# TinyMPC/tinympc-julia

Hardware: AMD Instinct MI355X
Metric: qp_solves_per_sec (higher is better)
Workload: dtype f64 recurrences and state trajectory, f32 input slack / dual

## Files before the change

### tinympc-julia_amd/csrc/admm_lean.hip.h

```cpp
#pragma once
#include <hip/hip_runtime.h>

#include "admm_params.h"
#include "admm_quad.hip.h"

#ifndef TMPC_LEAN_KNOT_BARRIER
#define TMPC_LEAN_KNOT_BARRIER 0
#endif
#ifndef TMPC_LEAN_SPLITK
#define TMPC_LEAN_SPLITK 0
#endif

#ifndef TMPC_LEAN_WIDE_STORE
#define TMPC_LEAN_WIDE_STORE 1
#endif
#ifndef TMPC_LEAN_STORE_W
#define TMPC_LEAN_STORE_W 0
#endif
#ifndef TMPC_LEAN_PK
#define TMPC_LEAN_PK 1
#endif
#ifndef TMPC_LEAN_FOLD_FIRST
#define TMPC_LEAN_FOLD_FIRST 0
#endif

namespace tmpc {

template <int NX, int NU>
struct LeanPack {
    static constexpr LeanLayout LL = lean_layout(NX, NU);
    static constexpr int O_M = LL.oM, O_K = LL.oK, O_B = LL.oB, O_C = LL.oC, O_H = LL.oH, O_S = LL.oS, O_P = LL.oP, O_T = LL.oT, LEN = LL.len;
    static constexpr int NLOADS = LL.padded / 8;
};

typedef float lean_f2 __attribute__((ext_vector_type(2)));

__device__ __forceinline__ float clamp3(float t, float lo, float hi) { return __builtin_amdgcn_fmed3f(t, lo, hi); }
__device__ __forceinline__ double clamp3(double t, double lo, double hi) { return fmin(fmax(t, lo), hi); }
__device__ __forceinline__ float lean_max(float a, float b) { return fmaxf(a, b); }
__device__ __forceinline__ double lean_max(double a, double b) { return fmax(a, b); }
__device__ __forceinline__ float lean_abs(float a) { return fabsf(a); }
__device__ __forceinline__ double lean_abs(double a) { return fabs(a); }

constexpr int lean_park_stride(int EX) { return (((EX + 3) / 4) % 2 ? (EX + 3) / 4 : (EX + 3) / 4 + 1) * 4; }
template <int NX, int NU, int N, bool LIVE, bool UBK, bool ONE, bool XB = false, int REFS = REF_ZERO, class ST = float, uint64_t SP = 0, bool WS = false,
          bool MPC = false>
__global__ __launch_bounds__(256, (ONE ? 1 : 2)) void admm_lean_kernel(const AdmmParams P) {
    constexpr bool F64 = std::is_same<ST, double>::value;
    static_assert(!F64 || ONE, "fp64 state: the 512-register form");
    static_assert(!WS || !F64, "kept workspace: fp32 state (the fp64 workspace has another format)");
    static_assert(!MPC || (WS && LIVE && ONE), "in-kernel closed loop: the tolerance-terminated workspace-keeping form");
    static_assert(REFS == REF_ZERO || REFS == REF_SHARED, "lean kernel: zero or shared references");
#ifdef TMPC_LEAN_CLOCK_PROBE
    const unsigned long long probe_entry = __builtin_amdgcn_s_memrealtime();
#endif
    using L = LeanPack<NX, NU>;
    constexpr int EX = NX * N, EU = NU * (N - 1);
    constexpr bool SPR = SP != 0;
    static_assert(!SPR || (NX <= 4 && NU <= 4), "sparse pattern: nx, nu <= 4");
    constexpr bool HB = !SPR && !LIVE && !XB && ONE;
    constexpr bool PK = TMPC_LEAN_PK && ONE && !LIVE && !XB && !WS && UBK && !F64;
    auto mh_zero = [](int m, int j) { return HB && j < m - NU; };
    auto bh_zero = [](int m, int a) { return HB && m > a; };
    auto a_nz = [](int m, int j) { return !SPR || lsp_a(SP, NX, m, j); };
    auto a_one = [](int m, int j) { return SPR && lsp_one(SP, NX, m, j); };
    auto b_nz = [](int m, int a) { return !SPR || lsp_b(SP, NU, m, a); };
    constexpr int BW = 2 * NX + 2 * NU;
    static_assert(L::NLOADS <= 4, "coefficient block too large for SGPRs");

    __shared__ float s_bnd[UBK ? 1 : 2 * NU * (N - 1)];
    __shared__ float s_xb[XB ? 2 * NX * N : 1];
    __shared__ double s_cq[REFS == REF_SHARED ? NX * N : 1], s_cr[REFS == REF_SHARED ? NU * (N - 1) : 1], s_cpt[REFS == REF_SHARED ? NX : 1];
    const int tid = threadIdx.x;
    if constexpr (!UBK) {
        for (int i = tid; i < 2 * NU * (N - 1); i += 256) {
            const int k = i / (2 * NU), j = i % (2 * NU);
            s_bnd[i] = P.bounds[k * BW + 2 * NX + j];
        }
    }
    if constexpr (XB)
        for (int i = tid; i < 2 * NX * N; i += 256) s_xb[i] = P.bounds[(i / (2 * NX)) * BW + i % (2 * NX)];
    if constexpr (REFS == REF_SHARED) {
        const float *qd = P.bounds + N * BW, *rd = qd + NX;
        const double irho = 1.0 / P.rho_family;
        for (int i = tid; i < NU * (N - 1); i += 256) s_cr[i] = (double)P.uref[i] * (double)rd[i % NU] * irho;
        if constexpr (HB) {
            const double *T = P.lean + L::O_T;
            for (int k = tid; k < N; k += 256) {
                double c[NX];
                for (int j = 0; j < NX; ++j) c[j] = (double)P.xref[k * NX + j] * (double)qd[j] * irho;
                for (int m = 0; m < NX; ++m) {
                    double acc = 0.0;
                    for (int j = 0; j < NX; ++j) acc = fma(T[j * NX + m], c[j], acc);
                    s_cq[k * NX + m] = acc;
                }
            }
            if (tid == 0) {
                double c[NX];
                for (int i = 0; i < NX; ++i) {
                    double acc = 0.0;
                    for (int j = 0; j < NX; ++j) acc = fma(P.lean[L::O_P + j * NX + i], (double)P.xref[(N - 1) * NX + j], acc);
                    c[i] = acc * irho;
                }
                for (int m = 0; m < NX; ++m) {
                    double acc = 0.0;
                    for (int j = 0; j < NX; ++j) acc = fma(T[j * NX + m], c[j], acc);
                    s_cpt[m] = acc;
                }
            }
        } else {
            for (int i = tid; i < NX * N; i += 256) s_cq[i] = (double)P.xref[i] * (double)qd[i % NX] * irho;
            if (tid < NX) {
                double acc = 0.0;
                for (int j = 0; j < NX; ++j) acc = fma(P.lean[L::O_P + j * NX + tid], (double)P.xref[(N - 1) * NX + j], acc);
                s_cpt[tid] = acc * irho;
            }
        }
    }
    __shared__ double s_T[HB ? NX * NX : 1];
    if constexpr (HB)
        if (tid < NX * NX) s_T[tid] = P.lean[L::O_T + tid];
    if constexpr (!UBK || XB || REFS == REF_SHARED || HB) __syncthreads();
    const long b = (long)blockIdx.x * 256 + tid;
    const bool active = b < P.batch;
    const int lane = tid & 63;
    constexpr int SW = !TMPC_LEAN_WIDE_STORE ? 0 : (TMPC_LEAN_STORE_W ? TMPC_LEAN_STORE_W : wide_stage_width(EX));
    static_assert(SW == 0 || (SW % 4 == 0 && EX % SW == 0), "wide store: W a multiple of 4 that divides nx N");
    constexpr int STAGE = SW ? wave_stage_floats_wide(EU, SW) : wave_stage_floats(EU);
    static_assert(SW == 0 || 4 * 64 * wide_stage_stride(SW) * sizeof(float) <= 48 * 1024, "wide store: staging beyond its 48 KiB");
    __shared__ __attribute__((aligned(16))) float s_stage[4][STAGE];
    constexpr bool PARK = WS && LIVE;
    constexpr int PVS = lean_park_stride(EX), PZS = EU | 1;
    __shared__ __attribute__((aligned(16))) float s_pv[PARK ? 256 * PVS : 4];
    __shared__ float s_pz[PARK ? 256 * PZS : 1];

    const SBlock<double, L::NLOADS> blk(P.lean + (HB ? L::O_H : (SPR ? L::O_S : 0)));
    const auto cM = blk.at(L::O_M), cK = blk.at(L::O_K), cB = blk.at(L::O_B), cC = blk.at(L::O_C);

    ST lo[NU], hi[NU];
#pragma unroll
    for (int a = 0; a < NU; ++a) lo[a] = (ST)P.bounds[2 * NX + a], hi[a] = (ST)P.bounds[2 * NX + NU + a];

    double X[XB ? 1 : N][NX];
    ST G[XB ? N : 1][NX], QT[XB ? N : 1][NX];
    ST Y[N - 1][NU], Z[N - 1][NU];
    using DT = std::conditional_t<ONE, double, float>;
    DT D[N - 1][NU];
#pragma unroll
    for (int m = 0; m < NX; ++m) {
        if constexpr (WS) X[0][m] = !active ? 0.0 : (P.x0d ? P.x0d[b * NX + m] : (double)P.x0[b * NX + m]);
        else X[0][m] = active ? (double)P.x0[b * NX + m] : 0.0;
    }
    if constexpr (HB) {
        double x0[NX];
#pragma unroll
        for (int m = 0; m < NX; ++m) x0[m] = X[0][m];
#pragma unroll
        for (int m = 0; m < NX; ++m) {
            double acc = P.lean[L::O_T + m] * x0[0];
#pragma unroll
            for (int j = 1; j < NX; ++j) acc = fma(P.lean[L::O_T + j * NX + m], x0[j], acc);
            X[0][m] = acc;
        }
    }
#pragma unroll
    for (int k = 1; k < (XB ? 1 : N); ++k)
#pragma unroll
        for (int m = 0; m < NX; ++m) X[k][m] = 0.0;
#pragma unroll
    for (int k = 0; k < (XB ? N : 1); ++k)
#pragma unroll
        for (int m = 0; m < NX; ++m) G[k][m] = (ST)0, QT[k][m] = (ST)0;
#pragma unroll
    for (int k = 0; k < N - 1; ++k)
#pragma unroll
        for (int a = 0; a < NU; ++a) Y[k][a] = (ST)0, Z[k][a] = (ST)0, D[k][a] = (DT)0;
    if constexpr (MPC) {
        const unsigned long long mask = __builtin_amdgcn_ballot_w64(active);
        int td = tid;
        asm volatile("" : "+v"(td));
        const int ln = td & 63;
        const long w0 = (long)blockIdx.x * 256 + (td & ~63);
        float *so = s_stage[td >> 6];
        load_wave_x<EX>(so, P.sv + w0 * EX, ln, mask, [&](auto ee, float val) { s_pv[td * PVS + decltype(ee)::value] = val; });
        load_wave_u<EU>(so, P.sz + w0 * EU, ln, mask, [&](auto ee, float val) { s_pz[td * PZS + decltype(ee)::value] = val; });
    }
    if constexpr (WS && !MPC) {
        if (!P.cold_start) {
            const unsigned long long mask = __builtin_amdgcn_ballot_w64(active);
            int td = tid;
            asm volatile("" : "+v"(td));
            const int ln = td & 63;
            const long w0 = (long)blockIdx.x * 256 + (td & ~63);
            float *so = s_stage[td >> 6];
            if (mask) {
                if constexpr (XB) {
                    load_wave_x<EX>(so, P.sg + w0 * EX, ln, mask, [&](auto ee, float val) { constexpr int e = decltype(ee)::value; G[e / NX][e % NX] = val; });
                    load_wave_x<EX>(so, P.sv + w0 * EX, ln, mask, [&](auto ee, float val) { constexpr int e = decltype(ee)::value; QT[e / NX][e % NX] = val - G[e / NX][e % NX]; });
                } else {
                    load_wave_x<EX>(so, P.sv + w0 * EX, ln, mask, [&](auto ee, float val) { constexpr int e = decltype(ee)::value; if constexpr (e >= NX) X[e / NX][e % NX] = (double)val; });
                    if constexpr (HB) {
#pragma unroll
                        for (int k = 1; k < N; ++k) {
                            double vk[NX];
#pragma unroll
                            for (int m = 0; m < NX; ++m) vk[m] = X[k][m];
#pragma unroll
                            for (int m = 0; m < NX; ++m) {
                                double acc = P.lean[L::O_T + m] * vk[0];
#pragma unroll
                                for (int j = 1; j < NX; ++j) acc = fma(P.lean[L::O_T + j * NX + m], vk[j], acc);
                                X[k][m] = acc;
                            }
                        }
                    }
                }
                load_wave_u<EU>(so, P.sy + w0 * EU, ln, mask, [&](auto ee, float val) { constexpr int e = decltype(ee)::value; Y[e / NU][e % NU] = val; });
                load_wave_u<EU>(so, P.sz + w0 * EU, ln, mask, [&](auto ee, float val) { constexpr int e = decltype(ee)::value; Z[e / NU][e % NU] = val; });
                load_wave_u<EU>(so, P.sd + w0 * EU, ln, mask, [&](auto ee, float val) { constexpr int e = decltype(ee)::value; D[e / NU][e % NU] = (DT)val; });
            }
        }
    }

#ifdef TMPC_LEAN_CLOCK_PROBE
    const unsigned long long probe_t0 = __builtin_amdgcn_s_memtime(), probe_r0 = __builtin_amdgcn_s_memrealtime();
#endif
    int it = 0, conv = 0;
    ST res0 = 0, res1 = 0, res2 = 0, res3 = 0;
    const int ct = P.check_termination;
    const int last_check_it = ct > 0 ? (P.max_iter / ct) * ct : 0;
    const ST rho = F64 ? (ST)P.rho_family : (ST)P.rho;
    const ST ptol = F64 ? (ST)P.abs_pri_tol64 : (ST)P.abs_pri_tol, dtol = F64 ? (ST)P.abs_dua_tol64 : (ST)P.abs_dua_tol;
    double dua_x = 0.0;
    ST pri_u = 0, dua_u = 0, pri_xf = 0, dua_xf = 0;
    auto park_v = [&](int k, const float (&pv)[NX]) {
        float *row = s_pv + tid * PVS + k * NX;
        if constexpr (NX % 4 == 0) {
#pragma unroll
            for (int q = 0; q < NX / 4; ++q)
                *reinterpret_cast<float4 *>(row + 4 * q) = make_float4(pv[4 * q], pv[4 * q + 1], pv[4 * q + 2], pv[4 * q + 3]);
        } else {
#pragma unroll
            for (int m = 0; m < NX; ++m) row[m] = pv[m];
        }
    };
    auto state_sets = [&](auto res_tag, auto kk, const double (&x)[NX]) {
        constexpr bool RES = decltype(res_tag)::value;
        constexpr int k = decltype(kk)::value;
#pragma unroll
        for (int m = 0; m < NX; ++m) {
            const ST xf = (ST)x[m];
            const ST t = xf + G[k][m];
            const ST vn = clamp3(t, (ST)s_xb[k * 2 * NX + m], (ST)s_xb[k * 2 * NX + NX + m]);
            const ST gn = t - vn;
            if constexpr (RES && PARK) {
                if constexpr (MPC) {
                    if (!conv) s_pv[tid * PVS + k * NX + m] = (float)(QT[k][m] + G[k][m]);
                } else {
                    s_pv[tid * PVS + k * NX + m] = (float)(QT[k][m] + G[k][m]);
                }
            }
            if constexpr (RES) {
                pri_xf = lean_max(pri_xf, lean_abs(xf - vn));
                dua_xf = lean_max(dua_xf, lean_abs((QT[k][m] + G[k][m]) - vn));
            }
            G[k][m] = gn;
            QT[k][m] = vn - gn;
        }
    };

    auto load_T = [&](double (&Tm)[NX * NX]) {
        const double *tp = s_T;
        asm volatile("" : "+v"(tp));
#pragma unroll
        for (int i = 0; i < NX * NX; ++i) Tm[i] = tp[i];
    };
    auto to_x = [](const double (&Tm)[NX * NX], const double (&xh)[NX], int m) {
        double acc = Tm[m * NX] * xh[0];
#pragma unroll
        for (int j = 1; j < NX; ++j) acc = fma(Tm[m * NX + j], xh[j], acc);
        return acc;
    };

    auto forward = [&](auto res_tag, bool first_iter) {
        constexpr bool RES = decltype(res_tag)::value;
        if constexpr (RES) {
            dua_x = 0.0, pri_u = 0, dua_u = 0, pri_xf = 0, dua_xf = 0;
            if constexpr (WS && !XB) {
                float v0p[NX];
#pragma unroll
                for (int m = 0; m < NX; ++m) v0p[m] = (float)X[0][m];
                if (first_iter) {
                    int td = tid;
                    asm volatile("" : "+v"(td));
                    const long bb = (long)blockIdx.x * 256 + td;
                    const bool warm0 = bb < P.batch && !P.cold_start;
                    double x0v[NX];
                    if constexpr (HB) {
                        double Tm[NX * NX];
#pragma unroll
                        for (int i = 0; i < NX * NX; ++i) Tm[i] = P.lean[L::O_T + i];
#pragma unroll
                        for (int m = 0; m < NX; ++m) x0v[m] = to_x(Tm, X[0], m);
                    } else {
#pragma unroll
                        for (int m = 0; m < NX; ++m) x0v[m] = X[0][m];
                    }
#pragma unroll
                    for (int m = 0; m < NX; ++m) {
                        if constexpr (MPC) v0p[m] = s_pv[td * PVS + m];
                        else v0p[m] = warm0 ? P.sv[bb * EX + m] : 0.f;
                        dua_x = fmax(dua_x, fabs((double)v0p[m] - x0v[m]));
                    }
                }
                if constexpr (PARK) {
                    if constexpr (MPC) {
                        if (!conv) park_v(0, v0p);
                    } else {
                        park_v(0, v0p);
                    }
                }
            }
            if constexpr (!WS && !XB)
                if (first_iter) {
#pragma unroll
                    for (int m = 0; m < NX; ++m) {
                        if constexpr (HB) {
                            double Tm[NX * NX];
                            load_T(Tm);
                            dua_x = fmax(dua_x, fabs(to_x(Tm, X[0], m)));
                        } else {
                            dua_x = fmax(dua_x, fabs(X[0][m]));
                        }
                    }
                }
        }
        if constexpr (HB || (SPR && (ONE || XB)))
#pragma unroll
            for (int m = 0; m < NX; ++m) asm volatile("" : "+v"(X[0][m]));
        double xr[NX];
#pragma unroll
        for (int m = 0; m < NX; ++m) xr[m] = X[0][m];
        float upk[PK ? NU : 1];
        sfor<0, N - 1>([&](auto kk) {
            constexpr int k = decltype(kk)::value;
            constexpr int kx = XB ? 0 : k;
            if constexpr (!UBK || XB) asm volatile("" ::: "memory");
            if constexpr (XB) state_sets(res_tag, kk, xr);
            const double (&xk)[NX] = XB ? xr : X[kx];
            double dk[NU], u[NU], xn[NX];
#pragma unroll
            for (int a = 0; a < NU; ++a) dk[a] = (double)D[k][a];
            bool started[NX];
            if constexpr (!SPR) {
#pragma unroll
                for (int m = 0; m < NX; ++m) {
                    started[m] = false;
#pragma unroll
                    for (int a = 0; a < NU; ++a) {
                        if (bh_zero(m, a)) continue;
                        xn[m] = started[m] ? fma(-cB[m * NU + a], dk[a], xn[m]) : -(cB[m * NU + a] * dk[a]);
                        started[m] = true;
                    }
                }
#pragma unroll
                for (int j = 0; j < NX; ++j)
#pragma unroll
                    for (int m = 0; m < NX; ++m) {
                        if (mh_zero(m, j)) continue;
                        xn[m] = started[m] ? fma(cM[m * NX + j], xk[j], xn[m]) : cM[m * NX + j] * xk[j];
                        started[m] = true;
                    }
            }
#pragma unroll
            for (int a = 0; a < NU; ++a) {
                if constexpr (SPR) {
                    double acc = -dk[a];
#pragma unroll
                    for (int pass = 0; pass < 2; ++pass)
#pragma unroll
                        for (int j = 0; j < NX; ++j) {
                            bool late = false;
#pragma unroll
                            for (int c = 0; c < NU; ++c) late = late || b_nz(j, c);
                            if (late == (pass == 1)) acc = fma(-cK[a * NX + j], xk[j], acc);
                        }
                    u[a] = acc;
                } else if constexpr (TMPC_LEAN_SPLITK && NX >= 4) {
                    double u0 = -dk[a], u1 = -(cK[a * NX + NX / 2] * xk[NX / 2]);
#pragma unroll
                    for (int j = 0; j < NX / 2; ++j) u0 = fma(-cK[a * NX + j], xk[j], u0);
#pragma unroll
                    for (int j = NX / 2 + 1; j < NX; ++j) u1 = fma(-cK[a * NX + j], xk[j], u1);
                    u[a] = u0 + u1;
                } else {
                    double acc = -dk[a];
#pragma unroll
                    for (int j = 0; j < NX; ++j) acc = fma(-cK[a * NX + j], xk[j], acc);
                    u[a] = acc;
                }
            }
            if constexpr (SPR) {
#pragma unroll
                for (int m = 0; m < NX; ++m) {
                    int s = -1;
#pragma unroll
                    for (int j = NX - 1; j >= 0; --j)
                        if (a_one(m, j)) s = j;
                    started[m] = s >= 0;
                    xn[m] = 0.0;
                    if (s >= 0) xn[m] = xk[s];
#pragma unroll
                    for (int j = 0; j < NX; ++j) {
                        if (!a_nz(m, j) || j == s) continue;
                        xn[m] = !started[m] ? cM[m * NX + j] * xk[j] : (a_one(m, j) ? xn[m] + xk[j] : fma(cM[m * NX + j], xk[j], xn[m]));
                        started[m] = true;
                    }
#pragma unroll
                    for (int a = 0; a < NU; ++a) {
                        if (!b_nz(m, a)) continue;
                        xn[m] = started[m] ? fma(cB[m * NU + a], u[a], xn[m]) : cB[m * NU + a] * u[a];
                        started[m] = true;
                    }
                }
            }
            constexpr bool PK_ODD = PK && !RES && (k & 1), PK_EVEN = PK && !RES && !(k & 1) && k + 1 < N - 1;
            if constexpr (PK_EVEN) {
#pragma unroll
                for (int a = 0; a < NU; ++a) upk[a] = (float)u[a];
            }
            if constexpr (PK_ODD) {
#pragma unroll
                for (int a = 0; a < NU; ++a) {
                    const lean_f2 t = lean_f2{upk[a], (float)u[a]} + lean_f2{(float)Y[k - 1][a], (float)Y[k][a]};
                    const lean_f2 zn = {clamp3(t.x, (float)lo[a], (float)hi[a]), clamp3(t.y, (float)lo[a], (float)hi[a])};
                    const lean_f2 yn = t - zn;
                    Y[k - 1][a] = yn.x, Y[k][a] = yn.y;
                    Z[k - 1][a] = zn.x, Z[k][a] = zn.y;
                }
            }
            if constexpr (!PK_ODD && !PK_EVEN)
#pragma unroll
            for (int a = 0; a < NU; ++a) {
                const ST uf = (ST)u[a];
                const ST t = uf + Y[k][a];
                ST l_ = lo[a], h_ = hi[a];
                if constexpr (!UBK) l_ = (ST)s_bnd[k * 2 * NU + a], h_ = (ST)s_bnd[k * 2 * NU + NU + a];
                const ST zn = clamp3(t, l_, h_);
                Y[k][a] = t - zn;
                if constexpr (RES) {
                    pri_u = lean_max(pri_u, lean_abs(uf - zn));
                    dua_u = lean_max(dua_u, lean_abs(Z[k][a] - zn));
                    if constexpr (PARK) {
                        if constexpr (MPC) {
                            if (!conv) s_pz[tid * PZS + k * NU + a] = (float)Z[k][a];
                        } else {
                            s_pz[tid * PZS + k * NU + a] = (float)Z[k][a];
                        }
                    }
                }
                Z[k][a] = zn;
            }
            if constexpr (RES && PARK && !XB) {
                float pv[NX];
#pragma unroll
                for (int m = 0; m < NX; ++m) pv[m] = (float)X[k + 1][m];
                if constexpr (MPC) {
                    if (!conv) park_v(k + 1, pv);
                } else {
                    park_v(k + 1, pv);
                }
            }
#pragma unroll
            for (int m = 0; m < NX; ++m) {
                if constexpr (XB) {
                    xr[m] = xn[m];
                } else {
                    if constexpr (RES && !HB) dua_x = fmax(dua_x, fabs(X[k + 1][m] - xn[m]));
                    if constexpr (!(RES && HB)) X[k + 1][m] = xn[m];
                }
            }
            if constexpr (RES && HB) {
                double dl[NX], Tm[NX * NX];
                load_T(Tm);
#pragma unroll
                for (int m = 0; m < NX; ++m) dl[m] = X[k + 1][m] - xn[m], X[k + 1][m] = xn[m];
#pragma unroll
                for (int m = 0; m < NX; ++m) dua_x = fmax(dua_x, fabs(to_x(Tm, dl, m)));
            }
            if constexpr (RES) asm volatile("" : "+v"(pri_u), "+v"(dua_u), "+v"(dua_x), "+v"(pri_xf), "+v"(dua_xf));
            if constexpr (TMPC_LEAN_KNOT_BARRIER) __builtin_amdgcn_sched_barrier(0);
        });
        if constexpr (XB) {
            asm volatile("" ::: "memory");
            state_sets(res_tag, std::integral_constant<int, N - 1>{}, xr);
            if constexpr (RES) asm volatile("" : "+v"(pri_xf), "+v"(dua_xf));
        }
    };

    auto backward = [&]() {
        double p[NX];
        if constexpr (REFS == REF_SHARED) asm volatile("" ::: "memory");
#pragma unroll
        for (int m = 0; m < NX; ++m) {
            p[m] = XB ? (double)QT[N - 1][m] : X[XB ? 0 : N - 1][m];
            if constexpr (REFS == REF_SHARED) p[m] += s_cpt[m];
        }
        float rpk[PK ? NU : 1];
        sfor<0, N - 1>([&](auto kk) {
            constexpr int k = N - 2 - decltype(kk)::value;
            double r[NU], t[NU];
            if constexpr (REFS == REF_SHARED) asm volatile("" ::: "memory");
#pragma unroll
            for (int a = 0; a < NU; ++a) {
                if constexpr (PK && (k & 1)) {
                    const lean_f2 rp = lean_f2{(float)Z[k - 1][a], (float)Z[k][a]} - lean_f2{(float)Y[k - 1][a], (float)Y[k][a]};
                    rpk[a] = rp.x;
                    r[a] = (double)rp.y;
                } else if constexpr (PK && k + 1 < N - 1) {
                    r[a] = (double)rpk[a];
                } else
                r[a] = (double)(Z[k][a] - Y[k][a]);
                if constexpr (REFS == REF_SHARED) r[a] += s_cr[k * NU + a];
                t[a] = r[a];
            }
#pragma unroll
            for (int j = 0; j < NX; ++j)
#pragma unroll
                for (int a = 0; a < NU; ++a)
                    if (!bh_zero(j, a) && b_nz(j, a)) t[a] = fma(cB[j * NU + a], p[j], t[a]);
#pragma unroll
            for (int a = 0; a < NU; ++a) {
                double acc = cC[a * NU] * t[0];
#pragma unroll
                for (int c = 1; c < NU; ++c) acc = fma(cC[a * NU + c], t[c], acc);
                D[k][a] = (DT)acc;
            }
            if constexpr (k > 0 && SPR) {
                double ap[NX];
#pragma unroll
                for (int m = 0; m < NX; ++m) {
                    double acc = XB ? (double)QT[k][m] : X[XB ? 0 : k][m];
                    if constexpr (REFS == REF_SHARED) acc += s_cq[k * NX + m];
#pragma unroll
                    for (int j = 0; j < NX; ++j)
                        if (a_nz(j, m)) acc = a_one(j, m) ? acc + p[j] : fma(cM[j * NX + m], p[j], acc);
#pragma unroll
                    for (int a = 0; a < NU; ++a) acc = fma(-cK[a * NX + m], t[a], acc);
                    ap[m] = acc;
                }
#pragma unroll
                for (int m = 0; m < NX; ++m) p[m] = ap[m];
            } else if constexpr (k > 0) {
                double ap[NX];
#pragma unroll
                for (int m = 0; m < NX; ++m) {
                    double acc = XB ? (double)QT[k][m] : X[XB ? 0 : k][m];
                    if constexpr (REFS == REF_SHARED) acc += s_cq[k * NX + m];
#pragma unroll
                    for (int a = 0; a < NU; ++a) acc = fma(-cK[a * NX + m], r[a], acc);
                    ap[m] = acc;
                }
#pragma unroll
                for (int j = 0; j < NX; ++j)
#pragma unroll
                    for (int m = 0; m < NX; ++m)
                        if (!mh_zero(j, m)) ap[m] = fma(cM[j * NX + m], p[j], ap[m]);
#pragma unroll
                for (int m = 0; m < NX; ++m) p[m] = ap[m];
            }
            if constexpr (TMPC_LEAN_KNOT_BARRIER) __builtin_amdgcn_sched_barrier(0);
        });
    };

    double Ts[HB ? NX * NX : 1];
    auto vnew_at = [&](auto kk, auto mm) -> float {
        constexpr int k = decltype(kk)::value, m = decltype(mm)::value;
        if constexpr (XB) return (float)clamp3(QT[k][m] + G[k][m], (ST)s_xb[k * 2 * NX + m], (ST)s_xb[k * 2 * NX + NX + m]);
        else if constexpr (HB) return (float)to_x(Ts, X[k], m);
        else return (float)X[XB ? 0 : k][m];
    };
    auto store = [&](bool solved_flag) {
        float *xo = P.xout + b * EX, *uo = P.uout + b * EU, *ro = P.res + b * 4;
        asm volatile("" : "+v"(xo), "+v"(uo), "+v"(ro));
        sfor<0, N>([&](auto kk) {
            constexpr int k = decltype(kk)::value;
            sfor<0, NX>([&](auto mm) { xo[k * NX + decltype(mm)::value] = vnew_at(kk, mm); });
            __builtin_amdgcn_sched_barrier(0);
        });
#pragma unroll
        for (int k = 0; k < N - 1; ++k)
#pragma unroll
            for (int a = 0; a < NU; ++a) uo[k * NU + a] = (float)Z[k][a];
        P.iter[b] = P.iter_offset + it;
        P.solved[b] = solved_flag ? 1 : 0;
        ro[0] = (float)res0;
        ro[1] = (float)res1;
        ro[2] = (float)res2;
        ro[3] = (float)res3;
    };

    auto store_ws = [&](unsigned long long mask, bool mine, auto conv_tag) {
        constexpr bool CV = decltype(conv_tag)::value;
        int td = tid;
        asm volatile("" : "+v"(td));
        const int ln = td & 63;
        const long bb = (long)blockIdx.x * 256 + td;
        float *so = s_stage[td >> 6];
        const long w0 = (long)blockIdx.x * 256 + (td & ~63);
        auto pair = [&](float *xo, float *uo, auto &&gx, auto &&gu) {
            if constexpr (SW != 0) store_wave_wide<EX, EU, SW>(so, xo, uo, ln, mask, gx, gu);
            else store_wave_coalesced<EX, EU>(so, xo, uo, ln, mask, gx, gu);
        };
        auto single = [&](float *uo, auto &&gu) {
            if constexpr (SW != 0) {
                if (mask == ~0ull) store_wave_u_wide<EU>(so, uo, ln, gu);
                else store_wave_u<EU, false>(so, uo, ln, mask, gu);
            } else {
                store_wave_u<EU, false>(so, uo, ln, mask, gu);
            }
        };
        auto getx = [&](auto ee) { constexpr int e = decltype(ee)::value; return vnew_at(std::integral_constant<int, e / NX>{}, std::integral_constant<int, e % NX>{}); };
        auto getu = [&](auto ee) { constexpr int e = decltype(ee)::value; return (float)Z[e / NU][e % NU]; };
        auto gety = [&](auto ee) { constexpr int e = decltype(ee)::value; return (float)Y[e / NU][e % NU]; };
        auto getd = [&](auto ee) { constexpr int e = decltype(ee)::value; return (float)D[e / NU][e % NU]; };
        pair(P.xout + w0 * EX, P.uout + w0 * EU, getx, getu);
        if (P.save_state) {
            if constexpr (CV) {
                pair(P.sv + w0 * EX, P.sz + w0 * EU, [&](auto ee) { return s_pv[td * PVS + decltype(ee)::value]; },
                     [&](auto ee) { return s_pz[td * PZS + decltype(ee)::value]; });
            } else {
                pair(P.sv + w0 * EX, P.sz + w0 * EU, getx, getu);
            }
            if constexpr (XB) pair(P.sg + w0 * EX, P.sy + w0 * EU, [&](auto ee) { constexpr int e = decltype(ee)::value; return (float)G[e / NX][e % NX]; }, gety);
            else single(P.sy + w0 * EU, gety);
            single(P.sd + w0 * EU, getd);
        }
        if (mine) {
            float *ro = P.res + bb * 4;
            P.iter[bb] = P.iter_offset + it;
            P.solved[bb] = CV ? 1 : 0;
            ro[0] = (float)res0, ro[1] = (float)res1, ro[2] = (float)res2, ro[3] = (float)res3;
        }
    };

    const bool can_converge = P.abs_pri_tol > 0.f && P.abs_dua_tol > 0.f;
    const int max_iter = P.max_iter;
    auto store_step = [&](unsigned long long mask) {
        int td = tid;
        asm volatile("" : "+v"(td));
        const int ln = td & 63;
        float *so = s_stage[td >> 6];
        const long w0 = (long)blockIdx.x * 256 + (td & ~63);
        auto single = [&](float *uo, auto &&gu) {
            if constexpr (SW != 0) {
                if (mask == ~0ull) store_wave_u_wide<EU>(so, uo, ln, gu);
                else store_wave_u<EU, false>(so, uo, ln, mask, gu);
            } else {
                store_wave_u<EU, false>(so, uo, ln, mask, gu);
            }
        };
        auto gety = [&](auto ee) { constexpr int e = decltype(ee)::value; return (float)Y[e / NU][e % NU]; };
        auto getd = [&](auto ee) { constexpr int e = decltype(ee)::value; return (float)D[e / NU][e % NU]; };
        if constexpr (XB) {
            auto getg = [&](auto ee) { constexpr int e = decltype(ee)::value; return (float)G[e / NX][e % NX]; };
            if constexpr (SW != 0) store_wave_wide<EX, EU, SW>(so, P.sg + w0 * EX, P.sy + w0 * EU, ln, mask, getg, gety);
            else store_wave_coalesced<EX, EU>(so, P.sg + w0 * EX, P.sy + w0 * EU, ln, mask, getg, gety);
        } else {
            single(P.sy + w0 * EU, gety);
        }
        single(P.sd + w0 * EU, getd);
    };
    float u0c[MPC ? NU : 1];
    auto plant = [&](int step, bool final_step) {
        const double *ab = P.lean + L::O_S;
        double xn[NX];
#pragma unroll
        for (int r = 0; r < NX; ++r) {
            double acc = 0.0;
#pragma unroll
            for (int j = 0; j < NX; ++j) acc = fma(ab[L::O_M + r * NX + j], X[0][j], acc);
#pragma unroll
            for (int a = 0; a < NU; ++a) acc = fma(ab[L::O_B + r * NU + a], (double)u0c[a], acc);
            xn[r] = acc;
        }
        int td = tid;
        asm volatile("" : "+v"(td));
        const long bb = (long)blockIdx.x * 256 + td;
        if (bb < P.batch) {
            const long so = bb * P.mpc_steps + step;
#pragma unroll
            for (int r = 0; r < NX; ++r) P.mpc_x[so * NX + r] = (float)xn[r];
#pragma unroll
            for (int a = 0; a < NU; ++a) P.mpc_u[so * NU + a] = u0c[a];
            P.mpc_iter[so] = conv ? P.iter_offset + it : -(P.iter_offset + it);
            if (final_step) {
#pragma unroll
                for (int r = 0; r < NX; ++r) P.x0_out[bb * NX + r] = (float)xn[r];
                if (double *xd = const_cast<double *>(P.x0d)) {
#pragma unroll
                    for (int r = 0; r < NX; ++r) xd[bb * NX + r] = xn[r];
                }
            }
        }
#pragma unroll
        for (int r = 0; r < NX; ++r) X[0][r] = xn[r];
    };
    int step = 0;
#ifdef TMPC_LEAN_CLOCK_PROBE
    unsigned long long probe_ph[4] = {0, 0, 0, 0}, probe_a = 0, probe_c = 0;
#endif
    do {
#ifdef TMPC_LEAN_CLOCK_PROBE
    probe_a = __builtin_amdgcn_s_memtime();
#endif
    if constexpr (MPC) {
        __builtin_amdgcn_fence(__ATOMIC_ACQUIRE, "agent");
        int td = tid;
        asm volatile("" : "+v"(td));
        const int ln = td & 63;
        const long w0 = (long)blockIdx.x * 256 + (td & ~63);
        const unsigned long long mask = __builtin_amdgcn_ballot_w64(w0 + ln < P.batch);
        float *so = s_stage[td >> 6];
        const float *rv = s_pv + td * PVS, *rz = s_pz + td * PZS;
        if constexpr (XB) {
            load_wave_x<EX>(so, P.sg + w0 * EX, ln, mask, [&](auto ee, float val) { constexpr int e = decltype(ee)::value; G[e / NX][e % NX] = val; });
            sfor<0, EX>([&](auto ee) { constexpr int e = decltype(ee)::value; QT[e / NX][e % NX] = rv[e] - G[e / NX][e % NX]; });
        } else {
            sfor<NX, EX>([&](auto ee) { constexpr int e = decltype(ee)::value; X[e / NX][e % NX] = (double)rv[e]; });
        }
        sfor<0, EU>([&](auto ee) { constexpr int e = decltype(ee)::value; Z[e / NU][e % NU] = rz[e]; });
        load_wave_u<EU>(so, P.sy + w0 * EU, ln, mask, [&](auto ee, float val) { constexpr int e = decltype(ee)::value; Y[e / NU][e % NU] = val; });
        load_wave_u<EU>(so, P.sd + w0 * EU, ln, mask, [&](auto ee, float val) { constexpr int e = decltype(ee)::value; D[e / NU][e % NU] = (DT)val; });
        it = 0, conv = 0;
        res0 = 0, res1 = 0, res2 = 0, res3 = 0;
    }
    const bool last_step = !MPC || step + 1 >= P.mpc_steps;
#ifdef TMPC_LEAN_CLOCK_PROBE
    probe_ph[0] += __builtin_amdgcn_s_memtime() - probe_a, probe_a = __builtin_amdgcn_s_memtime();
#endif
    int i = 0;
    while (i < max_iter) {
        int next_res = max_iter;
        if (ct > 0) {
            if (LIVE && can_converge) next_res = (i / ct) * ct + ct - 1;
            else if (last_check_it - 1 >= i) next_res = last_check_it - 1;
        }
        const int n_plain = (next_res < max_iter ? next_res : max_iter) - i;
        for (int j = 0; j < n_plain; ++j) {
            forward(std::false_type{}, false);
            backward();
        }
        i += n_plain;
        if (!LIVE || !conv) it += n_plain;
        if (i >= max_iter) break;
        forward(std::true_type{}, i == 0);
        i += 1;
        if (!LIVE || !conv) {
            it += 1;
            res0 = XB ? pri_xf : (ST)0;
            res1 = (XB ? dua_xf : (ST)dua_x) * rho;
            res2 = pri_u;
            res3 = dua_u * rho;
        }
        if constexpr (LIVE) {
            const bool now = active && !conv && res0 < ptol && res2 < ptol && res1 < dtol && res3 < dtol;
            if constexpr (WS) {
                const unsigned long long cm = __builtin_amdgcn_ballot_w64(now);
                if constexpr (MPC) {
#ifdef TMPC_LEAN_CLOCK_PROBE
                    probe_c = __builtin_amdgcn_s_memtime();
#endif
                    if (cm) {
                        if (last_step) store_ws(cm, now, std::true_type{});
                        else store_step(cm);
                    }
#ifdef TMPC_LEAN_CLOCK_PROBE
                    probe_ph[2] += __builtin_amdgcn_s_memtime() - probe_c;
#endif
                    if (now) {
#pragma unroll
                        for (int a = 0; a < NU; ++a) u0c[a] = (float)Z[0][a];
                    }
                } else
                if (cm) store_ws(cm, now, std::true_type{});
                if (now) conv = 1;
            } else
            if (now) {
                store(true);
                conv = 1;
            }
            if (!__builtin_amdgcn_ballot_w64(active && !conv)) break;
        }
        if (!(ONE && !XB) || WS || i < max_iter) backward();
    }
    if constexpr (MPC) {
#ifdef TMPC_LEAN_CLOCK_PROBE
        probe_ph[1] += __builtin_amdgcn_s_memtime() - probe_a, probe_a = __builtin_amdgcn_s_memtime();
#endif
#pragma unroll
        for (int a = 0; a < NU; ++a)
            if (!conv) u0c[a] = (float)Z[0][a];
        if (last_step) break;
        const bool mine = active && !conv;
        const unsigned long long mask = __builtin_amdgcn_ballot_w64(mine);
        if (mask) {
            if (mine) {
                int td = tid;
                asm volatile("" : "+v"(td));
                float *rv = s_pv + td * PVS, *rz = s_pz + td * PZS;
                sfor<0, EX>([&](auto ee) {
                    constexpr int e = decltype(ee)::value;
                    rv[e] = vnew_at(std::integral_constant<int, e / NX>{}, std::integral_constant<int, e % NX>{});
                });
                sfor<0, EU>([&](auto ee) { constexpr int e = decltype(ee)::value; rz[e] = (float)Z[e / NU][e % NU]; });
            }
            store_step(mask);
        }
        plant(step, false);
        asm volatile("s_waitcnt vmcnt(0)" ::: "memory");
#ifdef TMPC_LEAN_CLOCK_PROBE
        probe_ph[3] += __builtin_amdgcn_s_memtime() - probe_a;
#endif
        ++step;
    }
    } while (MPC);
    auto fold = [&]() {
        float m0 = active ? (float)res0 : 0.f, m1 = active ? (float)res1 : 0.f, m2 = active ? (float)res2 : 0.f, m3 = active ? (float)res3 : 0.f;
#pragma unroll
        for (int o = 1; o < 64; o <<= 1) {
            m0 = fmaxf(m0, __shfl_xor(m0, o, 64));
            m1 = fmaxf(m1, __shfl_xor(m1, o, 64));
            m2 = fmaxf(m2, __shfl_xor(m2, o, 64));
            m3 = fmaxf(m3, __shfl_xor(m3, o, 64));
        }
        const unsigned long long unsolved = __builtin_amdgcn_ballot_w64(active && !conv);
        if constexpr (WS) fold_status(P, m0, m1, m2, m3, __popcll(unsolved), tid);
        else fold_status_records(P, m0, m1, m2, m3, __popcll(unsolved), tid);
    };
#ifdef TMPC_LEAN_CLOCK_PROBE
    const unsigned long long probe_t1 = __builtin_amdgcn_s_memtime(), probe_r1 = __builtin_amdgcn_s_memrealtime();
    unsigned long long probe_fold = 0;
#endif
    if constexpr (TMPC_LEAN_FOLD_FIRST) {
        fold();
#ifdef TMPC_LEAN_CLOCK_PROBE
        probe_fold = __builtin_amdgcn_s_memrealtime();
#endif
    }
    {
        const bool mine = active && !conv;
        const unsigned long long mask = __builtin_amdgcn_ballot_w64(mine);
        if (mask) {
            if constexpr (HB) load_T(Ts);
            if constexpr (WS) {
                store_ws(mask, mine, std::false_type{});
            } else {
                const long w0 = (long)blockIdx.x * 256 + (tid & ~63);
                auto getx = [&](auto ee) { constexpr int e = decltype(ee)::value; return vnew_at(std::integral_constant<int, e / NX>{}, std::integral_constant<int, e % NX>{}); };
                auto getu = [&](auto ee) { constexpr int e = decltype(ee)::value; return (float)Z[e / NU][e % NU]; };
                if constexpr (SW != 0) store_wave_wide<EX, EU, SW>(s_stage[tid >> 6], P.xout + w0 * EX, P.uout + w0 * EU, lane, mask, getx, getu);
                else store_wave_coalesced<EX, EU>(s_stage[tid >> 6], P.xout + w0 * EX, P.uout + w0 * EU, lane, mask, getx, getu);
                if (mine) {
                    float *ro = P.res + b * 4;
                    P.iter[b] = P.iter_offset + it;
                    P.solved[b] = 0;
                    ro[0] = (float)res0, ro[1] = (float)res1, ro[2] = (float)res2, ro[3] = (float)res3;
                }
            }
        }
    }
    if constexpr (MPC) plant(step, true);
#ifdef TMPC_LEAN_CLOCK_PROBE
    if (active) P.iter[b] = (int)(__builtin_amdgcn_s_memrealtime() & 0xFFFFFFull);
    __builtin_amdgcn_s_waitcnt(0);
    if (active) P.solved[b] = (int)(__builtin_amdgcn_s_memrealtime() & 0xFFFFFFull);
#endif
    if constexpr (!TMPC_LEAN_FOLD_FIRST) {
        fold();
#ifdef TMPC_LEAN_CLOCK_PROBE
        probe_fold = __builtin_amdgcn_s_memrealtime();
#endif
    }
#ifdef TMPC_LEAN_CLOCK_PROBE
    if constexpr (MPC) {
        if (active)
            for (int q = 0; q < 4; ++q) P.res[b * 4 + q] = (float)probe_ph[q];
    } else
    if (active) {
        P.res[b * 4 + 0] = (float)(probe_t1 - probe_t0);
        P.res[b * 4 + 1] = (float)(probe_r1 - probe_r0);
        P.res[b * 4 + 2] = (float)(probe_entry & 0xFFFFFFull);
        P.res[b * 4 + 3] = (float)(probe_fold & 0xFFFFFFull);
    }
#endif
}

}
```

### tinympc-julia_amd/csrc/admm_params.h

```cpp
#pragma once
#include <stdint.h>

namespace tmpc {

enum RefMode : int {
    REF_ZERO = 0,
    REF_SHARED = 1,
    REF_PER_INSTANCE = 2,
};

enum { QUAD_REF_SEQ_MAX_N = 20 };

enum { GSTAT_WORDS = 8 };
enum { GSLOT_WORDS = 8, GSLOT_DEFAULT_CAP = 1024 };

constexpr int LIN_MAX_ROWS = 8, GEN_MAX_NX = 64;
constexpr int GEN_MAX_NU = 32;

struct AdmmParams {
    const float *coef;
    const float *bounds;
    const float *x0;
    const double *x0d;
    const float *xref;
    const float *uref;
    float *xout;
    float *uout;
    int *iter;
    int *solved;
    float *res;
    float *sd, *sy, *sz, *sg, *sv;
    uint32_t *gstat;
    uint32_t *gacc;
    float *scratch;
    const int *idx;
    int iter_offset;
    int batch;
    int max_iter;
    int check_termination;
    int ref_mode;
    int cold_start;
    int save_state;
    float abs_pri_tol, abs_dua_tol, rho;
    int nx, nu, N;
    int mpc_steps;
    float *mpc_x;
    float *mpc_u;
    int *mpc_iter;
    float *x0_out;
    int xb_active;
    int has_fdyn;
    int ncx, ncu;
    int Acx[8], qcx[8], Acu[8], qcu[8];
    float cx[8], cu[8];
    float *sgc, *svc, *syc, *szc;
    int mlx, mlu;
    const float *lin;
    float *sgl, *svl, *syl, *szl;
    int adaptive_rho;
    int rho_clip;
    double rho_family;
    float rho_min, rho_max;
    const double *sens;
    double *adapt;
    long adapt_stride;
    void *adp_cols;
    const float *het_aux;
    int bounds_stride;
    const float *xref_seq, *uref_seq;
    const double *lean;
    int host_flags;
    double *ws64;
    double abs_pri_tol64, abs_dua_tol64;
    uint32_t *gslot;
    int gslot_cap;
    const float *ibx, *ibu;
    long ib_kx, ib_ku, ib_hx, ib_hu;
    int ib_on;
};
enum : int { IB_STATE = 1, IB_INPUT = 2 };
enum : int { HF_NO_REFILL = 1, HF_NO_UNI = 2, HF_NO_OS = 4 };

struct LeanLayout {
    int oM;
    int oK;
    int oB;
    int oC;
    int len;
    int padded;
    int oH;
    int oS;
    int oP;
    int oT;
    int total;
};
constexpr LeanLayout lean_layout(int nx, int nu) {
    return LeanLayout{0, nx * nx, nx * nx + nu * nx, nx * nx + 2 * nu * nx, nx * nx + 2 * nu * nx + nu * nu,
                      (nx * nx + 2 * nu * nx + nu * nu + 7) / 8 * 8, (nx * nx + 2 * nu * nx + nu * nu + 7) / 8 * 8,
                      2 * ((nx * nx + 2 * nu * nx + nu * nu + 7) / 8 * 8),
                      3 * ((nx * nx + 2 * nu * nx + nu * nu + 7) / 8 * 8),
                      3 * ((nx * nx + 2 * nu * nx + nu * nu + 7) / 8 * 8) + nx * nx,
                      3 * ((nx * nx + 2 * nu * nx + nu * nu + 7) / 8 * 8) + 2 * nx * nx};
}

enum : int { LSP_UNIT = 16, LSP_B = 32, LSP_ON = 48 };
constexpr bool lsp_a(uint64_t sp, int nx, int i, int j) { return (sp >> (i * nx + j)) & 1; }
constexpr bool lsp_one(uint64_t sp, int nx, int i, int j) { return (sp >> (LSP_UNIT + i * nx + j)) & 1; }
constexpr bool lsp_b(uint64_t sp, int nu, int i, int a) { return (sp >> (LSP_B + i * nu + a)) & 1; }
constexpr uint64_t lean_pattern_rm(int nx, int nu, const double *A, const double *B) {
    if (nx < 1 || nu < 1 || nx > 4 || nu > 4) return 0;
    uint64_t sp = 1ull << LSP_ON;
    for (int i = 0; i < nx; ++i) {
        for (int j = 0; j < nx; ++j) {
            if (A[i * nx + j] != 0.0) sp |= 1ull << (i * nx + j);
            if (A[i * nx + j] == 1.0) sp |= 1ull << (LSP_UNIT + i * nx + j);
        }
        for (int a = 0; a < nu; ++a)
            if (B[i * nu + a] != 0.0) sp |= 1ull << (LSP_B + i * nu + a);
    }
    return sp;
}
constexpr int lean_cost_sparse(uint64_t sp, int nx, int nu) {
    int c = 2 * nx * nu + nu * nu;
    for (int i = 0; i < nx; ++i) {
        int terms = 0;
        bool unit = false;
        for (int j = 0; j < nx; ++j) terms += lsp_a(sp, nx, i, j), unit = unit || lsp_one(sp, nx, i, j);
        for (int a = 0; a < nu; ++a) terms += 2 * lsp_b(sp, nu, i, a);
        for (int j = 0; j < nx; ++j) terms += lsp_a(sp, nx, j, i);
        c += terms - (unit ? 1 : 0);
    }
    return c;
}
constexpr int lean_cost_hessenberg(int nx, int nu) {
    int band = 0, trap = 0;
    for (int m = 0; m < nx; ++m) {
        for (int j = 0; j < nx; ++j) band += j >= m - nu;
        for (int a = 0; a < nu; ++a) trap += m <= a;
    }
    return 2 * band + 2 * trap + 2 * nx * nu + nu * nu;
}
constexpr int lean_cost_dense(int nx, int nu) { return 2 * nx * nx + 4 * nx * nu + nu * nu; }
constexpr bool lean_pattern_covers(uint64_t built, uint64_t model) {
    const uint64_t nz = 0xFFFFull | (0xFFFFull << LSP_B), one = 0xFFFFull << LSP_UNIT;
    return built != 0 && model != 0 && (model & nz & ~built) == 0 && ((built & one) & ~(model & one)) == 0;
}

#ifdef __HIPCC__
__device__ __forceinline__ void fold_status(const AdmmParams &P, float m0, float m1, float m2, float m3,
                                            int unsolved_in_wave, int tid) {
    __shared__ float s_fold_m[4][4];
    __shared__ int s_fold_u[4];
    const int w = tid >> 6, nw = ((int)blockDim.x + 63) >> 6;
    const bool merged = nw <= 4;
    if ((tid & 63) == 0) {
        if (merged) {
            s_fold_m[w][0] = m0, s_fold_m[w][1] = m1, s_fold_m[w][2] = m2, s_fold_m[w][3] = m3;
            s_fold_u[w] = unsolved_in_wave;
        } else {
            atomicMax(&P.gacc[0], __float_as_uint(m0));
            atomicMax(&P.gacc[1], __float_as_uint(m1));
            atomicMax(&P.gacc[2], __float_as_uint(m2));
            atomicMax(&P.gacc[3], __float_as_uint(m3));
            if (unsolved_in_wave) atomicAdd(&P.gacc[4], (uint32_t)unsolved_in_wave);
        }
    }
    __syncthreads();
    if (tid == 0) {
        if (merged) {
            int un = 0;
            for (int i = 0; i < nw; ++i) {
                m0 = i ? fmaxf(m0, s_fold_m[i][0]) : s_fold_m[0][0];
                m1 = i ? fmaxf(m1, s_fold_m[i][1]) : s_fold_m[0][1];
                m2 = i ? fmaxf(m2, s_fold_m[i][2]) : s_fold_m[0][2];
                m3 = i ? fmaxf(m3, s_fold_m[i][3]) : s_fold_m[0][3];
                un += s_fold_u[i];
            }
            atomicMax(&P.gacc[0], __float_as_uint(m0));
            atomicMax(&P.gacc[1], __float_as_uint(m1));
            atomicMax(&P.gacc[2], __float_as_uint(m2));
            atomicMax(&P.gacc[3], __float_as_uint(m3));
            if (un) atomicAdd(&P.gacc[4], (uint32_t)un);
        }
        __threadfence();
        if (atomicAdd(&P.gacc[7], 1u) == gridDim.x - 1) {
            __threadfence();
            uint32_t tot[5];
#pragma unroll
            for (int i = 0; i < 5; ++i) tot[i] = atomicExch(&P.gacc[i], 0u);
            atomicExch(&P.gacc[6], 0u);
            atomicExch(&P.gacc[7], 0u);
#pragma unroll
            for (int i = 0; i < 5; ++i) P.gstat[i] = tot[i];
        }
    }
}

__device__ __forceinline__ void fold_status_records(const AdmmParams &P, float m0, float m1, float m2, float m3,
                                            int unsolved_in_wave, int tid) {
    __shared__ float s_fold_m[4][4];
    __shared__ int s_fold_u[4];
    const int w = tid >> 6, nw = ((int)blockDim.x + 63) >> 6;
    const bool merged = nw <= 4;
    if ((tid & 63) == 0) {
        if (merged) {
            s_fold_m[w][0] = m0, s_fold_m[w][1] = m1, s_fold_m[w][2] = m2, s_fold_m[w][3] = m3;
            s_fold_u[w] = unsolved_in_wave;
        } else {
            atomicMax(&P.gacc[0], __float_as_uint(m0));
            atomicMax(&P.gacc[1], __float_as_uint(m1));
            atomicMax(&P.gacc[2], __float_as_uint(m2));
            atomicMax(&P.gacc[3], __float_as_uint(m3));
            if (unsolved_in_wave) atomicAdd(&P.gacc[4], (uint32_t)unsolved_in_wave);
        }
    }
    __syncthreads();
    if (tid >= 64) return;
    const int nrec = P.gslot ? min((int)gridDim.x, P.gslot_cap) : 0;
    int last = 0;
    if (tid == 0) {
        bool recorded = false;
        if (merged) {
            int un = 0;
            for (int i = 0; i < nw; ++i) {
                m0 = i ? fmaxf(m0, s_fold_m[i][0]) : s_fold_m[0][0];
                m1 = i ? fmaxf(m1, s_fold_m[i][1]) : s_fold_m[0][1];
                m2 = i ? fmaxf(m2, s_fold_m[i][2]) : s_fold_m[0][2];
                m3 = i ? fmaxf(m3, s_fold_m[i][3]) : s_fold_m[0][3];
                un += s_fold_u[i];
            }
            if ((int)blockIdx.x < nrec) {
                unsigned long long *rec = reinterpret_cast<unsigned long long *>(P.gslot + (size_t)blockIdx.x * GSLOT_WORDS);
                __hip_atomic_store(rec + 0, (unsigned long long)__float_as_uint(m0) | ((unsigned long long)__float_as_uint(m1) << 32),
                                   __ATOMIC_RELAXED, __HIP_MEMORY_SCOPE_AGENT);
                __hip_atomic_store(rec + 1, (unsigned long long)__float_as_uint(m2) | ((unsigned long long)__float_as_uint(m3) << 32),
                                   __ATOMIC_RELAXED, __HIP_MEMORY_SCOPE_AGENT);
                __hip_atomic_store(rec + 2, (unsigned long long)(uint32_t)un, __ATOMIC_RELAXED, __HIP_MEMORY_SCOPE_AGENT);
                asm volatile("s_waitcnt vmcnt(0)" ::: "memory");
                recorded = true;
            } else {
                atomicMax(&P.gacc[0], __float_as_uint(m0));
                atomicMax(&P.gacc[1], __float_as_uint(m1));
                atomicMax(&P.gacc[2], __float_as_uint(m2));
                atomicMax(&P.gacc[3], __float_as_uint(m3));
                if (un) atomicAdd(&P.gacc[4], (uint32_t)un);
            }
        }
        if (!recorded) __threadfence();
        last = __hip_atomic_fetch_add(&P.gacc[7], 1u, __ATOMIC_RELAXED, __HIP_MEMORY_SCOPE_AGENT) == gridDim.x - 1;
    }
    if (!__shfl(last, 0, 64)) return;
    __builtin_amdgcn_fence(__ATOMIC_ACQUIRE, "agent");
    uint32_t tot[5] = {0, 0, 0, 0, 0};
    if (tid == 0) {
#pragma unroll
        for (int i = 0; i < 5; ++i) tot[i] = atomicExch(&P.gacc[i], 0u);
        atomicExch(&P.gacc[6], 0u);
        atomicExch(&P.gacc[7], 0u);
    }
    uint32_t r0 = 0, r1 = 0, r2 = 0, r3 = 0, ru = 0;
    for (int base = 0; base < nrec; base += 4 * 64) {
        unsigned long long a[4], b[4], c[4];
#pragma unroll
        for (int q = 0; q < 4; ++q) {
            const int s = min(base + q * 64 + tid, nrec - 1);
            unsigned long long *rec = reinterpret_cast<unsigned long long *>(P.gslot + (size_t)s * GSLOT_WORDS);
            a[q] = __hip_atomic_load(rec + 0, __ATOMIC_RELAXED, __HIP_MEMORY_SCOPE_AGENT);
            b[q] = __hip_atomic_load(rec + 1, __ATOMIC_RELAXED, __HIP_MEMORY_SCOPE_AGENT);
            c[q] = __hip_atomic_load(rec + 2, __ATOMIC_RELAXED, __HIP_MEMORY_SCOPE_AGENT);
        }
#pragma unroll
        for (int q = 0; q < 4; ++q)
            if (base + q * 64 + tid >= nrec) a[q] = b[q] = c[q] = 0;
#pragma unroll
        for (int q = 0; q < 4; ++q) {
            r0 = max(r0, (uint32_t)a[q]), r1 = max(r1, (uint32_t)(a[q] >> 32));
            r2 = max(r2, (uint32_t)b[q]), r3 = max(r3, (uint32_t)(b[q] >> 32));
            ru += (uint32_t)c[q];
        }
    }
    if (nrec) {
#pragma unroll
        for (int off = 1; off < 64; off <<= 1) {
            r0 = max(r0, (uint32_t)__shfl_xor((int)r0, off, 64)), r1 = max(r1, (uint32_t)__shfl_xor((int)r1, off, 64));
            r2 = max(r2, (uint32_t)__shfl_xor((int)r2, off, 64)), r3 = max(r3, (uint32_t)__shfl_xor((int)r3, off, 64));
            ru += (uint32_t)__shfl_xor((int)ru, off, 64);
        }
    }
    if (tid == 0) {
        tot[0] = max(tot[0], r0), tot[1] = max(tot[1], r1), tot[2] = max(tot[2], r2), tot[3] = max(tot[3], r3), tot[4] += ru;
#pragma unroll
        for (int i = 0; i < 5; ++i) P.gstat[i] = tot[i];
    }
}
#endif

}
```

### tinympc-julia_amd/csrc/kernels.hip

```cpp
#include <algorithm>
#include <atomic>
#include <cmath>
#include <cstring>
#include <limits>

#include "admm_generic.hip.h"
#include "host_setup.h"
#include "solver.h"

namespace tmpc {

#define TMPC_ENTRY(NX, NU, NN, GG) const KernelEntry *quad_entry_##NX##_##NU##_##NN##_g##GG();
TMPC_ENTRY(4, 1, 20, 4) TMPC_ENTRY(4, 1, 20, 2) TMPC_ENTRY(4, 1, 20, 1)
TMPC_ENTRY(4, 1, 10, 4) TMPC_ENTRY(4, 1, 10, 2) TMPC_ENTRY(4, 1, 10, 1) TMPC_ENTRY(4, 1, 2, 4)
TMPC_ENTRY(4, 1, 5, 4) TMPC_ENTRY(4, 1, 5, 1) TMPC_ENTRY(4, 1, 15, 4) TMPC_ENTRY(4, 1, 15, 1) TMPC_ENTRY(4, 1, 30, 4) TMPC_ENTRY(4, 1, 30, 1)
TMPC_ENTRY(12, 4, 30, 4) TMPC_ENTRY(12, 4, 20, 4)
TMPC_ENTRY(6, 3, 10, 4) TMPC_ENTRY(6, 3, 10, 2) TMPC_ENTRY(6, 3, 50, 4)
#undef TMPC_ENTRY

const KernelEntry *find_quad_kernel(int nx, int nu, int N, int group) {
    static const KernelEntry *const table[] = {
        quad_entry_4_1_20_g4(),  quad_entry_4_1_20_g2(),  quad_entry_4_1_20_g1(), quad_entry_4_1_10_g4(),
        quad_entry_4_1_10_g2(),  quad_entry_4_1_10_g1(),  quad_entry_4_1_2_g4(),  quad_entry_12_4_30_g4(),
        quad_entry_12_4_20_g4(), quad_entry_6_3_10_g4(),  quad_entry_6_3_10_g2(), quad_entry_6_3_50_g4(),
        quad_entry_4_1_5_g4(),   quad_entry_4_1_5_g1(),   quad_entry_4_1_15_g4(), quad_entry_4_1_15_g1(),
        quad_entry_4_1_30_g4(),  quad_entry_4_1_30_g1(),
    };
    for (const KernelEntry *e : table)
        if (e->nx == nx && e->nu == nu && e->N == N && (group < 0 || e->G == group)) return e;
    return jit_find(false, nx, nu, N, group);
}

const KernelEntry *mfma_entry_12_4_30();
const KernelEntry *mfma_entry_12_4_25();
const KernelEntry *mfma_entry_12_4_20();
const KernelEntry *mfma_entry_12_4_15();
const KernelEntry *mfma_entry_12_4_10();

const KernelEntry *find_mfma_kernel(int nx, int nu, int N) {
    static const KernelEntry *const table[] = {mfma_entry_12_4_30(), mfma_entry_12_4_25(), mfma_entry_12_4_20(), mfma_entry_12_4_15(),
                                               mfma_entry_12_4_10()};
    for (const KernelEntry *e : table)
        if (e->nx == nx && e->nu == nu && e->N == N) return e;
    return jit_find(true, nx, nu, N, -1);
}

const LeanEntry *lean_entry_4_1_20();
const LeanEntry *lean_entry_4_1_15();
const LeanEntry *lean_entry_4_1_10();
const LeanEntry *lean_entry_4_1_5();

const LeanEntry *find_lean_kernel(int nx, int nu, int N) {
    static const LeanEntry *const table[] = {lean_entry_4_1_20(), lean_entry_4_1_15(), lean_entry_4_1_10(), lean_entry_4_1_5()};
    for (const LeanEntry *e : table)
        if (e->nx == nx && e->nu == nu && e->N == N) return e;
    return nullptr;
}

bool build_lean_pack(const Solver &sv, std::vector<double> &out) {
    const int nx = sv.nx, nu = sv.nu;
    const LeanLayout L = lean_layout(nx, nu);
    out.assign((size_t)L.total, 0.0);
    const Cache &c = sv.cache;
    double scale = 0.0, diff = 0.0;
    for (int i = 0; i < nx; ++i)
        for (int j = 0; j < nx; ++j) {
            double m = sv.A(i, j);
            for (int a = 0; a < nu; ++a) m -= sv.B(i, a) * c.Kinf(a, j);
            out[L.oM + i * nx + j] = m;
            scale = std::max(scale, std::fabs(m));
            diff = std::max(diff, std::fabs(m - c.AmBKt(j, i)));
        }
    if (!(diff <= 1e-12 * std::max(scale, 1.0))) return false;
    for (int i = 0; i < nx; ++i)
        for (int j = 0; j < nx; ++j) out[L.oM + i * nx + j] = c.AmBKt(j, i);
    for (int a = 0; a < nu; ++a)
        for (int j = 0; j < nx; ++j) out[L.oK + a * nx + j] = c.Kinf(a, j);
    for (int i = 0; i < nx; ++i)
        for (int a = 0; a < nu; ++a) out[L.oB + i * nu + a] = sv.B(i, a);
    for (int a = 0; a < nu; ++a)
        for (int b2 = 0; b2 < nu; ++b2) out[L.oC + a * nu + b2] = -c.rho * c.Quu_inv(a, b2);
    for (int i = 0; i < nx; ++i)
        for (int j = 0; j < nx; ++j) out[L.oP + i * nx + j] = c.Pinf(i, j);
    std::vector<double> Mh((size_t)nx * nx), Bh((size_t)nx * nu);
    staircase_form(nx, nu, out.data() + L.oM, out.data() + L.oB, out.data() + L.oT, Mh.data(), Bh.data());
    const double *T = out.data() + L.oT;
    for (int i = 0; i < nx * nx; ++i) out[L.oH + L.oM + i] = Mh[i];
    for (int i = 0; i < nx * nu; ++i) out[L.oH + L.oB + i] = Bh[i];
    for (int a = 0; a < nu; ++a)
        for (int j = 0; j < nx; ++j) {
            double s = 0.0;
            for (int l = 0; l < nx; ++l) s += c.Kinf(a, l) * T[l * nx + j];
            out[L.oH + L.oK + a * nx + j] = s;
        }
    for (int i = 0; i < nu * nu; ++i) out[L.oH + L.oC + i] = out[L.oC + i];
    for (int i = 0; i < nx; ++i)
        for (int j = 0; j < nx; ++j) out[L.oS + L.oM + i * nx + j] = sv.A(i, j);
    for (int i = L.oK; i < L.len; ++i) out[L.oS + i] = out[i];
    return true;
}

void append_lean_bounds(const Solver &sv, std::vector<double> &out) {
    constexpr float kInf = std::numeric_limits<float>::infinity();
    const int nx = sv.nx, nu = sv.nu, N = sv.N, BW = 2 * nx + 2 * nu;
    std::vector<float> lb((size_t)N * BW + nx + nu + 1, 0.f);
    for (int k = 0; k < N; ++k) {
        float *p = lb.data() + (size_t)k * BW;
        for (int r = 0; r < nx; ++r) {
            p[r] = sv.st.en_state_bound ? (float)sv.x_min[r + (size_t)k * nx] : -kInf;
            p[nx + r] = sv.st.en_state_bound ? (float)sv.x_max[r + (size_t)k * nx] : kInf;
        }
        for (int a = 0; a < nu; ++a) {
            const bool on = sv.st.en_input_bound && k < N - 1;
            p[2 * nx + a] = on ? (float)sv.u_min[a + (size_t)k * nu] : -kInf;
            p[2 * nx + nu + a] = on ? (float)sv.u_max[a + (size_t)k * nu] : kInf;
        }
    }
    for (int r = 0; r < nx; ++r) lb[(size_t)N * BW + r] = (float)sv.cache.Qd[r];
    for (int a = 0; a < nu; ++a) lb[(size_t)N * BW + nx + a] = (float)sv.cache.Rd[a];
    const size_t at = out.size();
    out.resize(at + (lb.size() + 1) / 2, 0.0);
    std::memcpy(out.data() + at, lb.data(), lb.size() * sizeof(float));
}

LeanPlan lean_plan(const LeanPlanIn &in) {
    LeanPlan p;
    const int nx = in.nx, nu = in.nu, N = in.N;
    const bool f64 = in.precision == 2 && in.quad_G == 0 && in.lean_jit && !in.stream_ext;
    if (!(in.quad_G ? in.precision == 0 : f64) || !in.lean_ok || !(in.builtin || in.lean_jit)) return p;
    if (in.indexed || in.ref_mode == REF_PER_INSTANCE || in.adaptive_rho || in.iters < 1) return p;
    const bool ws = !(in.cold && !in.save);
    if (ws && !(in.sw_ws && in.quad_G > 0 && in.quad_G < 16 && in.precision == 0 && (!in.builtin || (in.kinds & LK_WS)))) return p;
    const bool mpc = in.loop && in.sw_loop && ws && in.mpc_steps > 0;
    if ((in.loop || in.mpc_steps > 0) && !mpc) return p;
    const bool xb = in.state_bounds || (ws && in.g_maybe_nonzero), shared = in.ref_mode == REF_SHARED;
    const bool live = in.live || mpc || (ws && xb && shared && in.knot_bounds);
    const bool one = live || ws || f64 || in.sw_one || (in.slots + 255) / 256 <= in.cus ||
                     (!in.builtin && 2 * N * nx + 3 * N * nu + 50 > 250);
    if (ws && !in.builtin && !lean_ws_fits(nx, nu, N, live, xb, shared, in.knot_bounds)) return p;
    bool sparse_allowed = !in.sw_dense;
    p.sp = in.model_sp;
    if (in.builtin) {
        const bool has = (in.kinds & (mpc ? LK_SPARSE_MPC : (ws ? LK_SPARSE_WS : LK_SPARSE))) != 0;
        p.sp = has ? in.builtin_sp : 0;
        sparse_allowed = sparse_allowed && has && in.ref_mode == REF_ZERO && !in.knot_bounds;
    }
    p.form = lean_pick_form(nx, nu, p.sp, in.model_sp, one, live, xb, sparse_allowed);
    if (mpc && in.builtin && !(in.kinds & (p.form == LF_SPARSE ? LK_SPARSE_MPC : LK_MPC))) return LeanPlan();
    p.take = true;
    p.variant = (live ? LV_LIVE : 0) | (in.knot_bounds ? 0 : LV_UBK) | (one ? LV_ONE : 0) | (xb ? LV_XB : 0) | (shared ? LV_SHARED : 0) |
                (f64 ? LV_F64 : 0) | (p.form == LF_SPARSE ? LV_SPARSE : 0) | (ws ? LV_WS : 0) | (mpc ? LV_MPC : 0);
    p.cost_sparse = p.sp ? lean_cost_sparse(p.sp, nx, nu) : 0;
    p.cost_dense = (one && !live && !xb) ? lean_cost_hessenberg(nx, nu) : lean_cost_dense(nx, nu);
    return p;
}

uint64_t lean_pattern(const Mat &A, const Mat &B) {
    const int nx = A.r, nu = B.c;
    if (nx < 1 || nu < 1 || nx > 4 || nu > 4) return 0;
    double a[16], b[16];
    for (int i = 0; i < nx; ++i) {
        for (int j = 0; j < nx; ++j) a[i * nx + j] = A(i, j);
        for (int c = 0; c < nu; ++c) b[i * nu + c] = B(i, c);
    }
    return lean_pattern_rm(nx, nu, a, b);
}

}

extern "C" unsigned long long tmpc_lean_pattern(int nx, int nu, const double *A, const double *B) {
    return (A && B) ? tmpc::lean_pattern_rm(nx, nu, A, B) : 0;
}
extern "C" int tmpc_lean_costs(int nx, int nu, unsigned long long sp, int *out3) {
    if (nx < 1 || nu < 1 || nx > 4 || nu > 4 || !out3) return 1;
    out3[0] = tmpc::lean_cost_sparse(sp, nx, nu), out3[1] = tmpc::lean_cost_hessenberg(nx, nu), out3[2] = tmpc::lean_cost_dense(nx, nu);
    return 0;
}
extern "C" int tmpc_lean_covers(unsigned long long built, unsigned long long model) { return tmpc::lean_pattern_covers(built, model) ? 1 : 0; }
extern "C" int tmpc_lean_pick_form(int nx, int nu, unsigned long long built, unsigned long long model, int one, int live, int xb) {
    return tmpc::lean_pick_form(nx, nu, built, model, one != 0, live != 0, xb != 0, true);
}
extern "C" unsigned long long tmpc_lean_builtin_pattern(int nx, int nu, int N) {
    const tmpc::LeanEntry *e = tmpc::find_lean_kernel(nx, nu, N);
    return (e && (e->kinds & tmpc::LK_SPARSE)) ? e->sp : 0;
}
extern "C" int tmpc_lean_plan(const int *in, int n_in, unsigned long long builtin_sp, unsigned long long model_sp, int *out5,
                              unsigned long long *weighed) {
    if (!in || n_in != 28 || !out5) return -1;
    tmpc::LeanPlanIn q;
    int i = 0;
    q.nx = in[i++], q.nu = in[i++], q.N = in[i++];
    q.builtin = in[i++] != 0, q.kinds = in[i++], q.builtin_sp = builtin_sp;
    q.lean_jit = in[i++] != 0, q.lean_ok = in[i++] != 0, q.model_sp = model_sp, q.knot_bounds = in[i++] != 0;
    q.quad_G = in[i++], q.precision = in[i++];
    q.sw_one = in[i++] != 0, q.sw_dense = in[i++] != 0, q.sw_ws = in[i++] != 0, q.sw_loop = in[i++] != 0;
    q.slots = in[i++], q.iters = in[i++], q.mpc_steps = in[i++];
    q.cold = in[i++] != 0, q.save = in[i++] != 0, q.indexed = in[i++] != 0, q.adaptive_rho = in[i++] != 0;
    q.ref_mode = in[i++];
    q.loop = in[i++] != 0, q.state_bounds = in[i++] != 0, q.g_maybe_nonzero = in[i++] != 0, q.live = in[i++] != 0, q.stream_ext = in[i++] != 0;
    q.cus = in[i++];
    const tmpc::LeanPlan p = tmpc::lean_plan(q);
    out5[0] = p.take ? 1 : 0, out5[1] = p.variant, out5[2] = p.form, out5[3] = p.cost_sparse, out5[4] = p.cost_dense;
    if (weighed) *weighed = p.sp;
    return 0;
}

namespace tmpc {

const KernelEntry *select_quad_kernel(int nx, int nu, int N, int batch) {
    const int pref[2][3] = {{1, 2, 4}, {4, 2, 1}};
    const int *order = batch >= 20480 ? pref[0] : pref[1];
    for (int i = 0; i < 3; ++i)
        if (const KernelEntry *e = find_quad_kernel(nx, nu, N, order[i])) return e;
    return nullptr;
}

const ConeEntry *mfmac_entry_6_3();
const ConeEntry *mfmar_entry_6_3_50();
const ConeEntry *mfmar_entry_6_3_10();
const ConeEntry *mfmar_entry_6_3_20();
const ConeEntry *mfmar_entry_6_3_30();

const ConeEntry *find_cone_kernel(int nx, int nu, int N) {
    static const ConeEntry *const table[] = {mfmar_entry_6_3_50(), mfmar_entry_6_3_30(), mfmar_entry_6_3_20(), mfmar_entry_6_3_10(), mfmac_entry_6_3()};
    for (const ConeEntry *e : table)
        if (e->nx == nx && e->nu == nu && e->N == N) return e;
    return nullptr;
}

const ConeEntry *mfmat_entry_6_3_50();
const ConeEntry *mfmat_entry_6_3_30();
const ConeEntry *mfmat_entry_6_3_20();
const ConeEntry *mfmat_entry_6_3_10();

const ConeEntry *find_trans_kernel(int nx, int nu, int N) {
    static const ConeEntry *const table[] = {mfmat_entry_6_3_50(), mfmat_entry_6_3_30(), mfmat_entry_6_3_20(), mfmat_entry_6_3_10()};
    for (const ConeEntry *e : table)
        if (e->nx == nx && e->nu == nu && e->N == N) return e;
    return nullptr;
}

int device_cu_count() {
    static std::atomic<int> cus[64];
    int dev = 0;
    if (hipGetDevice(&dev) != hipSuccess) return 256;
    int c = cus[dev & 63].load(std::memory_order_relaxed);
    if (c <= 0) {
        hipDeviceProp_t prop;
        c = hipGetDeviceProperties(&prop, dev) == hipSuccess && prop.multiProcessorCount > 0 ? prop.multiProcessorCount : 256;
        cus[dev & 63].store(c, std::memory_order_relaxed);
    }
    return c;
}

const StreamEntry *stream4_entry_2_1();
const StreamEntry *stream4_entry_2_2();
const StreamEntry *stream4_entry_3_1();
const StreamEntry *stream4_entry_3_2();
const StreamEntry *stream4_entry_3_3();
const StreamEntry *stream4_entry_4_1();
const StreamEntry *stream4_entry_4_2();
const StreamEntry *stream4_entry_4_3();
const StreamEntry *stream4_entry_4_4();
const StreamEntry *stream4_entry_6_1();
const StreamEntry *stream4_entry_6_2();
const StreamEntry *stream4_entry_6_3();
const StreamEntry *stream4_entry_6_4();
const StreamEntry *stream4_entry_8_1();
const StreamEntry *stream4_entry_8_2();
const StreamEntry *stream4_entry_8_3();
const StreamEntry *stream4_entry_8_4();
const StreamEntry *stream4_entry_10_1();
const StreamEntry *stream4_entry_10_2();
const StreamEntry *stream4_entry_10_3();
const StreamEntry *stream4_entry_10_4();
const StreamEntry *stream4_entry_12_1();
const StreamEntry *stream4_entry_12_2();
const StreamEntry *stream4_entry_12_3();
const StreamEntry *stream4_entry_12_4();

const StreamEntry *find_stream_kernel(int nx, int nu) {
    static const StreamEntry *const table[] = {stream4_entry_2_1(), stream4_entry_2_2(), stream4_entry_3_1(), stream4_entry_3_2(), stream4_entry_3_3(), stream4_entry_4_1(), stream4_entry_4_2(), stream4_entry_4_3(), stream4_entry_4_4(), stream4_entry_6_1(), stream4_entry_6_2(), stream4_entry_6_3(), stream4_entry_6_4(), stream4_entry_8_1(), stream4_entry_8_2(), stream4_entry_8_3(), stream4_entry_8_4(), stream4_entry_10_1(), stream4_entry_10_2(), stream4_entry_10_3(), stream4_entry_10_4(), stream4_entry_12_1(), stream4_entry_12_2(), stream4_entry_12_3(), stream4_entry_12_4()};
    for (const StreamEntry *e : table)
        if (e->nx == nx && e->nu == nu) return e;
    return nullptr;
}

hipError_t launch_generic(const AdmmParams &P, int precision, hipStream_t stream) {
    const int threads = 256;
    const int grid = (P.batch + threads - 1) / threads;
    if (P.ibx) {
        if (precision == 2)
            hipLaunchKernelGGL((admm_generic_kernel<double, double, true>), dim3(grid), dim3(threads), 0, stream, P);
        else if (precision == 0)
            hipLaunchKernelGGL((admm_generic_kernel<double, float, true>), dim3(grid), dim3(threads), 0, stream, P);
        else
            hipLaunchKernelGGL((admm_generic_kernel<float, float, true>), dim3(grid), dim3(threads), 0, stream, P);
        return hipGetLastError();
    }
    if (precision == 2)
        hipLaunchKernelGGL((admm_generic_kernel<double, double>), dim3(grid), dim3(threads), 0, stream, P);
    else if (precision == 0)
        hipLaunchKernelGGL((admm_generic_kernel<double, float>), dim3(grid), dim3(threads), 0, stream, P);
    else
        hipLaunchKernelGGL((admm_generic_kernel<float, float>), dim3(grid), dim3(threads), 0, stream, P);
    return hipGetLastError();
}

template <class RT>
static void fill_generic_coef(const Solver &sv, std::vector<unsigned char> &out) {
    const int nx = sv.nx, nu = sv.nu;
    const GenericPack pk(nx, nu);
    out.assign((size_t)pk.len * sizeof(RT), 0);
    auto put = [&](size_t idx, double val) {
        const RT v = (RT)val;
        std::memcpy(out.data() + idx * sizeof(RT), &v, sizeof(RT));
    };
    const Cache &c = sv.cache;
    for (int j = 0; j < nx; ++j)
        for (int i = 0; i < nx; ++i) {
            put(pk.oA + i + j * nx, sv.A(i, j));
            put(pk.oP + i + j * nx, c.Pinf(i, j));
            put(pk.oAt + i + j * nx, c.AmBKt(i, j));
        }
    for (int a = 0; a < nu; ++a)
        for (int i = 0; i < nx; ++i) {
            put(pk.oB + i + a * nx, sv.B(i, a));
            put(pk.oK + a + i * nu, c.Kinf(a, i));
        }
// ... 43 lines not shown
```

### tinympc-julia_amd/csrc/lean_entry.hip.h

```cpp
#pragma once
#include <hip/hip_ext.h>

#include "admm_lean.hip.h"
#include "solver.h"

namespace tmpc {

template <class K>
inline void lean_dispatch(K kernel, int grid, hipStream_t stream, hipEvent_t ev0, hipEvent_t ev1, const AdmmParams &P) {
    if (ev0 || ev1) hipExtLaunchKernelGGL(kernel, dim3(grid), dim3(256), 0, stream, ev0, ev1, 0, P);
    else hipLaunchKernelGGL(kernel, dim3(grid), dim3(256), 0, stream, P);
}

#define TMPC_LEAN_ARGS const AdmmParams &P, int variant, hipStream_t stream, hipEvent_t ev0, hipEvent_t ev1

template <int NX, int NU, int N, bool XB, int REFS, bool WS = false, bool MPC = false>
hipError_t launch_lean_v(TMPC_LEAN_ARGS) {
    const int grid = (P.batch + 255) / 256;
    constexpr bool FIXED = !MPC, FIXED_KNOT = FIXED && !(WS && XB && REFS == REF_SHARED), TWO = !WS;
#define TMPC_LEAN_LAUNCH(LIVE_, UBK_, ONE_) \
    lean_dispatch(admm_lean_kernel<NX, NU, N, LIVE_, UBK_, ONE_, XB, REFS, float, 0, WS, MPC>, grid, stream, ev0, ev1, P)
    switch (variant & (LV_LIVE | LV_UBK | LV_ONE)) {
        case LV_LIVE | LV_UBK | LV_ONE: TMPC_LEAN_LAUNCH(true, true, true); break;
        case LV_LIVE | LV_ONE: TMPC_LEAN_LAUNCH(true, false, true); break;
        case LV_UBK | LV_ONE: if constexpr (FIXED) TMPC_LEAN_LAUNCH(false, true, true); else return hipErrorNotSupported; break;
        case LV_ONE: if constexpr (FIXED_KNOT) TMPC_LEAN_LAUNCH(false, false, true); else return hipErrorNotSupported; break;
        case LV_UBK: if constexpr (TWO) TMPC_LEAN_LAUNCH(false, true, false); else return hipErrorNotSupported; break;
        case 0: if constexpr (TWO) TMPC_LEAN_LAUNCH(false, false, false); else return hipErrorNotSupported; break;
        default: return hipErrorNotSupported;
    }
#undef TMPC_LEAN_LAUNCH
    return hipGetLastError();
}

template <int NX, int NU, int N>
hipError_t launch_lean(TMPC_LEAN_ARGS) {
    if (variant & (LV_F64 | LV_SPARSE | LV_WS | LV_MPC)) return hipErrorNotSupported;
    if (variant & LV_SHARED)
        return (variant & LV_XB) ? launch_lean_v<NX, NU, N, true, REF_SHARED>(P, variant, stream, ev0, ev1)
                                 : launch_lean_v<NX, NU, N, false, REF_SHARED>(P, variant, stream, ev0, ev1);
    return (variant & LV_XB) ? launch_lean_v<NX, NU, N, true, REF_ZERO>(P, variant, stream, ev0, ev1)
                             : launch_lean_v<NX, NU, N, false, REF_ZERO>(P, variant, stream, ev0, ev1);
}

template <int NX, int NU, int N, uint64_t SP, bool WS = false, bool MPC = false>
hipError_t launch_lean_sparse(TMPC_LEAN_ARGS) {
    if ((variant & (LV_UBK | LV_SHARED)) != LV_UBK) return hipErrorNotSupported;
    const int grid = (P.batch + 255) / 256;
#define TMPC_LEAN_LAUNCH(LIVE_, ONE_, XB_) \
    lean_dispatch(admm_lean_kernel<NX, NU, N, LIVE_, true, ONE_, XB_, REF_ZERO, float, SP, WS, MPC>, grid, stream, ev0, ev1, P)
    switch (variant & (LV_LIVE | LV_ONE | LV_XB)) {
        case LV_LIVE | LV_ONE | LV_XB: TMPC_LEAN_LAUNCH(true, true, true); break;
        case LV_LIVE | LV_ONE: TMPC_LEAN_LAUNCH(true, true, false); break;
        case LV_ONE | LV_XB: if constexpr (!MPC) TMPC_LEAN_LAUNCH(false, true, true); else return hipErrorNotSupported; break;
        case LV_ONE: if constexpr (!MPC) TMPC_LEAN_LAUNCH(false, true, false); else return hipErrorNotSupported; break;
        case LV_XB: if constexpr (!WS) TMPC_LEAN_LAUNCH(false, false, true); else return hipErrorNotSupported; break;
        case 0: if constexpr (!WS) TMPC_LEAN_LAUNCH(false, false, false); else return hipErrorNotSupported; break;
        default: return hipErrorNotSupported;
    }
#undef TMPC_LEAN_LAUNCH
    return hipGetLastError();
}

template <int NX, int NU, int N, int V, class ST, uint64_t SP>
hipError_t launch_lean_exact(TMPC_LEAN_ARGS) {
    if (variant != V) return hipErrorNotSupported;
    lean_dispatch(admm_lean_kernel<NX, NU, N, (V & LV_LIVE) != 0, (V & LV_UBK) != 0, (V & LV_ONE) != 0, (V & LV_XB) != 0,
                                   (V & LV_SHARED) ? REF_SHARED : REF_ZERO, ST, SP, (V & LV_WS) != 0, (V & LV_MPC) != 0>,
                  (P.batch + 255) / 256, stream, ev0, ev1, P);
    return hipGetLastError();
}
#define TMPC_DEFINE_LEAN_JIT_VARIANT(NAME, NX, NU, NN, V, ST, SP)                                                       \
    namespace tmpc {                                                                                                     \
    const LeanEntry *lean_jit_entry() {                                                                                  \
        static const LeanEntry e = {NX, NU, NN, NAME, SP, 0, &launch_lean_exact<NX, NU, NN, (V), ST, SP>};               \
        return &e;                                                                                                       \
    }                                                                                                                    \
    }                                                                                                                    \
    extern "C" const void *tmpc_jit_entry() { return tmpc::lean_jit_entry(); }
#define TMPC_LEAN_BITS(LIVE, UBK, ONE, XB, REFS, ST, SP)                                                                 \
    ((LIVE ? tmpc::LV_LIVE : 0) | (UBK ? tmpc::LV_UBK : 0) | (ONE ? tmpc::LV_ONE : 0) | (XB ? tmpc::LV_XB : 0) |       \
     ((REFS) == tmpc::REF_SHARED ? tmpc::LV_SHARED : 0) | (sizeof(ST) == 8 ? tmpc::LV_F64 : 0) | ((SP) ? tmpc::LV_SPARSE : 0))
#define TMPC_DEFINE_LEAN_JIT_ENTRY_SP(NAME, NX, NU, NN, LIVE, UBK, ONE, XB, REFS, ST, SP) \
    TMPC_DEFINE_LEAN_JIT_VARIANT(NAME, NX, NU, NN, TMPC_LEAN_BITS(LIVE, UBK, ONE, XB, REFS, ST, SP), ST, SP)
#define TMPC_DEFINE_LEAN_JIT_ENTRY(NAME, NX, NU, NN, LIVE, UBK, ONE, XB, REFS, ST) \
    TMPC_DEFINE_LEAN_JIT_ENTRY_SP(NAME, NX, NU, NN, LIVE, UBK, ONE, XB, REFS, ST, 0)
#define TMPC_DEFINE_LEAN_JIT_ENTRY_WS(NAME, NX, NU, NN, LIVE, UBK, ONE, XB, REFS, SP) \
    TMPC_DEFINE_LEAN_JIT_VARIANT(NAME, NX, NU, NN, TMPC_LEAN_BITS(LIVE, UBK, ONE, XB, REFS, float, SP) | tmpc::LV_WS, float, SP)
#define TMPC_DEFINE_LEAN_JIT_ENTRY_MPC(NAME, NX, NU, NN, LIVE, UBK, ONE, XB, REFS, SP) \
    TMPC_DEFINE_LEAN_JIT_VARIANT(NAME, NX, NU, NN, TMPC_LEAN_BITS(LIVE, UBK, ONE, XB, REFS, float, SP) | tmpc::LV_WS | tmpc::LV_MPC, float, SP)

#define TMPC_DEFINE_LEAN_ENTRY(NX, NU, NN)                                                                \
    const LeanEntry *lean_entry_##NX##_##NU##_##NN() {                                                    \
        static const LeanEntry e = {NX, NU, NN, "lean<" #NX "," #NU "," #NN ">", 0, 0, &launch_lean<NX, NU, NN>}; \
        return &e;                                                                                        \
    }

constexpr double kCartpoleA[16] = {1.0, 0.01, 0.0, 0.0,
                                   0.0, 1.0, 0.039, 0.0,
                                   0.0, 0.0, 1.002, 0.01,
                                   0.0, 0.0, 0.458, 1.002};
constexpr double kCartpoleB[4] = {0.0, 0.02, 0.0, 0.067};
constexpr uint64_t kCartpolePattern = lean_pattern_rm(4, 1, kCartpoleA, kCartpoleB);

#define TMPC_DECLARE_LEAN_PARTS(KIND, NX, NU, NN)                          \
    hipError_t lean_##KIND##_##NX##_##NU##_##NN##_z(TMPC_LEAN_ARGS);      \
    hipError_t lean_##KIND##_##NX##_##NU##_##NN##_zx(TMPC_LEAN_ARGS);     \
    hipError_t lean_##KIND##_##NX##_##NU##_##NN##_s(TMPC_LEAN_ARGS);      \
    hipError_t lean_##KIND##_##NX##_##NU##_##NN##_sx(TMPC_LEAN_ARGS);     \
    hipError_t lean_##KIND##_##NX##_##NU##_##NN##_sparse(TMPC_LEAN_ARGS);
#define TMPC_LEAN_PARTS(KIND, NX, NU, NN)                                                                              \
    {&lean_##KIND##_##NX##_##NU##_##NN##_z, &lean_##KIND##_##NX##_##NU##_##NN##_zx, &lean_##KIND##_##NX##_##NU##_##NN##_s, \
     &lean_##KIND##_##NX##_##NU##_##NN##_sx, &lean_##KIND##_##NX##_##NU##_##NN##_sparse}
#define TMPC_DEFINE_LEAN_PART(KIND, WS, MPC, NX, NU, NN, TAG, XB, REFS)                          \
    hipError_t lean_##KIND##_##NX##_##NU##_##NN##_##TAG(TMPC_LEAN_ARGS) {                         \
        return launch_lean_v<NX, NU, NN, XB, REFS, WS, MPC>(P, variant, stream, ev0, ev1);        \
    }
#define TMPC_DEFINE_LEAN_PART_SPARSE(KIND, WS, MPC, NX, NU, NN, SP)                               \
    hipError_t lean_##KIND##_##NX##_##NU##_##NN##_sparse(TMPC_LEAN_ARGS) {                        \
        return launch_lean_sparse<NX, NU, NN, (SP), WS, MPC>(P, variant, stream, ev0, ev1);       \
    }
#define TMPC_DEFINE_LEAN_WS_PART(NX, NU, NN, TAG, XB, REFS) TMPC_DEFINE_LEAN_PART(ws, true, false, NX, NU, NN, TAG, XB, REFS)
#define TMPC_DEFINE_LEAN_WS_SPARSE(NX, NU, NN, SP) TMPC_DEFINE_LEAN_PART_SPARSE(ws, true, false, NX, NU, NN, SP)
#define TMPC_DEFINE_LEAN_MPC_PART(NX, NU, NN, TAG, XB, REFS) TMPC_DEFINE_LEAN_PART(mpc, true, true, NX, NU, NN, TAG, XB, REFS)
#define TMPC_DEFINE_LEAN_MPC_SPARSE(NX, NU, NN, SP) TMPC_DEFINE_LEAN_PART_SPARSE(mpc, true, true, NX, NU, NN, SP)
#define TMPC_DEFINE_LEAN_ENTRY_FULL(NX, NU, NN, SP)                                                                    \
    TMPC_DECLARE_LEAN_PARTS(ws, NX, NU, NN)                                                                            \
    TMPC_DECLARE_LEAN_PARTS(mpc, NX, NU, NN)                                                                           \
    static hipError_t lean_launch_##NX##_##NU##_##NN(TMPC_LEAN_ARGS) {                                                 \
        static constexpr LeanLaunch ws[5] = TMPC_LEAN_PARTS(ws, NX, NU, NN), mpc[5] = TMPC_LEAN_PARTS(mpc, NX, NU, NN); \
        if (variant & LV_F64) return hipErrorNotSupported;                                                             \
        const int part = (variant & LV_SPARSE) ? 4 : ((variant & LV_SHARED) ? 2 : 0) + ((variant & LV_XB) ? 1 : 0);    \
        if (variant & LV_MPC) return mpc[part](P, variant, stream, ev0, ev1);                                          \
        if (variant & LV_WS) return ws[part](P, variant, stream, ev0, ev1);                                            \
        return part == 4 ? launch_lean_sparse<NX, NU, NN, (SP)>(P, variant, stream, ev0, ev1)                          \
                         : launch_lean<NX, NU, NN>(P, variant, stream, ev0, ev1);                                      \
    }                                                                                                                  \
    const LeanEntry *lean_entry_##NX##_##NU##_##NN() {                                                                 \
        static const LeanEntry e = {NX, NU, NN, "lean<" #NX "," #NU "," #NN ">", (SP), LK_ALL, &lean_launch_##NX##_##NU##_##NN}; \
        return &e;                                                                                                     \
    }

}
```

### tinympc-julia_amd/csrc/linst_4_1_20.hip

```cpp
#include "lean_entry.hip.h"
namespace tmpc {
TMPC_DEFINE_LEAN_ENTRY_FULL(4, 1, 20, kCartpolePattern)
}
```

### tinympc-julia_amd/csrc/solver.h

```cpp
#pragma once
#include <hip/hip_runtime.h>

#include <string>
#include <vector>

#include "admm_params.h"
#include "host_setup.h"

namespace tmpc {

struct Solver;

struct KernelEntry {
    int nx, nu, N, G;
    const char *name;
    void (*build_coef)(const Solver &, std::vector<unsigned char> &);
    void (*build_bounds)(const Solver &, std::vector<float> &);
    hipError_t (*launch)(const AdmmParams &, int precision, bool state_bounds_active, hipStream_t);
    bool adp = false;
    bool jit = false;
};
const KernelEntry *jit_kernel_for(int nx, int nu, int N, int verbose);
const KernelEntry *jit_find(bool mfma, int nx, int nu, int N, int group);
struct ConeEntry;
const ConeEntry *jit_trans_find(const Solver &);
const ConeEntry *jit_trans_for(const Solver &, int verbose);
const KernelEntry *find_quad_kernel(int nx, int nu, int N, int group = -1);
const KernelEntry *select_quad_kernel(int nx, int nu, int N, int batch);
const KernelEntry *find_mfma_kernel(int nx, int nu, int N);
enum { LV_LIVE = 1, LV_UBK = 2, LV_ONE = 4, LV_XB = 8, LV_SHARED = 16, LV_F64 = 32, LV_SPARSE = 64, LV_WS = 128, LV_MPC = 256, LV_COUNT = 512 };
enum { LK_SPARSE = 1, LK_WS = 2, LK_SPARSE_WS = 4, LK_MPC = 8, LK_SPARSE_MPC = 16, LK_ALL = 31 };
using LeanLaunch = hipError_t (*)(const AdmmParams &, int variant, hipStream_t, hipEvent_t ev0, hipEvent_t ev1);
struct LeanEntry {
    int nx, nu, N;
    const char *name;
    uint64_t sp;
    int kinds;
    LeanLaunch launch;
};
const LeanEntry *find_lean_kernel(int nx, int nu, int N);
const LeanEntry *jit_lean_for(int nx, int nu, int N, int variant, uint64_t sp, int verbose);
bool lean_ws_fits(int nx, int nu, int N, bool live, bool xb, bool shared, bool knot_bounds);
int device_cu_count();
enum { LF_NONE = 0, LF_PLAIN = 1, LF_HB = 2, LF_SPARSE = 3 };
inline int lean_pick_form(int nx, int nu, uint64_t built, uint64_t model, bool one, bool live, bool xb, bool sparse_allowed) {
    const bool hb = one && !live && !xb;
    const int dense = hb ? lean_cost_hessenberg(nx, nu) : lean_cost_dense(nx, nu);
    if (sparse_allowed && lean_pattern_covers(built, model) && lean_cost_sparse(built, nx, nu) < dense) return LF_SPARSE;
    return hb ? LF_HB : LF_PLAIN;
}
struct LeanPlanIn {
    int nx = 0, nu = 0, N = 0;
    bool builtin = false;
    int kinds = 0;
    uint64_t builtin_sp = 0;
    bool lean_jit = false;
    bool lean_ok = false;
    uint64_t model_sp = 0;
    bool knot_bounds = false;
    int quad_G = 0;
    int precision = 0;
    bool sw_one = false, sw_dense = false, sw_ws = false, sw_loop = false;
    int slots = 0, iters = 0, mpc_steps = 0;
    bool cold = false, save = false, indexed = false, adaptive_rho = false;
    int ref_mode = REF_ZERO;
    bool loop = false;
    bool state_bounds = false;
    bool g_maybe_nonzero = false;
    bool live = false;
    bool stream_ext = false;
    int cus = 256;
};
struct LeanPlan {
    bool take = false;
    int variant = 0;
    int form = LF_NONE;
    uint64_t sp = 0;
    int cost_sparse = 0, cost_dense = 0;
};
LeanPlan lean_plan(const LeanPlanIn &);
uint64_t lean_pattern(const Mat &A, const Mat &B);
bool build_lean_pack(const Solver &, std::vector<double> &);
void append_lean_bounds(const Solver &, std::vector<double> &);
struct StreamEntry {
    int nx, nu;
    int lanes;
    const char *name;
    void (*build_coef)(const Solver &, std::vector<unsigned char> &);
    void (*build_bounds)(const Solver &, std::vector<float> &);
    size_t (*lds_bytes)(int N, int precision);
    size_t (*scratch_floats)(int N, int sets);
    hipError_t (*launch)(const AdmmParams &, int precision, int ext, bool het, hipStream_t);
    hipError_t (*launch_f64)(const AdmmParams &, int ext, hipStream_t) = nullptr;
    const char *name_f64 = nullptr;
    hipError_t (*launch_mpc)(const AdmmParams &, int precision, int ext, bool het, hipStream_t) = nullptr;
    bool (*has_mpc)(int precision, int ext, bool het) = nullptr;
    hipError_t (*launch_ib)(const AdmmParams &, int ext, bool het, hipStream_t) = nullptr;
    const char *name_ib = nullptr;
};
const StreamEntry *find_stream_kernel(int nx, int nu);
struct ConeEntry {
    int nx, nu;
    int N;
    bool (*supports)(const Solver &);
    bool plain;
    const char *name;
    void (*build_coef)(const Solver &, std::vector<unsigned char> &);
    void (*build_bounds)(const Solver &, std::vector<float> &);
    size_t (*lds_bytes)(const Solver &);
    size_t (*scratch_floats)(const Solver &);
    bool (*bounds_vary)(const Solver &);
    hipError_t (*launch)(const AdmmParams &, bool ext, size_t lds, hipStream_t);
    bool ws = false;
};
const ConeEntry *find_cone_kernel(int nx, int nu, int N);
const ConeEntry *find_trans_kernel(int nx, int nu, int N);
hipError_t launch_generic(const AdmmParams &, int precision, hipStream_t);
void build_generic_coef(const Solver &, std::vector<unsigned char> &);
void build_generic_bounds(const Solver &, std::vector<float> &);

struct Switches {
    int group = 0;
    bool strict_fp32 = false, no_quad = false, no_quad_adp = false, no_quad_adp1 = false, no_mfma = false, no_mfma_adp = false,
         mfma_oneshot_only = false, no_stream = false, no_stream_adp = false, no_mfmar = false, no_mfmac = false, mfmac_all = false,
         no_mfmat = false, mfmat_all = false, mfmat_ws_only = false, no_lean = false, no_refill = false,
         no_uni = false, no_os = false, lean_one = false,
         no_jit = false,
         lean_dense = false,
         lean_ws = false,
         lean_loop = false,
         stream_f64 = false,
         stream_mpc = false,
         stream_loop = false,
         event_markers = false,
         noise_split = false;
    int mfmac_debug = 0;
    int fold_slots = -1;
};
Switches read_switches();

struct Settings {
    double abs_pri_tol = 1e-3, abs_dua_tol = 1e-3;
    int max_iter = 100;
    int check_termination = 1;
    int en_state_bound = 0, en_input_bound = 0;
    int en_state_soc = 0, en_input_soc = 0;
    int en_state_linear = 0, en_input_linear = 0;
    int adaptive_rho = 0, adaptive_rho_clip = 1;
    double adaptive_rho_min = 0.1, adaptive_rho_max = 10.0;
};

struct Solver {
    int nx = 0, nu = 0, N = 0, batch = 1, device = 0;
    int verbose = 0;
    Mat A, B, Q, R;
    Cache cache;
    Settings st;
    std::vector<double> x_min, x_max, u_min, u_max;
    int bounds_mode = 0;
    std::vector<double> ib_xmin, ib_xmax, ib_umin, ib_umax;
    float *d_ibx = nullptr, *d_ibu = nullptr;
    int set_instance_bounds(const double *xmin, const double *xmax, const double *umin, const double *umax, int per_knot);
    void drop_instance_bounds();
    int upload_instance_bounds();
    std::vector<double> fdyn;
    bool has_fdyn = false;
    int ncx = 0, ncu = 0;
    int Acx[8] = {0}, qcx[8] = {0}, Acu[8] = {0}, qcu[8] = {0};
    double cx[8] = {0}, cu[8] = {0};
    float *d_sgc = nullptr, *d_svc = nullptr, *d_syc = nullptr, *d_szc = nullptr;
    bool cones_active() const { return (st.en_state_soc && ncx > 0) || (st.en_input_soc && ncu > 0); }
    int mlx = 0, mlu = 0;
    std::vector<double> lin_Ax, lin_bx, lin_Au, lin_bu;
    float *d_lin = nullptr, *d_sgl = nullptr, *d_svl = nullptr, *d_syl = nullptr, *d_szl = nullptr;
    bool lin_dirty = false;
    bool lin_active() const { return (st.en_state_linear && mlx > 0) || (st.en_input_linear && mlu > 0); }
    int constraint_sets() const { return lin_active() ? 3 : (cones_active() ? 2 : 1); }
    std::vector<double> sens;
    bool sens_set = false, sens_dirty = true, adapt_dirty = true;
    bool adapt_pure = true;
    double *d_sens = nullptr, *d_adapt = nullptr;
    unsigned char *d_adp_cols = nullptr;
    size_t adp_cols_bytes = 0;
    int set_sensitivity(const double *dK, const double *dP);
    int get_adaptive_state(double *rho, double *Kinf, double *Pinf);
    bool hetero = false;
    bool no_specialise = false;
    bool layout_final = false;
    std::vector<double> het_A, het_B;
    std::vector<Cache> het_cache;
    float *d_het_aux = nullptr;
    std::vector<float> h_xref, h_uref;
    int xref_kind = 0, uref_kind = 0;
    bool refs_dirty = true;
    bool refs_device_owned = false;
    bool refs_per_instance() const { return refs_device_owned ? ref_mode == REF_PER_INSTANCE : (xref_kind >= 2 || uref_kind >= 2); }
    int ref_mode = REF_ZERO;
    bool warm_start = true;
    bool cache_overridden = false;
    bool packs_dirty = true;
    bool state_bounds_active = false;
    const KernelEntry *ke = nullptr;
    const StreamEntry *se = nullptr;
    const ConeEntry *ce = nullptr;
    std::string kernel_name;
    const LeanEntry *le = nullptr;
    bool lean_jit = false;
    const LeanEntry *le_var[LV_COUNT] = {};
    bool le_var_tried[LV_COUNT] = {};
    double *d_lean = nullptr;
    bool lean_ok = false, lean_knot_bounds = false;
    bool lean_enabled = true;
    uint64_t lean_sp = 0;
    int last_lean_form = LF_NONE;
    int last_lean_cost[2] = {0, 0};
    std::string last_launch_name;
    unsigned char *d_coef = nullptr;
    float *d_bounds = nullptr;
    float *d_x0 = nullptr, *d_xref = nullptr, *d_uref = nullptr;
    size_t xref_cap = 0, uref_cap = 0;
    float *d_xout = nullptr, *d_uout = nullptr, *d_res = nullptr;
    int *d_iter = nullptr, *d_solved = nullptr;
    float *d_sd = nullptr, *d_sy = nullptr, *d_sz = nullptr, *d_sg = nullptr, *d_sv = nullptr;
    uint32_t *d_gstat = nullptr;
    uint32_t *d_gslot = nullptr;
    uint32_t *h_gstat = nullptr;
    float *h_stage = nullptr;
    size_t stage_cap = 0;
    hipStream_t s_copy = nullptr;
    hipEvent_t ev_copy[2] = {nullptr, nullptr};
    int d2h_double(const float *d, double *out, size_t n);
    std::vector<std::pair<void *, size_t>> pinned_ranges;
    int pin_host_range(void *p, size_t bytes);
    int unpin_host_range(void *p);
    int h2d_float(float *d, const double *in, size_t n);
    float *d_scratch = nullptr;
    double *d_ws64 = nullptr;
    size_t ws64_cap = 0;
    float *d_mpc_x = nullptr, *d_mpc_u = nullptr;
    int *d_mpc_iter = nullptr;
    int mpc_cap = 0, mpc_steps_last = 0;
    size_t scratch_cap = 0;
    bool solved_once = false;
    bool g_maybe_nonzero = false;
    bool profiling = false;
    static constexpr int EV_RING = 256;
    std::vector<hipEvent_t> ev_ring;
    long launches = 0;
    int precision = 0;

    int ex() const { return nx * N; }
    int eu() const { return nu * (N - 1); }

    ~Solver();
    int init(const double *A_, const double *B_, const double *Q_, const double *R_, double rho,
             int nx_, int nu_, int N_, int batch_, int device_, int verbose_);
    int init_families(const double *A_, const double *B_, const double *Q_, const double *R_, const double *rho_,
                      int nx_, int nu_, int N_, int batch_, int device_, int verbose_);
    int alloc_batch(int batch_);
    int copy_family_state(const Solver &o);
    hipEvent_t ev_done = nullptr, ev_wait = nullptr;
    bool ev_done_pending = false;
    int wait_last_launch();
    int select_kernel(bool rollout = false);
    Switches sw;
    bool strict_precision = false;
    bool strict_fp32() const { return precision != 0 && (sw.strict_fp32 || strict_precision); }
    bool extensions_active() const { return has_fdyn || cones_active() || lin_active(); }
    bool rollout_on_quad() const { return sw.mfma_oneshot_only || !warm_start; }
    const KernelEntry *route_quad(bool rollout) const;
    const KernelEntry *route_mfma(bool rollout, const KernelEntry *quad) const;
    const StreamEntry *route_stream() const;
    const StreamEntry *route_stream_f64() const;
    const ConeEntry *route_cone(bool rollout, bool have_quad, bool have_stream) const;
    const ConeEntry *route_trans(bool rollout, const ConeEntry *oneshot) const;
    std::vector<long> routing_key(bool rollout) const;
    bool bounds_vary_by_knot() const;
    std::vector<long> routed_key;
    bool routed = false;
    unsigned route_gen = 0;
    void free_batch();
    int upload_packs();
    int upload_refs();
    int set_x0(const double *x0, int cols);
    int set_ref(bool is_x, const double *ref, int cols);
    int set_ref_sequence(const double *x_seq, const double *u_seq, int steps);
    float *d_xref_seq = nullptr, *d_uref_seq = nullptr;
    int ref_seq_steps = 0;
    int set_bounds(const double *xmin, const double *xmax, const double *umin, const double *umax);
    int set_fdyn(const double *f);
    int set_cones(const int *Acu_, const int *qcu_, const double *cu_, int ncu_, const int *Acx_, const int *qcx_,
                  const double *cx_, int ncx_);
    int set_linear(const double *Ax, int mx, const double *bx, const double *Au, int mu, const double *bu);
    int ensure_extension_buffers();
    int reset();
    int solve_async(hipStream_t stream, int mpc_steps = 0);
    struct Pass {
        const int *idx = nullptr;
        int slots = 0, iter_offset = 0, iters = 0;
        bool cold = false, save = false;
        int mpc_steps = 0;
        const double *x0d = nullptr;
        const float *xref = nullptr, *uref = nullptr;
        bool loop = false;
        bool stream_loop = false;
    };
    Pass whole_batch(bool cold, bool save, int mpc_steps = 0) const;
    int launch_pass(hipStream_t stream, const Pass &);
    LeanPlan plan_lean(const Pass &) const;
    struct Pick {
        LeanPlan plan;
        const LeanEntry *lean = nullptr;
        bool stream_loop = false;
    };
    Pick pick_kernel(const Pass &);
    void fill_params(AdmmParams &P, const Pass &) const;
    int ensure_mpc_log(int mpc_steps);
    int record_done(hipStream_t stream, hipEvent_t carried = nullptr);
    int solve_chunked(hipStream_t stream);
    enum class Rollout { Refused, Fused, Chain, LeanLoop, StreamLoop };
    struct RolloutPlan {
        Rollout route = Rollout::Refused;
        bool stream_plant = false;
        bool own_plant = false;
    };
    RolloutPlan plan_rollout(int mpc_steps);
    int rollout_chain(hipStream_t stream, int mpc_steps, bool stream_plant);
    int rollout_chain_own(hipStream_t stream, int mpc_steps);
    int rollout_loop(hipStream_t stream, int mpc_steps, Rollout route);
    int stream_ext() const { return lin_active() ? 2 : ((has_fdyn || cones_active()) ? 1 : 0); }
    int last_rollout_launches = -1;
    double *d_plant = nullptr, *d_x0d = nullptr;
    double *d_plant_het = nullptr;
    bool plant_dirty = true;
    bool x0d_live = false;
    int plant_start(hipStream_t stream, bool resume);
    int ensure_plant();
    int plant_kind = 0, dist_kind = 0, dist_steps = 0;
    std::vector<double> own_A, own_B, own_f, dist_w;
    double *d_own_plant = nullptr, *d_dist = nullptr;
    bool own_plant_dirty = true;
    bool own_plant() const { return plant_kind != 0 || dist_kind != 0 || noisy(); }
    bool own_plant_per_instance() const { return plant_kind == 2 || (plant_kind == 0 && hetero); }
    int plant_mode() const { return plant_kind | (dist_kind == 1 ? 4 : (dist_kind == 2 ? 8 : 0)); }
    int set_plant(const double *A_, const double *B_, const double *f_, int per_instance);
    int set_disturbance(const double *w, int steps, int per_instance);
    void drop_own_plant();
    int ensure_own_plant();
    int noise_kind[2] = {0, 0};
    unsigned long long noise_seed[2] = {0, 0};
    int noise_cursor = 0;
    std::vector<double> noise_G[2];
    double *d_noise_G[2] = {nullptr, nullptr};
    float *d_mpc_y = nullptr;
    int mpc_y_cap = 0, mpc_y_steps = 0;
    bool noisy() const { return noise_kind[0] != 0 || noise_kind[1] != 0; }
    int noise_mode() const { return noise_kind[0] | (noise_kind[1] == 1 ? 4 : (noise_kind[1] == 2 ? 8 : 0)); }
    int set_noise(int which, const double *G, int per_instance, unsigned long long seed);
    void drop_noise();
    int get_noise(int which, int t0, int steps, double *buf);
    int get_mpc_measured(double *y);
    int traj_kind = 0, traj_Lx = 0, traj_Lu = 0;
    int ref_cursor = 0, traj_dev_cursor = -1;
    std::vector<float> h_xtraj, h_utraj;
    float *d_xtraj = nullptr, *d_utraj = nullptr;
    int set_ref_trajectory(const double *x_traj, int Lx, const double *u_traj, int Lu, int per_instance);
// ... 26 lines not shown
```

### tinympc-julia_amd/csrc/solver.hip

```cpp
#include "solver.h"
#include "admm_generic.hip.h"
#include "noise.h"

#include <climits>
#include <cmath>
#include <cstdio>
#include <cstdlib>
#include <algorithm>
#include <condition_variable>
#include <functional>
#include <mutex>
#include <cstring>
#include <thread>


namespace tmpc {

static thread_local std::string g_err;
void set_error(const std::string &msg) {
    g_err = msg;
    std::fprintf(stderr, "tinympc_hip: %s\n", msg.c_str());
}
const char *last_error() { return g_err.c_str(); }
bool hip_ok(hipError_t e, const char *what) {
// ... 176 lines not shown
    dev_free(d_xout);
    dev_free(d_uout);
    dev_free(d_res);
    dev_free(d_iter);
    dev_free(d_solved);
    dev_free(d_sd);
    dev_free(d_sy);
    dev_free(d_sz);
    dev_free(d_sg);
    dev_free(d_sv);
    dev_free(d_scratch);
    dev_free(d_ws64);
    ws64_cap = 0;
    dev_free(d_het_aux);
    dev_free(d_ibx);
    dev_free(d_ibu);
    dev_free(d_sgc);
    dev_free(d_svc);
    dev_free(d_syc);
    dev_free(d_szc);
    dev_free(d_idx[0]);
    dev_free(d_idx[1]);
    dev_free(d_count);
    dev_free(d_lin);
    dev_free(d_sgl);
    dev_free(d_svl);
    dev_free(d_syl);
    dev_free(d_szl);
    dev_free(d_adapt);
    dev_free(d_adp_cols);
    adp_cols_bytes = 0;
    dev_free(d_x0d);
    x0d_live = false;
    adapt_dirty = true;
    dev_free(d_mpc_x);
    dev_free(d_mpc_u);
    dev_free(d_mpc_iter);
    dev_free(d_mpc_y);
    mpc_y_steps = 0;
    dev_free(d_xref_seq);
    dev_free(d_uref_seq);
    ref_seq_steps = 0;
    mpc_cap = 0;
    xref_cap = uref_cap = scratch_cap = 0;
}

int Solver::init(const double *A_, const double *B_, const double *Q_, const double *R_, double rho,
                 int nx_, int nu_, int N_, int batch_, int device_, int verbose_) {
    if (nx_ < 1 || nu_ < 1 || N_ < 2 || batch_ < 1) {
        set_error("invalid dimensions (need nx >= 1, nu >= 1, N >= 2, batch >= 1)");
        return -1;
    }
    int ndev = 0;
    if (hipGetDeviceCount(&ndev) != hipSuccess || ndev < 1) {
        set_error("no HIP device available (this library has no CPU fallback)");
        return -1;
    }
    if (device_ < 0) HIP_TRY(hipGetDevice(&device_));
    device = device_;
    HIP_TRY(hipSetDevice(device));
    sw = read_switches();
    lean_enabled = !sw.no_lean;
    nx = nx_;
    nu = nu_;
    N = N_;
    verbose = verbose_;
    A = Mat(nx, nx, A_);
    B = Mat(nx, nu, B_);
    Q = Mat(nx, nx, Q_);
    R = Mat(nu, nu, R_);
    if (precompute_cache(A, B, Q, R, rho, cache) != 0) {
        set_error("Riccati precompute failed: R + B'PB is singular");
        return -1;
    }
    if (!no_specialise && !find_quad_kernel(nx, nu, N, -1) && !find_mfma_kernel(nx, nu, N) && !find_trans_kernel(nx, nu, N))
        (void)jit_kernel_for(nx, nu, N, verbose);
    if (verbose)
        std::printf("tinympc_hip: setup nx=%d nu=%d N=%d rho=%g batch=%d (Riccati %d sweeps)\n", nx, nu,
                    N, rho, batch_, cache.riccati_iters);
    fdyn.assign((size_t)nx, 0.0);
    x_min.assign((size_t)ex(), -1e17);
    x_max.assign((size_t)ex(), 1e17);
    u_min.assign((size_t)eu(), -1e17);
    u_max.assign((size_t)eu(), 1e17);
    batch = batch_;
    if (select_kernel()) return -1;
    if (dev_alloc(d_gstat, (size_t)2 * GSTAT_WORDS)) return -1;
    HIP_TRY(hipMemset(d_gstat, 0, 2 * GSTAT_WORDS * sizeof(uint32_t)));
    if (dev_alloc(d_gslot, (size_t)GSLOT_DEFAULT_CAP * GSLOT_WORDS)) return -1;
    HIP_TRY(hipHostMalloc((void **)&h_gstat, GSTAT_WORDS * sizeof(uint32_t), hipHostMallocDefault));
    std::memset(h_gstat, 0, GSTAT_WORDS * sizeof(uint32_t));
    packs_dirty = true;
    return alloc_batch(batch_);
}

int Solver::init_families(const double *A_, const double *B_, const double *Q_, const double *R_, const double *rho_,
                          int nx_, int nu_, int N_, int batch_, int device_, int verbose_) {
    no_specialise = true;
    if (init(A_, B_, Q_, R_, rho_[0], nx_, nu_, N_, batch_, device_, verbose_)) return -1;
    hetero = true;
    const size_t Bn = (size_t)batch, nxx = (size_t)nx * nx, nxu = (size_t)nx * nu, nuu = (size_t)nu * nu;
    het_A.assign(A_, A_ + Bn * nxx);
    het_B.assign(B_, B_ + Bn * nxu);
    het_cache.assign(Bn, Cache());
    std::vector<int> bad(1, 0);
    parallel_chunks(Bn, [&](size_t lo, size_t hi) {
        for (size_t b = lo; b < hi; ++b)
            if (precompute_cache(Mat(nx, nx, A_ + b * nxx), Mat(nx, nu, B_ + b * nxu), Mat(nx, nx, Q_ + b * nxx),
                                 Mat(nu, nu, R_ + b * nuu), rho_[b], het_cache[b]))
                bad[0] = 1;
    }, 64);
    if (bad[0]) {
        set_error("Riccati precompute failed for at least one instance (R + B'PB singular)");
        return -1;
    }
    std::vector<float> aux((size_t)(nx + nu + 1) * Bn);
    for (size_t b = 0; b < Bn; ++b) {
        for (int i = 0; i < nx; ++i) aux[(size_t)i * Bn + b] = (float)het_cache[b].Qd[i];
        for (int a = 0; a < nu; ++a) aux[(size_t)(nx + a) * Bn + b] = (float)het_cache[b].Rd[a];
        aux[(size_t)(nx + nu) * Bn + b] = (float)het_cache[b].rho;
    }
    if (dev_alloc(d_het_aux, aux.size())) return -1;
    HIP_TRY(hipMemcpy(d_het_aux, aux.data(), aux.size() * sizeof(float), hipMemcpyHostToDevice));
    packs_dirty = true;
    return select_kernel() || ensure_extension_buffers();
}

Switches read_switches() {
    auto on = [](const char *name) { return std::getenv(name) != nullptr; };
    Switches w;
    if (const char *g = std::getenv("TINYMPC_HIP_GROUP")) w.group = std::atoi(g);
    w.strict_fp32 = on("TINYMPC_HIP_STRICT_FP32");
    w.no_quad = on("TINYMPC_HIP_NO_QUAD");
    w.no_quad_adp = on("TINYMPC_HIP_NO_QUAD_ADP");
    w.no_quad_adp1 = on("TINYMPC_HIP_NO_QUAD_ADP1");
    w.no_mfma = on("TINYMPC_HIP_NO_MFMA");
    w.no_mfma_adp = on("TINYMPC_HIP_NO_MFMA_ADP");
    w.mfma_oneshot_only = on("TINYMPC_HIP_MFMA_ONESHOT_ONLY");
    w.no_stream = on("TINYMPC_HIP_NO_STREAM");
    w.no_stream_adp = on("TINYMPC_HIP_NO_STREAM_ADP");
    w.no_mfmar = on("TINYMPC_HIP_NO_MFMAR");
    w.no_mfmac = on("TINYMPC_HIP_NO_MFMAC");
    w.mfmac_all = on("TINYMPC_HIP_MFMAC_ALL");
    w.no_jit = on("TINYMPC_HIP_NO_JIT");
    w.no_mfmat = on("TINYMPC_HIP_NO_MFMAT");
    w.mfmat_all = on("TINYMPC_HIP_MFMAT_ALL");
    w.mfmat_ws_only = on("TINYMPC_HIP_MFMAT_WS_ONLY");
    w.no_lean = on("TINYMPC_HIP_NO_LEAN");
    w.no_refill = on("TINYMPC_HIP_NO_REFILL");
    w.no_uni = on("TINYMPC_HIP_NO_UNI");
    w.no_os = on("TINYMPC_HIP_NO_OS");
    w.lean_one = on("TINYMPC_HIP_LEAN_ONE");
    w.lean_dense = on("TINYMPC_HIP_LEAN_DENSE");
    w.lean_ws = on("TINYMPC_HIP_LEAN_WS");
    w.lean_loop = on("TINYMPC_HIP_LEAN_LOOP");
    w.stream_f64 = on("TINYMPC_HIP_STREAM_F64");
    w.stream_mpc = on("TINYMPC_HIP_STREAM_MPC");
    w.stream_loop = on("TINYMPC_HIP_STREAM_LOOP");
    w.event_markers = on("TINYMPC_HIP_EVENT_MARKERS");
    w.noise_split = on("TINYMPC_HIP_NOISE_SPLIT");
    if (const char *d = std::getenv("TINYMPC_HIP_MFMAC_DEBUG")) w.mfmac_debug = std::atoi(d);
    if (const char *f = std::getenv("TINYMPC_HIP_FOLD_SLOTS")) w.fold_slots = std::max(0, std::atoi(f));
    return w;
}


const KernelEntry *Solver::route_quad(bool rollout) const {
    if (sw.no_quad || extensions_active() || hetero || bounds_mode) return nullptr;
    if (!st.adaptive_rho) {
        const KernelEntry *k = sw.group ? find_quad_kernel(nx, nu, N, sw.group) : nullptr;
        if (!k) k = select_quad_kernel(nx, nu, N, batch);
        return (k && k->jit && (precision != 0 || sw.no_jit)) ? nullptr : k;
    }
    const KernelEntry *ka = sw.no_quad_adp ? nullptr : find_quad_kernel(nx, nu, N, 4);
    if (!(ka && ka->adp && chunk_iters == 0 && !rollout && !cache_overridden)) return nullptr;
    if (batch >= 20480 && precision == 0 && !sw.group && !refs_device_owned && xref_kind <= 1 && uref_kind <= 1 &&
        (adapt_pure || adapt_dirty) && !sw.no_quad_adp1)
        if (const KernelEntry *k1 = find_quad_kernel(nx, nu, N, 1))
            if (k1->adp) return k1;
    return ka;
}

const KernelEntry *Solver::route_mfma(bool rollout, const KernelEntry *quad) const {
    if (strict_fp32() || sw.group || sw.no_mfma || sw.no_quad || bounds_mode) return nullptr;
    const KernelEntry *m = find_mfma_kernel(nx, nu, N);
    if (!m || (m->jit && sw.no_jit)) return nullptr;
    if (st.adaptive_rho)
        return (!quad && m->adp && !extensions_active() && chunk_iters == 0 && !rollout && !cache_overridden &&
                (adapt_pure || adapt_dirty) && !sw.no_mfma_adp) ? m : nullptr;
    if (!(quad || !(extensions_active() || hetero))) return nullptr;
    if (rollout && rollout_on_quad()) return nullptr;
    if (!(!sw.mfma_oneshot_only || (!warm_start && chunk_iters == 0))) return nullptr;
    return m;
}

const StreamEntry *Solver::route_stream() const {
    const bool adp_ok = !extensions_active() && chunk_iters == 0 && !sw.no_stream_adp;
    if ((st.adaptive_rho && !adp_ok) || sw.no_stream) return nullptr;
    const StreamEntry *s2 = find_stream_kernel(nx, nu);
    if (s2 && 16.0 * batch * std::max(nx, nu) >= 4.0e9) s2 = nullptr;
    if (s2 && s2->lds_bytes(N, precision) > 150 * 1024) s2 = nullptr;
    if (s2 && bounds_mode && (precision != 0 || !s2->launch_ib)) s2 = nullptr;
    return s2;
}

const StreamEntry *Solver::route_stream_f64() const {
    if (!sw.stream_f64 || sw.no_stream || st.adaptive_rho || hetero || chunk_iters != 0 || bounds_mode) return nullptr;
    const StreamEntry *s2 = find_stream_kernel(nx, nu);
    if (!s2 || !s2->launch_f64) return nullptr;
    if (32.0 * batch * std::max(nx, nu) >= 4.0e9) return nullptr;
    if (s2->lds_bytes(N, 2) > 150 * 1024) return nullptr;
    return s2;
}

const ConeEntry *Solver::route_cone(bool rollout, bool have_quad, bool have_stream) const {
    if (bounds_mode) return nullptr;
    const ConeEntry *cn = sw.no_mfmar ? nullptr : find_cone_kernel(nx, nu, N);
    if (cn && cn->supports && !cn->supports(*this)) cn = nullptr;
    const bool plain_ok = sw.mfmac_all || (cn != nullptr && cn->plain);
    if (!((have_stream || (have_quad && plain_ok)) && !warm_start && chunk_iters == 0 && !rollout && !strict_fp32() && !hetero &&
          !st.adaptive_rho && (extensions_active() || plain_ok) && xref_kind < 2 && uref_kind < 2 &&
          !(refs_device_owned && ref_mode == REF_PER_INSTANCE) && !sw.no_mfmac && !sw.group && !sw.no_mfma))
        return nullptr;
    const ConeEntry *c2 = cn ? cn : find_cone_kernel(nx, nu, 0);
    if (c2 && c2->lds_bytes(*this) > 160 * 1024 - 1024) c2 = nullptr;
    if ((st.en_state_soc && ncx > 1) || (st.en_input_soc && ncu > 1) || lin_active()) c2 = nullptr;
    return c2;
}

const ConeEntry *Solver::route_trans(bool rollout, const ConeEntry *oneshot) const {
    if (sw.no_mfmat || sw.no_mfma || sw.group || bounds_mode) return nullptr;
    if (strict_fp32() || hetero || st.adaptive_rho || (rollout && refs_per_instance() && ref_seq_steps > 0) || st.max_iter < 1 || (double)batch * ex() >= 2.0e9)
        return nullptr;
    const ConeEntry *ct = find_trans_kernel(nx, nu, N);
    if (ct && (lin_active() || (ct->supports && !ct->supports(*this)))) ct = nullptr;
    if (ct && !(has_fdyn || cones_active() || ct->plain || sw.mfmat_all)) return nullptr;
    if (!ct && extensions_active() && !sw.no_jit) {
        ct = jit_trans_find(*this);
        if (!ct && !no_specialise && layout_final) ct = jit_trans_for(*this, verbose);
    }
    if (!ct || ct->lds_bytes(*this) > 160 * 1024 - 1024) return nullptr;
    if (sw.mfmat_ws_only && !warm_start && chunk_iters == 0 && !rollout && oneshot) return nullptr;
    return ct;
}

bool Solver::bounds_vary_by_knot() const {
    if (st.en_state_bound)
        for (int k = 1; k < N; ++k)
            for (int r = 0; r < nx; ++r)
                if (x_min[r + (size_t)k * nx] != x_min[r] || x_max[r + (size_t)k * nx] != x_max[r]) return true;
    if (st.en_input_bound)
        for (int k = 1; k < N - 1; ++k)
            for (int a = 0; a < nu; ++a)
                if (u_min[a + (size_t)k * nu] != u_min[a] || u_max[a + (size_t)k * nu] != u_max[a]) return true;
    return false;
}

std::vector<long> Solver::routing_key(bool rollout) const {
    return {nx, nu, N, batch, precision, warm_start, chunk_iters, has_fdyn, cones_active(), lin_active(), hetero, st.adaptive_rho,
            cache_overridden, refs_device_owned, xref_kind, uref_kind, ref_mode, adapt_pure, adapt_dirty, ref_seq_steps,
            st.max_iter < 1, st.en_state_soc, st.en_input_soc, ncx, ncu, Acx[0], qcx[0], Acu[0], qcu[0], mlx, mlu, rollout, strict_precision,
            (long)route_gen, Acx[1], qcx[1], Acu[1], qcu[1], st.en_state_linear, st.en_input_linear,
            extensions_active() && bounds_vary_by_knot(), layout_final, bounds_mode};
}

int Solver::select_kernel(bool rollout) {
    std::vector<long> key = routing_key(rollout);
    if (routed && key == routed_key) return 0;
    if (st.adaptive_rho && hetero) {
        set_error("adaptive_rho is not available on a per-instance-family solver");
        return -1;
    }
    if (st.adaptive_rho && bounds_mode) {
        set_error("adaptive_rho is not available with per-instance bounds (set_instance_bounds); shared bounds (set_bound_constraints) drop them");
        return -1;
    }
    if (precision == 2) {
        if (hetero || (rollout && !sw.stream_mpc)) {
            set_error(hetero ? "precision 2 is not available on a per-instance-family solver" : "precision 2 has no fused closed loop (step it from the host)");
            return -1;
        }
        if (nx > GEN_MAX_NX || nu > GEN_MAX_NU) {
            set_error("problem shape exceeds the generic kernel limits (nx <= 64, nu <= 32)");
            return -1;
        }
        const StreamEntry *s2 = route_stream_f64();
        if (ke || ce || s2 != se) packs_dirty = true;
        ke = nullptr, se = s2, ce = nullptr;
        kernel_name = se ? se->name_f64 : (bounds_mode ? "generic<f64;ib>" : "generic<f64>");
        routed_key = std::move(key);
        routed = true;
        return 0;
    }
    const KernelEntry *q = route_quad(rollout), *m = route_mfma(rollout, q), *k = m ? m : q;
    if (!k && (nx > GEN_MAX_NX || nu > GEN_MAX_NU)) {
        set_error("problem shape exceeds the generic kernel limits (nx <= 64, nu <= 32)");
        return -1;
    }
    const StreamEntry *s2 = k ? nullptr : route_stream();
    if (hetero && !s2) {
        set_error(bounds_mode ? "per-instance families with per-instance bounds need the stream kernel's ib form: (nx, nu) in {(4,1), (6,3), (12,4)}, precision 0" :
                  "per-instance families need a stream-kernel instantiation for (nx, nu) (nx in {2,3,4,6,8,10,12}, nu <= 4)");
        return -1;
    }
    const ConeEntry *c2 = route_cone(rollout, k != nullptr, s2 != nullptr), *ct = route_trans(rollout, c2);
    if (ct) c2 = ct;
// ... 2 lines not shown
    ke = k, se = s2, ce = c2;
    kernel_name = ke ? ke->name : (se ? (bounds_mode ? se->name_ib : se->name) : (ce ? ce->name : (bounds_mode ? "generic<ib>" : "generic")));
    routed_key = std::move(key);
    routed = true;
    return 0;
}

int Solver::alloc_batch(int batch_) {
    if (hetero && batch_ != batch) {
        set_error("set_batch_size: a per-instance-family solver has a fixed batch");
        return -1;
    }
    if (batch_ < 1) {
        set_error("batch must be >= 1");
        return -1;
    }
    HIP_TRY(hipSetDevice(device));
    free_batch();
    drop_instance_bounds();
    drop_own_plant();
    (void)drop_ref_trajectory(false);
    drop_noise();
    batch = batch_;
    if (select_kernel()) return -1;
    const size_t Bn = (size_t)batch, EX = (size_t)ex(), EU = (size_t)eu();
    if (dev_alloc(d_x0, Bn * nx) || dev_alloc(d_xout, Bn * EX) || dev_alloc(d_uout, Bn * EU) ||
        dev_alloc(d_res, Bn * 4) || dev_alloc(d_iter, Bn) || dev_alloc(d_solved, Bn) ||
        dev_alloc(d_sd, Bn * EU) || dev_alloc(d_sy, Bn * EU) || dev_alloc(d_sz, Bn * EU) ||
        dev_alloc(d_sg, Bn * EX) || dev_alloc(d_sv, Bn * EX))
        return -1;
    if (dev_alloc(d_xref, EX) || dev_alloc(d_uref, EU)) return -1;
    xref_cap = EX;
    uref_cap = EU;
    HIP_TRY(hipMemset(d_x0, 0, Bn * nx * sizeof(float)));
    HIP_TRY(hipMemset(d_xout, 0, Bn * EX * sizeof(float)));
    HIP_TRY(hipMemset(d_uout, 0, Bn * EU * sizeof(float)));
    HIP_TRY(hipMemset(d_iter, 0, Bn * sizeof(int)));
    HIP_TRY(hipMemset(d_solved, 0, Bn * sizeof(int)));
    HIP_TRY(hipMemset(d_xref, 0, EX * sizeof(float)));
    HIP_TRY(hipMemset(d_uref, 0, EU * sizeof(float)));
    h_xref.clear();
    h_uref.clear();
    xref_kind = uref_kind = 0;
    ref_mode = REF_ZERO;
    refs_dirty = false;
    refs_device_owned = false;
    if (ensure_extension_buffers()) return -1;
    solved_once = false;
    return reset();
}

int Solver::reset() {
    HIP_TRY(hipSetDevice(device));
    if (wait_last_launch()) return -1;
    const size_t Bn = (size_t)batch, EX = (size_t)ex(), EU = (size_t)eu();
    HIP_TRY(hipMemset(d_sd, 0, Bn * EU * sizeof(float)));
    HIP_TRY(hipMemset(d_sy, 0, Bn * EU * sizeof(float)));
    HIP_TRY(hipMemset(d_sz, 0, Bn * EU * sizeof(float)));
    HIP_TRY(hipMemset(d_sg, 0, Bn * EX * sizeof(float)));
    HIP_TRY(hipMemset(d_sv, 0, Bn * EX * sizeof(float)));
    HIP_TRY(hipMemset(d_res, 0, Bn * 4 * sizeof(float)));
    if (d_sgc) {
        HIP_TRY(hipMemset(d_sgc, 0, Bn * EX * sizeof(float)));
        HIP_TRY(hipMemset(d_svc, 0, Bn * EX * sizeof(float)));
        HIP_TRY(hipMemset(d_syc, 0, Bn * EU * sizeof(float)));
        HIP_TRY(hipMemset(d_szc, 0, Bn * EU * sizeof(float)));
    }
    if (d_sgl) {
        HIP_TRY(hipMemset(d_sgl, 0, Bn * EX * sizeof(float)));
        HIP_TRY(hipMemset(d_svl, 0, Bn * EX * sizeof(float)));
        HIP_TRY(hipMemset(d_syl, 0, Bn * EU * sizeof(float)));
        HIP_TRY(hipMemset(d_szl, 0, Bn * EU * sizeof(float)));
    }
    if (d_ws64) HIP_TRY(hipMemset(d_ws64, 0, ws64_cap * sizeof(double)));
    adapt_dirty = true;
    g_maybe_nonzero = false;
    return 0;
}

__global__ void adapt_fill_kernel(double *adapt, const double *family, int n, long batch) {
    const long i = (long)blockIdx.x * blockDim.x + threadIdx.x;
    if (i < (long)n * batch) adapt[i] = family[i / batch];
}

int Solver::set_sensitivity(const double *dK, const double *dP) {
    sens.assign((size_t)nu * nx + (size_t)nx * nx, 0.0);
    std::copy(dK, dK + (size_t)nu * nx, sens.begin());
    std::copy(dP, dP + (size_t)nx * nx, sens.begin() + (size_t)nu * nx);
    if (d_adapt && !adapt_dirty && sens_set) adapt_pure = false;
    sens_set = true;
    sens_dirty = true;
    packs_dirty = true;
    return 0;
}

int Solver::get_adaptive_state(double *rho, double *Kinf, double *Pinf) {
    HIP_TRY(hipSetDevice(device));
    if (wait_last_launch()) return -1;
    const size_t Bn = (size_t)batch, nk = (size_t)nu * nx, np = (size_t)nx * nx;
    if (!d_adapt || adapt_dirty) {
        for (size_t b = 0; b < Bn; ++b) {
            if (rho) rho[b] = cache.rho;
            if (Kinf) std::copy(cache.Kinf.a.begin(), cache.Kinf.a.end(), Kinf + b * nk);
            if (Pinf) std::copy(cache.Pinf.a.begin(), cache.Pinf.a.end(), Pinf + b * np);
        }
        return 0;
    }
    std::vector<double> h((1 + nk + np) * Bn);
    HIP_TRY(hipMemcpy(h.data(), d_adapt, h.size() * sizeof(double), hipMemcpyDeviceToHost));
    for (size_t b = 0; b < Bn; ++b) {
        if (rho) rho[b] = h[b];
        if (Kinf)
            for (size_t e = 0; e < nk; ++e) Kinf[b * nk + e] = h[(1 + e) * Bn + b];
        if (Pinf)
            for (size_t e = 0; e < np; ++e) Pinf[b * np + e] = h[(1 + nk + e) * Bn + b];
    }
    return 0;
}

int Solver::upload_packs() {
    if (wait_last_launch()) return -1;
    state_bounds_active = false;
    const std::vector<double> &sxmin = bounds_mode ? ib_xmin : x_min, &sxmax = bounds_mode ? ib_xmax : x_max;
    if (st.en_state_bound)
        for (size_t i = 0; i < sxmin.size(); ++i)
            if (sxmin[i] > -1e17 || sxmax[i] < 1e17) {
                state_bounds_active = true;
                break;
            }
    if (bounds_mode && upload_instance_bounds()) return -1;
    std::vector<unsigned char> coef;
    std::vector<float> bnd;
    if (ke) {
        ke->build_coef(*this, coef);
        ke->build_bounds(*this, bnd);
    } else if (ce) {
        ce->build_coef(*this, coef);
        ce->build_bounds(*this, bnd);
    } else if (se) {
        se->build_coef(*this, coef);
        se->build_bounds(*this, bnd);
    } else {
        build_generic_coef(*this, coef);
        build_generic_bounds(*this, bnd);
    }
    if (dev_alloc(d_coef, coef.size()) || dev_alloc(d_bounds, bnd.size())) return -1;
    HIP_TRY(hipMemcpy(d_coef, coef.data(), coef.size(), hipMemcpyHostToDevice));
    HIP_TRY(hipMemcpy(d_bounds, bnd.data(), bnd.size() * sizeof(float), hipMemcpyHostToDevice));
    le = (ke && ke->G == 1 && lean_enabled) ? find_lean_kernel(nx, nu, N) : nullptr;
    lean_jit = !le && ke && lean_enabled && !sw.no_jit && !no_specialise && (ke->G == 1 || (ke->jit && ke->G < 16 && batch >= 20480));
    if (precision == 2 && !ke && !ce && !hetero && !extensions_active() && lean_enabled && !sw.no_jit && !no_specialise && !bounds_mode) lean_jit = true;
    std::fill(le_var_tried, le_var_tried + LV_COUNT, false);
    lean_ok = false;
    lean_sp = lean_pattern(A, B);
    if (le || lean_jit) {
        std::vector<double> lp;
        if (build_lean_pack(*this, lp)) {
            if (!le && (!ke || ke->G != 1)) append_lean_bounds(*this, lp);
            if (dev_alloc(d_lean, lp.size())) return -1;
            HIP_TRY(hipMemcpy(d_lean, lp.data(), lp.size() * sizeof(double), hipMemcpyHostToDevice));
            lean_ok = true;
            lean_knot_bounds = false;
            if (st.en_input_bound)
                for (int k = 1; k < N - 1 && !lean_knot_bounds; ++k)
                    for (int a = 0; a < nu; ++a)
                        if (u_min[a + (size_t)k * nu] != u_min[a] || u_max[a + (size_t)k * nu] != u_max[a]) lean_knot_bounds = true;
        }
    }
    packs_dirty = false;
    return 0;
}

int Solver::set_x0(const double *x0, int cols) {
    if (cols != 1 && cols != batch) {
        set_error("set_x0: expected nx x 1 or nx x batch");
        return -1;
    }
    HIP_TRY(hipSetDevice(device));
    if (wait_last_launch()) return -1;
    std::vector<float> h((size_t)batch * nx);
    for (int b = 0; b < batch; ++b)
        for (int i = 0; i < nx; ++i) h[(size_t)b * nx + i] = (float)x0[(cols == 1 ? 0 : (size_t)b * nx) + i];
    HIP_TRY(hipMemcpy(d_x0, h.data(), h.size() * sizeof(float), hipMemcpyHostToDevice));
    return 0;
}

int Solver::set_ref(bool is_x, const double *ref, int cols) {
    const int kn = is_x ? N : N - 1;
    const int rows = is_x ? nx : nu;
    int kind;
    if (cols == kn)
        kind = 1;
    else if ((long)cols == (long)kn * batch)
        kind = 2;
    else {
        set_error(is_x ? "set_x_ref: expected nx x N or nx x (N*batch)"
                       : "set_u_ref: expected nu x (N-1) or nu x ((N-1)*batch)");
        return -1;
    }
    if (traj_kind && drop_ref_trajectory(true)) return -1;
    std::vector<float> &h = is_x ? h_xref : h_uref;
    const size_t n = (size_t)rows * cols;
    h.resize(n);
    bool all_zero = true;
    for (size_t i = 0; i < n; ++i) {
        h[i] = (float)ref[i];
        all_zero = all_zero && (ref[i] == 0.0);
    }
    if (all_zero) {
        kind = 0;
        h.clear();
    }
    (is_x ? xref_kind : uref_kind) = kind;
    if (kind != 2) ref_seq_steps = 0;
    refs_dirty = true;
    refs_device_owned = false;
    return 0;
}

int Solver::set_ref_sequence(const double *x_seq, const double *u_seq, int steps) {
    if (steps <= 0) {
        ref_seq_steps = 0;
        return 0;
    }
    if (!x_seq || !u_seq) {
        set_error("set_ref_sequence: null reference sequence");
        return -1;
    }
    HIP_TRY(hipSetDevice(device));
    if (wait_last_launch()) return -1;
    if (traj_kind && drop_ref_trajectory(false)) return -1;
    const size_t EX = (size_t)ex(), EU = (size_t)eu();
    std::vector<float> hx(EX * steps), hu(EU * steps);
    for (size_t i = 0; i < hx.size(); ++i) hx[i] = (float)x_seq[i];
    for (size_t i = 0; i < hu.size(); ++i) hu[i] = (float)u_seq[i];
    if (dev_alloc(d_xref_seq, hx.size()) || dev_alloc(d_uref_seq, hu.size())) return -1;
    HIP_TRY(hipMemcpy(d_xref_seq, hx.data(), hx.size() * sizeof(float), hipMemcpyHostToDevice));
    HIP_TRY(hipMemcpy(d_uref_seq, hu.data(), hu.size() * sizeof(float), hipMemcpyHostToDevice));
    h_xref.assign(hx.begin(), hx.begin() + EX);
    h_uref.assign(hu.begin(), hu.begin() + EU);
    xref_kind = uref_kind = 1;
    refs_dirty = true;
    refs_device_owned = false;
    ref_seq_steps = steps;
    return 0;
}

int Solver::upload_refs() {
    if (refs_device_owned || !refs_dirty) return 0;
    HIP_TRY(hipSetDevice(device));
    if (wait_last_launch()) return -1;
    const int mode = xref_kind > uref_kind ? xref_kind : uref_kind;
    const size_t EX = (size_t)ex(), EU = (size_t)eu(), Bn = (size_t)batch;
    auto put = [&](float *&dptr, size_t &cap, const std::vector<float> &h, int kind, size_t E) -> int {
        const size_t need = mode == REF_PER_INSTANCE ? Bn * E : E;
        if (cap < need) {
            if (dev_alloc(dptr, need)) return -1;
            cap = need;
        }
        if (mode == REF_ZERO) return 0;
        std::vector<float> tmp;
        const float *src;
        if (kind == mode) {
            src = h.data();
        } else {
            tmp.assign(need, 0.f);
            if (kind == 1)
                for (size_t b = 0; b < Bn; ++b) std::memcpy(tmp.data() + b * E, h.data(), E * sizeof(float));
            src = tmp.data();
        }
        HIP_TRY(hipMemcpy(dptr, src, need * sizeof(float), hipMemcpyHostToDevice));
        return 0;
    };
    if (put(d_xref, xref_cap, h_xref, xref_kind, EX)) return -1;
    if (put(d_uref, uref_cap, h_uref, uref_kind, EU)) return -1;
    ref_mode = mode;
    refs_dirty = false;
    return 0;
}

int Solver::set_bounds(const double *xmin, const double *xmax, const double *umin, const double *umax) {
    route_gen += 1;
    const bool had_instance_bounds = bounds_mode != 0;
    drop_instance_bounds();
    x_min.assign(xmin, xmin + ex());
    x_max.assign(xmax, xmax + ex());
    u_min.assign(umin, umin + eu());
    u_max.assign(umax, umax + eu());
    st.en_state_bound = 1;
    st.en_input_bound = 1;
    packs_dirty = true;
    return had_instance_bounds ? (select_kernel() || ensure_extension_buffers()) : 0;
}

int Solver::set_instance_bounds(const double *xmin, const double *xmax, const double *umin, const double *umax, int per_knot) {
    if (!xmin || !xmax || !umin || !umax) {
        set_error("set_instance_bounds: null bound array");
        return -1;
    }
    if (st.adaptive_rho) {
        set_error("set_instance_bounds: per-instance bounds are not available with adaptive rho");
        return -1;
    }
    if (wait_last_launch()) return -1;
    const int old_mode = bounds_mode;
    const size_t Bn = (size_t)batch, nxe = per_knot ? (size_t)ex() * Bn : (size_t)nx * Bn, nue = per_knot ? (size_t)eu() * Bn : (size_t)nu * Bn;
    route_gen += 1;
    bounds_mode = per_knot ? 2 : 1;
    ib_xmin.assign(xmin, xmin + nxe);
    ib_xmax.assign(xmax, xmax + nxe);
// ... 359 lines not shown
        if (dev_alloc(d_idx[0], (size_t)batch) || dev_alloc(d_idx[1], (size_t)batch) || dev_alloc(d_count, 1)) return -1;
    }
    uint32_t acc[GSTAT_WORDS] = {0};
    const int *idx = nullptr;
    int n = batch, offset = 0, cur = 0;
    for (;;) {
        const int iters = std::min(chunk, st.max_iter - offset);
        Pass chunk_pass;
        chunk_pass.idx = idx, chunk_pass.slots = n, chunk_pass.iter_offset = offset, chunk_pass.iters = iters;
        chunk_pass.cold = offset == 0 && !warm_start, chunk_pass.save = true;
        if (launch_pass(stream, chunk_pass)) return -1;
        offset += iters;
        HIP_TRY(hipMemcpyAsync(h_gstat, d_gstat, GSTAT_WORDS * sizeof(uint32_t), hipMemcpyDeviceToHost, stream));
        const bool last = offset >= st.max_iter;
        int count = 0;
        if (!last) {
            HIP_TRY(hipMemsetAsync(d_count, 0, sizeof(int), stream));
            hipLaunchKernelGGL(compact_unsolved_kernel, dim3((n + 255) / 256), dim3(256), 0, stream, d_solved, idx, n,
                               d_idx[cur], d_count);
            HIP_TRY(hipGetLastError());
            HIP_TRY(hipMemcpyAsync(&count, d_count, sizeof(int), hipMemcpyDeviceToHost, stream));
        }
        HIP_TRY(hipStreamSynchronize(stream));
        acc[4] = h_gstat[4];
        if (last || count == 0) {
            if (count == 0 && !last) acc[4] = 0;
            break;
        }
        idx = d_idx[cur];
        n = count;
        cur ^= 1;
    }
    HIP_TRY(hipMemcpyAsync(d_gstat, acc, GSTAT_WORDS * sizeof(uint32_t), hipMemcpyHostToDevice, stream));
    hipLaunchKernelGGL(residual_max_kernel, dim3((unsigned)std::min<long>(1024, ((long)batch + 255) / 256)), dim3(256), 0,
                       stream, d_res, (long)batch, d_gstat);
    HIP_TRY(hipGetLastError());
    HIP_TRY(hipStreamSynchronize(stream));
    return 0;
}

Solver::Pass Solver::whole_batch(bool cold, bool save, int mpc_steps) const {
    Pass a;
    a.slots = batch, a.iters = st.max_iter, a.cold = cold, a.save = save, a.mpc_steps = mpc_steps;
    return a;
}

LeanPlan Solver::plan_lean(const Pass &a) const {
    LeanPlanIn in;
    in.nx = nx, in.nu = nu, in.N = N;
    in.builtin = le != nullptr, in.kinds = le ? le->kinds : 0, in.builtin_sp = le ? le->sp : 0;
    in.lean_jit = lean_jit, in.lean_ok = lean_ok, in.model_sp = lean_sp, in.knot_bounds = lean_knot_bounds;
    in.quad_G = ke ? ke->G : 0, in.precision = precision;
    in.sw_one = sw.lean_one, in.sw_dense = sw.lean_dense, in.sw_ws = sw.lean_ws, in.sw_loop = sw.lean_loop;
    in.slots = a.slots, in.iters = a.iters, in.mpc_steps = a.mpc_steps;
    in.cold = a.cold, in.save = a.save, in.indexed = a.idx != nullptr, in.adaptive_rho = st.adaptive_rho != 0;
    in.ref_mode = ref_mode, in.loop = a.loop;
    in.state_bounds = state_bounds_active, in.g_maybe_nonzero = g_maybe_nonzero;
    in.live = st.abs_pri_tol > 0.0 && st.abs_dua_tol > 0.0;
    in.stream_ext = se && extensions_active();
    in.cus = device_cu_count();
    return lean_plan(in);
}

void Solver::fill_params(AdmmParams &P, const Pass &a) const {
    std::memset(&P, 0, sizeof(P));
    P.coef = reinterpret_cast<const float *>(d_coef);
    P.bounds = d_bounds;
    P.x0 = d_x0;
    P.x0d = a.x0d;
    P.xref = a.xref ? a.xref : d_xref;
    P.uref = a.uref ? a.uref : d_uref;
    P.xout = d_xout;
    P.uout = d_uout;
    P.iter = d_iter;
    P.solved = d_solved;
    P.res = d_res;
    P.sd = d_sd;
    P.sy = d_sy;
    P.sz = d_sz;
    P.sg = d_sg;
    P.sv = d_sv;
    P.gstat = d_gstat;
    P.gacc = d_gstat + GSTAT_WORDS;
    P.gslot_cap = sw.fold_slots < 0 ? (int)GSLOT_DEFAULT_CAP : std::min(sw.fold_slots, (int)GSLOT_DEFAULT_CAP);
    P.gslot = P.gslot_cap > 0 ? d_gslot : nullptr;
    P.scratch = d_scratch;
    P.idx = a.idx;
    P.iter_offset = a.iter_offset;
    P.batch = a.slots;
    P.max_iter = a.iters;
    P.check_termination = st.check_termination;
    P.ref_mode = ref_mode;
    P.cold_start = a.cold ? 1 : 0;
    P.save_state = a.save ? 1 : 0;
    P.abs_pri_tol = (float)st.abs_pri_tol;
    P.abs_dua_tol = (float)st.abs_dua_tol;
    P.rho = (float)cache.rho;
    P.nx = nx;
    P.nu = nu;
    P.N = N;
    P.mpc_steps = a.mpc_steps;
    P.mpc_x = d_mpc_x;
    P.mpc_u = d_mpc_u;
    P.mpc_iter = d_mpc_iter;
    P.x0_out = d_x0;
    P.xb_active = state_bounds_active ? 1 : 0;
    P.has_fdyn = has_fdyn ? 1 : 0;
    P.ncx = st.en_state_soc ? ncx : 0;
    P.ncu = st.en_input_soc ? ncu : 0;
    for (int i = 0; i < 8; ++i) {
        P.Acx[i] = Acx[i];
        P.qcx[i] = qcx[i];
        P.cx[i] = (float)cx[i];
        P.Acu[i] = Acu[i];
        P.qcu[i] = qcu[i];
        P.cu[i] = (float)cu[i];
    }
    P.het_aux = d_het_aux;
    P.adaptive_rho = st.adaptive_rho;
    P.rho_clip = st.adaptive_rho_clip;
    P.rho_family = cache.rho;
    P.rho_min = (float)st.adaptive_rho_min;
    P.rho_max = (float)st.adaptive_rho_max;
    P.sens = d_sens;
    P.adapt = d_adapt;
    P.adapt_stride = batch;
    P.adp_cols = d_adp_cols;
    P.sgc = d_sgc;
    P.svc = d_svc;
    P.syc = d_syc;
    P.szc = d_szc;
    P.mlx = st.en_state_linear ? mlx : 0;
    P.mlu = st.en_input_linear ? mlu : 0;
    P.lin = d_lin;
    P.sgl = d_sgl;
    P.svl = d_svl;
    P.syl = d_syl;
    P.szl = d_szl;
    P.bounds_stride = (ce && ce->bounds_vary(*this)) ? 1 : 0;
    if (a.mpc_steps > 0 && ref_seq_steps > 0) {
        P.xref_seq = d_xref_seq;
        P.uref_seq = d_uref_seq;
    }
    P.lean = d_lean;
    P.ws64 = d_ws64;
    P.abs_pri_tol64 = st.abs_pri_tol;
    P.abs_dua_tol64 = st.abs_dua_tol;
    if (bounds_mode) {
        P.ibx = d_ibx, P.ibu = d_ibu;
        P.ib_kx = bounds_mode == 2 ? (long)batch * nx : 0, P.ib_ku = bounds_mode == 2 ? (long)batch * nu : 0;
        P.ib_hx = (long)batch * nx * (bounds_mode == 2 ? N : 1), P.ib_hu = (long)batch * nu * (bounds_mode == 2 ? N - 1 : 1);
        P.ib_on = (st.en_state_bound ? IB_STATE : 0) | (st.en_input_bound ? IB_INPUT : 0);
    }
    P.host_flags = (sw.no_refill ? HF_NO_REFILL : 0) | (sw.no_uni ? HF_NO_UNI : 0) | (sw.no_os ? HF_NO_OS : 0);
}

int Solver::ensure_mpc_log(int mpc_steps) {
    if (mpc_cap < mpc_steps) {
        const size_t n = (size_t)batch * mpc_steps;
        if (dev_alloc(d_mpc_x, n * nx) || dev_alloc(d_mpc_u, n * nu) || dev_alloc(d_mpc_iter, n)) return -1;
        mpc_cap = mpc_steps;
    }
    return 0;
}

int Solver::record_done(hipStream_t stream, hipEvent_t carried) {
    if (carried) {
        ev_wait = carried;
    } else {
        if (!ev_done) HIP_TRY(hipEventCreateWithFlags(&ev_done, hipEventDisableTiming));
        HIP_TRY(hipEventRecord(ev_done, stream));
        ev_wait = ev_done;
    }
    ev_done_pending = true;
    return 0;
}

Solver::Pick Solver::pick_kernel(const Pass &a) {
    Pick k;
    k.plan = plan_lean(a);
    k.lean = k.plan.take ? le : nullptr;
    if (k.plan.take && !le) {
        const int v = k.plan.variant;
        if (!le_var_tried[v]) le_var[v] = jit_lean_for(nx, nu, N, v, k.plan.form == LF_SPARSE ? k.plan.sp : 0, verbose), le_var_tried[v] = true;
        k.lean = le_var[v];
    }
    k.stream_loop = a.stream_loop && !k.lean && se && !bounds_mode && se->launch_mpc && se->has_mpc(precision, stream_ext(), hetero);
    return k;
}

int Solver::launch_pass(hipStream_t stream, const Pass &a) {
    if (packs_dirty && upload_packs()) return -1;
    if (upload_refs()) return -1;
    if (a.mpc_steps > 0 && ref_seq_steps > 0 && ke && ke->N > QUAD_REF_SEQ_MAX_N) {
        set_error("mpc_rollout: the lanes-per-instance kernels take a reference sequence at horizons up to " +
                  std::to_string((int)QUAD_REF_SEQ_MAX_N) + " (this entry: " + ke->name + "); step the loop from the host");
        return -1;
    }
    AdmmParams P;
    fill_params(P, a);
    if (!ke && !se && !ce) HIP_TRY(hipMemsetAsync(d_gstat, 0, GSTAT_WORDS * sizeof(uint32_t), stream));
    hipEvent_t ev0 = nullptr, ev1 = nullptr;
    if (profiling) {
        if (ev_ring.empty()) {
            ev_ring.assign(2 * EV_RING, nullptr);
            for (hipEvent_t &e : ev_ring) HIP_TRY(hipEventCreate(&e));
        }
        ev0 = ev_ring[2 * (launches % EV_RING)];
        ev1 = ev_ring[2 * (launches % EV_RING) + 1];
    }
    if (state_bounds_active && a.save) g_maybe_nonzero = true;
    const bool carry_g = state_bounds_active || (ke && ke->G == 16 && g_maybe_nonzero);
    const Pick pick = pick_kernel(a);
    const LeanPlan &plan = pick.plan;
    const LeanEntry *lk = pick.lean;
    const bool lean = lk != nullptr, sloop = pick.stream_loop;
    if (lean && !le && (!ke || ke->G != 1)) P.bounds = reinterpret_cast<const float *>(d_lean + lean_layout(nx, nu).total);
    const bool attached = profiling && lean && !sw.event_markers;
    if (profiling && !attached) HIP_TRY(hipEventRecord(ev0, stream));
    if (lean)
        HIP_TRY(lk->launch(P, plan.variant, stream, attached ? ev0 : nullptr, attached ? ev1 : nullptr));
    else
        HIP_TRY(ke ? ke->launch(P, precision, carry_g, stream)
                   : (ce ? ce->launch(P, cones_active(), ce->lds_bytes(*this), stream)
                         : (se ? (sloop ? se->launch_mpc(P, precision, stream_ext(), hetero, stream)
                                        : (precision == 2 ? se->launch_f64(P, stream_ext(), stream)
                                                          : (bounds_mode ? se->launch_ib(P, stream_ext(), hetero, stream)
                                                                         : se->launch(P, precision, stream_ext(), hetero, stream))))
                               : launch_generic(P, precision, stream))));
    if (profiling) {
        if (!attached) HIP_TRY(hipEventRecord(ev1, stream));
        launches += 1;
    }
    last_launch_name = lean ? lk->name : kernel_name;
    last_lean_form = lean ? plan.form : LF_NONE;
    last_lean_cost[0] = lean ? plan.cost_sparse : 0;
    last_lean_cost[1] = lean ? plan.cost_dense : 0;
    solved_once = true;
    return record_done(stream, attached ? ev1 : nullptr);
}

__global__ void plant_init_kernel(double *x0d, const float *x0, long n) {
    const long i = (long)blockIdx.x * blockDim.x + threadIdx.x;
    if (i < n) x0d[i] = (double)x0[i];
}

__global__ void plant_resume_kernel(double *x0d, const float *x0, long n) {
    const long i = (long)blockIdx.x * blockDim.x + threadIdx.x;
    if (i < n && (float)x0d[i] != x0[i]) x0d[i] = (double)x0[i];
}

int Solver::plant_start(hipStream_t stream, bool resume) {
    if (!d_x0d && dev_alloc(d_x0d, (size_t)batch * nx)) return -1;
    const long n0 = (long)batch * nx;
    (resume && x0d_live ? plant_resume_kernel : plant_init_kernel)<<<(unsigned)((n0 + 255) / 256), 256, 0, stream>>>(d_x0d, d_x0, n0);
    HIP_TRY(hipGetLastError());
    if (resume) x0d_live = true;
    return 0;
}

__global__ void plant_step_kernel(double *x0d, float *x0, const float *uout, const int *iter, const int *solved,
                                  const double *AB, float *mpc_x, float *mpc_u, int *mpc_iter, int nx, int nu, int N,
                                  long batch, int steps, int step) {
    const long b = (long)blockIdx.x * blockDim.x + threadIdx.x;
    if (b >= batch) return;
    const double *A = AB, *Bm = AB + nx * nx;
    const float *u0 = uout + b * (long)nu * (N - 1);
    const long so = b * steps + step;
    double xn[GEN_MAX_NX];
    for (int r = 0; r < nx; ++r) {
        double acc = 0.0;
        for (int j = 0; j < nx; ++j) acc = fma(A[r + j * nx], x0d[b * nx + j], acc);
        for (int a = 0; a < nu; ++a) acc = fma(Bm[r + a * nx], (double)u0[a], acc);
        xn[r] = acc;
    }
    for (int r = 0; r < nx; ++r) {
        x0d[b * nx + r] = xn[r];
        x0[b * nx + r] = (float)xn[r];
        mpc_x[so * nx + r] = (float)xn[r];
    }
    for (int a = 0; a < nu; ++a) mpc_u[so * nu + a] = u0[a];
    mpc_iter[so] = solved[b] ? iter[b] : -iter[b];
}

__global__ void plant_step_affine_kernel(double *x0d, float *x0, const float *uout, const int *iter, const int *solved,
                                         const double *AB, const double *ABb, float *mpc_x, float *mpc_u, int *mpc_iter, int nx,
                                         int nu, int N, long batch, int steps, int step) {
    const int per_block = (int)blockDim.x / nx, t = (int)threadIdx.x, r = t % nx;
    const long b = (long)blockIdx.x * per_block + t / nx;
    const bool on = t < per_block * nx && b < batch;
    double acc = 0.0;
    if (on) {
        const double *A = ABb ? ABb + b * (long)(nx * nx + nx * nu) : AB, *Bm = A + nx * nx;
        const float *u0 = uout + b * (long)nu * (N - 1);
        acc = AB[nx * nx + nx * nu + r];
        for (int j = 0; j < nx; ++j) acc = fma(A[r + j * nx], x0d[b * nx + j], acc);
        for (int a = 0; a < nu; ++a) acc = fma(Bm[r + a * nx], (double)u0[a], acc);
    }
    __syncthreads();
    if (!on) return;
    const long so = b * steps + step;
    x0d[b * nx + r] = acc;
    x0[b * nx + r] = (float)acc;
    mpc_x[so * nx + r] = (float)acc;
    for (int a = r; a < nu; a += nx) mpc_u[so * nu + a] = uout[b * (long)nu * (N - 1) + a];
    if (r == 0) mpc_iter[so] = solved[b] ? iter[b] : -iter[b];
}

int Solver::ensure_plant() {
    const size_t nab = (size_t)nx * nx + (size_t)nx * nu;
    if (d_plant && !plant_dirty) return 0;
    if (wait_last_launch()) return -1;
    if (!d_plant && dev_alloc(d_plant, nab + nx)) return -1;
    std::vector<double> ab(A.a);
    ab.insert(ab.end(), B.a.begin(), B.a.end());
    for (int r = 0; r < nx; ++r) ab.push_back(has_fdyn ? fdyn[r] : 0.0);
    HIP_TRY(hipMemcpy(d_plant, ab.data(), ab.size() * sizeof(double), hipMemcpyHostToDevice));
    if (hetero && !d_plant_het) {
        std::vector<double> abb((size_t)batch * nab);
        for (size_t b = 0; b < (size_t)batch; ++b) {
            std::copy(het_A.begin() + b * nx * nx, het_A.begin() + (b + 1) * nx * nx, abb.begin() + b * nab);
            std::copy(het_B.begin() + b * nx * nu, het_B.begin() + (b + 1) * nx * nu, abb.begin() + b * nab + (size_t)nx * nx);
        }
        if (dev_alloc(d_plant_het, abb.size())) return -1;
        HIP_TRY(hipMemcpy(d_plant_het, abb.data(), abb.size() * sizeof(double), hipMemcpyHostToDevice));
    }
    plant_dirty = false;
    return 0;
}

int Solver::rollout_chain(hipStream_t stream, int mpc_steps, bool stream_plant) {
    if (ensure_plant() || plant_start(stream, stream_plant)) return -1;
    const size_t EX = (size_t)ex(), EU = (size_t)eu(), per_block = 256 / nx;
    Pass pass = whole_batch(false, true);
    pass.x0d = stream_plant ? nullptr : d_x0d;
    for (int step = 0; step < mpc_steps; ++step) {
        if (ref_seq_steps > 0 && step > 0) pass.xref = d_xref_seq + step * EX, pass.uref = d_uref_seq + step * EU;
        if (launch_pass(stream, pass)) return -1;
        if (stream_plant)
            plant_step_affine_kernel<<<(unsigned)((batch + per_block - 1) / per_block), 256, 0, stream>>>(
                d_x0d, d_x0, d_uout, d_iter, d_solved, d_plant, hetero ? d_plant_het : nullptr, d_mpc_x, d_mpc_u, d_mpc_iter, nx, nu, N, (long)batch,
                mpc_steps, step);
        else
            plant_step_kernel<<<(unsigned)((batch + 255) / 256), 256, 0, stream>>>(d_x0d, d_x0, d_uout, d_iter, d_solved, d_plant, d_mpc_x, d_mpc_u,
                                                                               d_mpc_iter, nx, nu, N, (long)batch, mpc_steps, step);
    }
    HIP_TRY(hipGetLastError());
    return record_done(stream);
}

__global__ void plant_step_own_kernel(double *x0d, float *x0, const float *uout, const int *iter, const int *solved,
                                      const double *plant, long plant_stride, const double *w, long w_stride, float *mpc_x,
                                      float *mpc_u, int *mpc_iter, int nx, int nu, int N, long batch, int steps, int step) {
    const int per_block = (int)blockDim.x / nx, t = (int)threadIdx.x, r = t % nx;
    const long b = (long)blockIdx.x * per_block + t / nx;
    const bool on = t < per_block * nx && b < batch;
    double acc = 0.0;
    if (on) {
        const double *A = plant + b * plant_stride, *Bm = A + nx * nx;
        const float *u0 = uout + b * (long)nu * (N - 1);
        acc = Bm[nx * nu + r];
        for (int j = 0; j < nx; ++j) acc = fma(A[r + j * nx], x0d[b * nx + j], acc);
        for (int a = 0; a < nu; ++a) acc = fma(Bm[r + a * nx], (double)u0[a], acc);
        if (w) acc = acc + w[b * w_stride + r];
    }
    __syncthreads();
    if (!on) return;
    const long so = b * steps + step;
    x0d[b * nx + r] = acc;
    x0[b * nx + r] = (float)acc;
    mpc_x[so * nx + r] = (float)acc;
    for (int a = r; a < nu; a += nx) mpc_u[so * nu + a] = uout[b * (long)nu * (N - 1) + a];
    if (r == 0) mpc_iter[so] = solved[b] ? iter[b] : -iter[b];
}

int Solver::set_plant(const double *A_, const double *B_, const double *f_, int per_instance) {
    if (!A_ && !B_) {
        if (plant_kind && wait_last_launch()) return -1;
        plant_kind = 0;
        own_A.clear(), own_B.clear(), own_f.clear();
        own_plant_dirty = true;
        if (!own_plant()) dev_free(d_own_plant);
        return 0;
    }
    if (!A_ || !B_) {
        set_error("set_plant: expected both A (nx x nx) and B (nx x nu), or neither to drop the plant");
        return -1;
    }
// ... 406 lines not shown
}

double Solver::kernel_elapsed_ms() { return kernel_elapsed_mean_ms(1); }

double Solver::kernel_elapsed_mean_ms(int last_n) {
    if (!profiling || ev_ring.empty() || launches == 0 || last_n <= 0) return -1.0;
    const long n = std::min<long>(std::min<long>(last_n, EV_RING), launches);
    double sum = 0.0;
    for (long i = launches - n; i < launches; ++i) {
        float ms = -1.f;
        if (hipEventElapsedTime(&ms, ev_ring[2 * (i % EV_RING)], ev_ring[2 * (i % EV_RING) + 1]) != hipSuccess) return -1.0;
        sum += ms;
    }
    return sum / (double)n;
}

int Solver::get_traj(bool states, double *buf) {
    HIP_TRY(hipSetDevice(device));
    if (wait_last_launch()) return -1;
    return d2h_double(states ? d_xout : d_uout, buf, (size_t)batch * (states ? ex() : eu()));
}

int Solver::get_status(int *iter, int *solved, double *res4) {
    HIP_TRY(hipSetDevice(device));
    if (wait_last_launch()) return -1;
    const size_t Bn = (size_t)batch;
    if (iter) HIP_TRY(hipMemcpy(iter, d_iter, Bn * sizeof(int), hipMemcpyDeviceToHost));
    if (solved) HIP_TRY(hipMemcpy(solved, d_solved, Bn * sizeof(int), hipMemcpyDeviceToHost));
    if (res4) {
        std::vector<float> h(Bn * 4);
        HIP_TRY(hipMemcpy(h.data(), d_res, Bn * 4 * sizeof(float), hipMemcpyDeviceToHost));
        for (size_t i = 0; i < Bn * 4; ++i) res4[i] = (double)h[i];
    }
    return 0;
}

int Solver::d2h_double(const float *d, double *out, size_t n) {
    if (!out || n == 0) return 0;
    constexpr size_t CHUNK = (size_t)1 << 21;
    if (!s_copy) {
        HIP_TRY(hipStreamCreate(&s_copy));
        for (hipEvent_t &e : ev_copy) HIP_TRY(hipEventCreateWithFlags(&e, hipEventDisableTiming));
    }
    if (stage_cap < 2 * CHUNK) {
        if (h_stage) (void)hipHostFree(h_stage);
        h_stage = nullptr;
        HIP_TRY(hipHostMalloc((void **)&h_stage, 2 * CHUNK * sizeof(float), hipHostMallocDefault));
        stage_cap = 2 * CHUNK;
    }
    const size_t nchunks = (n + CHUNK - 1) / CHUNK;
    for (size_t c = 0; c <= nchunks; ++c) {
        if (c < nchunks) {
            const size_t off = c * CHUNK, len = std::min(CHUNK, n - off);
            HIP_TRY(hipMemcpyAsync(h_stage + (c & 1) * CHUNK, d + off, len * sizeof(float), hipMemcpyDeviceToHost, s_copy));
            HIP_TRY(hipEventRecord(ev_copy[c & 1], s_copy));
        }
        if (c > 0) {
            const size_t pc = c - 1, off = pc * CHUNK, len = std::min(CHUNK, n - off);
            HIP_TRY(hipEventSynchronize(ev_copy[pc & 1]));
            widen(h_stage + (pc & 1) * CHUNK, out + off, len);
        }
    }
    return 0;
}
int Solver::pin_host_range(void *p, size_t bytes) {
    if (!p || bytes == 0) {
        set_error("pin_host: null or empty range");
        return -1;
    }
    for (const auto &r : pinned_ranges)
        if (r.first == p) {
            if (r.second >= bytes) return 0;
            set_error("pin_host: this address is already pinned with a smaller size; unpin it first");
            return -1;
        }
    HIP_TRY(hipSetDevice(device));
    HIP_TRY(hipHostRegister(p, bytes, hipHostRegisterDefault));
    pinned_ranges.emplace_back(p, bytes);
    return 0;
}
int Solver::unpin_host_range(void *p) {
    for (size_t i = 0; i < pinned_ranges.size(); ++i)
        if (pinned_ranges[i].first == p) {
            HIP_TRY(hipSetDevice(device));
            if (wait_last_launch()) return -1;
            pinned_ranges.erase(pinned_ranges.begin() + i);
            HIP_TRY(hipHostUnregister(p));
            return 0;
        }
    set_error("unpin_host: this address was not pinned through this solver");
    return -1;
}

int Solver::h2d_float(float *d, const double *in, size_t n) {
    if (!in) return 0;
    std::vector<float> h(n);
    narrow(in, h.data(), n);
    HIP_TRY(hipMemcpy(d, h.data(), n * sizeof(float), hipMemcpyHostToDevice));
    return 0;
}

int Solver::get_workspace(double *d, double *y, double *g, double *v, double *z) {
    HIP_TRY(hipSetDevice(device));
    if (wait_last_launch()) return -1;
    const size_t Bn = (size_t)batch, EX = (size_t)ex(), EU = (size_t)eu();
    if (precision == 2 && d_ws64) {
        const Ws64 w(d_ws64, (long)Bn, (long)EX, (long)EU);
        auto get = [&](double *dst, const double *src, size_t n) { return !dst || hipMemcpy(dst, src, n * sizeof(double), hipMemcpyDeviceToHost) == hipSuccess; };
        if (!(get(d, w.sd, Bn * EU) && get(y, w.sy, Bn * EU) && get(z, w.sz, Bn * EU) && get(g, w.sg, Bn * EX) && get(v, w.sv, Bn * EX))) {
            set_error("get_workspace: copy failed");
            return -1;
        }
        return 0;
    }
    if (d2h_double(d_sd, d, Bn * EU) || d2h_double(d_sy, y, Bn * EU) || d2h_double(d_sz, z, Bn * EU) ||
        d2h_double(d_sg, g, Bn * EX) || d2h_double(d_sv, v, Bn * EX))
        return -1;
    return 0;
}

int Solver::set_workspace(const double *d, const double *y, const double *g, const double *v,
                          const double *z) {
    HIP_TRY(hipSetDevice(device));
    if (wait_last_launch()) return -1;
    const size_t Bn = (size_t)batch, EX = (size_t)ex(), EU = (size_t)eu();
    if (precision == 2) {
        if (select_kernel() || ensure_extension_buffers()) return -1;
        const Ws64 w(d_ws64, (long)Bn, (long)EX, (long)EU);
        auto put = [&](double *dst, const double *src, size_t n) { return !src || hipMemcpy(dst, src, n * sizeof(double), hipMemcpyHostToDevice) == hipSuccess; };
        if (!(put(w.sd, d, Bn * EU) && put(w.sy, y, Bn * EU) && put(w.sz, z, Bn * EU) && put(w.sg, g, Bn * EX) && put(w.sv, v, Bn * EX))) {
            set_error("set_workspace: copy failed");
            return -1;
        }
        return 0;
    }
    if (h2d_float(d_sd, d, Bn * EU) || h2d_float(d_sy, y, Bn * EU) || h2d_float(d_sz, z, Bn * EU) ||
        h2d_float(d_sg, g, Bn * EX) || h2d_float(d_sv, v, Bn * EX))
        return -1;
    g_maybe_nonzero = true;
    return 0;
}

}

extern "C" int tmpc_lean_last_form(tinympc_solver *s, unsigned long long *pattern, int *cost_sparse, int *cost_dense, int *form) {
    if (!s) return 1;
    if (pattern) *pattern = s->s.lean_sp;
    if (cost_sparse) *cost_sparse = s->s.last_lean_cost[0];
    if (cost_dense) *cost_dense = s->s.last_lean_cost[1];
    if (form) *form = s->s.last_lean_form;
    return 0;
}

extern "C" int tmpc_last_rollout_launches(tinympc_solver *s) { return s ? s->s.last_rollout_launches : -1; }
```

Baseline: 559.0 million.

## Add diagonally scaled sparse lean kernel turning dynamics coefficients into unit entries

Adds a state-scaling transform chosen on the host, which picks a diagonal similarity so that selected off-diagonal A entries and one B entry become exactly one. This lets the sparse lean kernel replace those multiply-adds with plain adds in the forward rollout and the backward pass. The kernel scales x0 on entry, unscales states on store, and rescales the dual residual per component. The cost is extra per-component residual bookkeeping and scale loads, plus possible rounding differences from the change of coordinates.

```diff
diff --git a/tinympc-julia_amd/csrc/admm_lean.hip.h b/tinympc-julia_amd/csrc/admm_lean.hip.h
--- a/tinympc-julia_amd/csrc/admm_lean.hip.h
+++ b/tinympc-julia_amd/csrc/admm_lean.hip.h
@@ -31,6 +31,7 @@
     static constexpr LeanLayout LL = lean_layout(NX, NU);
     static constexpr int O_M = LL.oM, O_K = LL.oK, O_B = LL.oB, O_C = LL.oC, O_H = LL.oH, O_S = LL.oS, O_P = LL.oP, O_T = LL.oT, LEN = LL.len;
     static constexpr int NLOADS = LL.padded / 8;
+    static constexpr int O_Z = LL.oZ, O_W = LL.oW, O_SC = LL.oSc, O_SI = LL.oSi, NLOADS_Z = LL.padZ / 8;
 };
 
 typedef float lean_f2 __attribute__((ext_vector_type(2)));
@@ -57,6 +58,9 @@
     using L = LeanPack<NX, NU>;
     constexpr int EX = NX * N, EU = NU * (N - 1);
     constexpr bool SPR = SP != 0;
+    constexpr bool SCL = lsp_scaled(SP);
+    static_assert(!SCL || (!XB && !WS && !F64 && REFS == REF_ZERO), "scaled pattern: one-shot, no state bound, zero references, fp32 state");
+    static_assert(!SCL || L::NLOADS_Z <= 4, "scaled coefficient block too large for SGPRs");
     static_assert(!SPR || (NX <= 4 && NU <= 4), "sparse pattern: nx, nu <= 4");
     constexpr bool HB = !SPR && !LIVE && !XB && ONE;
     constexpr bool PK = TMPC_LEAN_PK && ONE && !LIVE && !XB && !WS && UBK && !F64;
@@ -65,6 +69,7 @@
     auto a_nz = [](int m, int j) { return !SPR || lsp_a(SP, NX, m, j); };
     auto a_one = [](int m, int j) { return SPR && lsp_one(SP, NX, m, j); };
     auto b_nz = [](int m, int a) { return !SPR || lsp_b(SP, NU, m, a); };
+    auto b_one = [](int m, int a) { return SCL && lsp_b_one(SP, NU, m, a); };
     constexpr int BW = 2 * NX + 2 * NU;
     static_assert(L::NLOADS <= 4, "coefficient block too large for SGPRs");
 
@@ -134,8 +139,9 @@
     __shared__ __attribute__((aligned(16))) float s_pv[PARK ? 256 * PVS : 4];
     __shared__ float s_pz[PARK ? 256 * PZS : 1];
 
-    const SBlock<double, L::NLOADS> blk(P.lean + (HB ? L::O_H : (SPR ? L::O_S : 0)));
+    const SBlock<double, (SCL ? L::NLOADS_Z : L::NLOADS)> blk(P.lean + (HB ? L::O_H : (SCL ? L::O_Z : (SPR ? L::O_S : 0))));
     const auto cM = blk.at(L::O_M), cK = blk.at(L::O_K), cB = blk.at(L::O_B), cC = blk.at(L::O_C);
+    const auto cW = blk.at(SCL ? L::O_W : 0);
 
     ST lo[NU], hi[NU];
 #pragma unroll
@@ -150,6 +156,7 @@
     for (int m = 0; m < NX; ++m) {
         if constexpr (WS) X[0][m] = !active ? 0.0 : (P.x0d ? P.x0d[b * NX + m] : (double)P.x0[b * NX + m]);
         else X[0][m] = active ? (double)P.x0[b * NX + m] : 0.0;
+        if constexpr (SCL) X[0][m] *= P.lean[L::O_SC + m];
     }
     if constexpr (HB) {
         double x0[NX];
@@ -232,6 +239,7 @@
     const ST rho = F64 ? (ST)P.rho_family : (ST)P.rho;
     const ST ptol = F64 ? (ST)P.abs_pri_tol64 : (ST)P.abs_pri_tol, dtol = F64 ? (ST)P.abs_dua_tol64 : (ST)P.abs_dua_tol;
     double dua_x = 0.0;
+    double dua_xs[SCL ? NX : 1] = {};
     ST pri_u = 0, dua_u = 0, pri_xf = 0, dua_xf = 0;
     auto park_v = [&](int k, const float (&pv)[NX]) {
         float *row = s_pv + tid * PVS + k * NX;
@@ -286,6 +294,9 @@
         constexpr bool RES = decltype(res_tag)::value;
         if constexpr (RES) {
             dua_x = 0.0, pri_u = 0, dua_u = 0, pri_xf = 0, dua_xf = 0;
+            if constexpr (SCL)
+#pragma unroll
+                for (int m = 0; m < NX; ++m) dua_xs[m] = 0.0;
             if constexpr (WS && !XB) {
                 float v0p[NX];
 #pragma unroll
@@ -329,13 +340,15 @@
                             double Tm[NX * NX];
                             load_T(Tm);
                             dua_x = fmax(dua_x, fabs(to_x(Tm, X[0], m)));
+                        } else if constexpr (SCL) {
+                            dua_xs[m] = fabs(X[0][m]);
                         } else {
                             dua_x = fmax(dua_x, fabs(X[0][m]));
                         }
                     }
                 }
         }
-        if constexpr (HB || (SPR && (ONE || XB)))
+        if constexpr (HB || (SPR && (ONE || XB) && !(SCL && ONE)))
 #pragma unroll
             for (int m = 0; m < NX; ++m) asm volatile("" : "+v"(X[0][m]));
         double xr[NX];
@@ -372,9 +385,15 @@
                         started[m] = true;
                     }
             }
+            constexpr bool K0H = SCL && ONE && k == 0;
 #pragma unroll
             for (int a = 0; a < NU; ++a) {
-                if constexpr (SPR) {
+                if constexpr (K0H) {
+                    double acc = -(cK[a * NX] * xk[0]);
+#pragma unroll
+                    for (int j = 1; j < NX; ++j) acc = fma(-cK[a * NX + j], xk[j], acc);
+                    u[a] = acc - dk[a];
+                } else if constexpr (SPR) {
                     double acc = -dk[a];
 #pragma unroll
                     for (int pass = 0; pass < 2; ++pass)
@@ -403,13 +422,17 @@
             if constexpr (SPR) {
 #pragma unroll
                 for (int m = 0; m < NX; ++m) {
-                    int s = -1;
+                    int s = -1, sb = -1;
 #pragma unroll
                     for (int j = NX - 1; j >= 0; --j)
                         if (a_one(m, j)) s = j;
-                    started[m] = s >= 0;
+#pragma unroll
+                    for (int a = NU - 1; a >= 0; --a)
+                        if (s < 0 && b_one(m, a) && !K0H) sb = a;
+                    started[m] = s >= 0 || sb >= 0;
                     xn[m] = 0.0;
                     if (s >= 0) xn[m] = xk[s];
+                    else if (sb >= 0) xn[m] = u[sb];
 #pragma unroll
                     for (int j = 0; j < NX; ++j) {
                         if (!a_nz(m, j) || j == s) continue;
@@ -418,8 +441,8 @@
                     }
 #pragma unroll
                     for (int a = 0; a < NU; ++a) {
-                        if (!b_nz(m, a)) continue;
-                        xn[m] = started[m] ? fma(cB[m * NU + a], u[a], xn[m]) : cB[m * NU + a] * u[a];
+                        if (!b_nz(m, a) || a == sb) continue;
+                        xn[m] = !started[m] ? cB[m * NU + a] * u[a] : (b_one(m, a) ? xn[m] + u[a] : fma(cB[m * NU + a], u[a], xn[m]));
                         started[m] = true;
                     }
                 }
@@ -476,7 +499,8 @@
                 if constexpr (XB) {
                     xr[m] = xn[m];
                 } else {
-                    if constexpr (RES && !HB) dua_x = fmax(dua_x, fabs(X[k + 1][m] - xn[m]));
+                    if constexpr (RES && SCL) dua_xs[m] = fmax(dua_xs[m], fabs(X[k + 1][m] - xn[m]));
+                    else if constexpr (RES && !HB) dua_x = fmax(dua_x, fabs(X[k + 1][m] - xn[m]));
                     if constexpr (!(RES && HB)) X[k + 1][m] = xn[m];
                 }
             }
@@ -489,8 +513,16 @@
                 for (int m = 0; m < NX; ++m) dua_x = fmax(dua_x, fabs(to_x(Tm, dl, m)));
             }
             if constexpr (RES) asm volatile("" : "+v"(pri_u), "+v"(dua_u), "+v"(dua_x), "+v"(pri_xf), "+v"(dua_xf));
+            if constexpr (RES && SCL)
+#pragma unroll
+                for (int m = 0; m < NX; ++m) asm volatile("" : "+v"(dua_xs[m]));
             if constexpr (TMPC_LEAN_KNOT_BARRIER) __builtin_amdgcn_sched_barrier(0);
         });
+        if constexpr (RES && SCL) {
+#pragma unroll
+            for (int m = 0; m < NX; ++m) dua_x = fmax(dua_x, dua_xs[m] * fabs(P.lean[L::O_SI + m]));
+            asm volatile("" : "+v"(dua_x));
+        }
         if constexpr (XB) {
             asm volatile("" ::: "memory");
             state_sets(res_tag, std::integral_constant<int, N - 1>{}, xr);
@@ -504,6 +536,7 @@
 #pragma unroll
         for (int m = 0; m < NX; ++m) {
             p[m] = XB ? (double)QT[N - 1][m] : X[XB ? 0 : N - 1][m];
+            if constexpr (SCL) p[m] *= cW[m];
             if constexpr (REFS == REF_SHARED) p[m] += s_cpt[m];
         }
         float rpk[PK ? NU : 1];
@@ -528,7 +561,7 @@
             for (int j = 0; j < NX; ++j)
 #pragma unroll
                 for (int a = 0; a < NU; ++a)
-                    if (!bh_zero(j, a) && b_nz(j, a)) t[a] = fma(cB[j * NU + a], p[j], t[a]);
+                    if (!bh_zero(j, a) && b_nz(j, a)) t[a] = b_one(j, a) ? t[a] + p[j] : fma(cB[j * NU + a], p[j], t[a]);
 #pragma unroll
             for (int a = 0; a < NU; ++a) {
                 double acc = cC[a * NU] * t[0];
@@ -542,9 +575,16 @@
                 for (int m = 0; m < NX; ++m) {
                     double acc = XB ? (double)QT[k][m] : X[XB ? 0 : k][m];
                     if constexpr (REFS == REF_SHARED) acc += s_cq[k * NX + m];
+                    int ju = -1;
+                    if constexpr (SCL) {
+#pragma unroll
+                        for (int j = NX - 1; j >= 0; --j)
+                            if (a_one(j, m)) ju = j;
+                        acc = ju >= 0 ? fma(cW[m], acc, p[ju]) : cW[m] * acc;
+                    }
 #pragma unroll
                     for (int j = 0; j < NX; ++j)
-                        if (a_nz(j, m)) acc = a_one(j, m) ? acc + p[j] : fma(cM[j * NX + m], p[j], acc);
+                        if (a_nz(j, m) && j != ju) acc = a_one(j, m) ? acc + p[j] : fma(cM[j * NX + m], p[j], acc);
 #pragma unroll
                     for (int a = 0; a < NU; ++a) acc = fma(-cK[a * NX + m], t[a], acc);
                     ap[m] = acc;
@@ -574,15 +614,24 @@
     };
 
     double Ts[HB ? NX * NX : 1];
+    double Si[SCL ? NX : 1];
+    auto load_Si = [&]() {
+        const double *sp = P.lean + L::O_SI;
+        asm volatile("" : "+s"(sp));
+#pragma unroll
+        for (int m = 0; m < (SCL ? NX : 0); ++m) Si[m] = sp[m];
+    };
     auto vnew_at = [&](auto kk, auto mm) -> float {
         constexpr int k = decltype(kk)::value, m = decltype(mm)::value;
         if constexpr (XB) return (float)clamp3(QT[k][m] + G[k][m], (ST)s_xb[k * 2 * NX + m], (ST)s_xb[k * 2 * NX + NX + m]);
         else if constexpr (HB) return (float)to_x(Ts, X[k], m);
+        else if constexpr (SCL) return (float)(X[k][m] * Si[m]);
         else return (float)X[XB ? 0 : k][m];
     };
     auto store = [&](bool solved_flag) {
         float *xo = P.xout + b * EX, *uo = P.uout + b * EU, *ro = P.res + b * 4;
         asm volatile("" : "+v"(xo), "+v"(uo), "+v"(ro));
+        if constexpr (SCL) load_Si();
         sfor<0, N>([&](auto kk) {
             constexpr int k = decltype(kk)::value;
             sfor<0, NX>([&](auto mm) { xo[k * NX + decltype(mm)::value] = vnew_at(kk, mm); });
@@ -853,6 +902,7 @@
         const unsigned long long mask = __builtin_amdgcn_ballot_w64(mine);
         if (mask) {
             if constexpr (HB) load_T(Ts);
+            if constexpr (SCL) load_Si();
             if constexpr (WS) {
                 store_ws(mask, mine, std::false_type{});
             } else {
diff --git a/tinympc-julia_amd/csrc/admm_params.h b/tinympc-julia_amd/csrc/admm_params.h
--- a/tinympc-julia_amd/csrc/admm_params.h
+++ b/tinympc-julia_amd/csrc/admm_params.h
@@ -79,7 +79,7 @@
     int ib_on;
 };
 enum : int { IB_STATE = 1, IB_INPUT = 2 };
-enum : int { HF_NO_REFILL = 1, HF_NO_UNI = 2, HF_NO_OS = 4 };
+enum : int { HF_NO_REFILL = 1, HF_NO_UNI = 2, HF_NO_OS = 4, HF_LEAN_SCALED = 8 };
 
 struct LeanLayout {
     int oM;
@@ -93,14 +93,13 @@
     int oP;
     int oT;
     int total;
+    int oZ, oW, padZ, oSc, oSi;
 };
 constexpr LeanLayout lean_layout(int nx, int nu) {
-    return LeanLayout{0, nx * nx, nx * nx + nu * nx, nx * nx + 2 * nu * nx, nx * nx + 2 * nu * nx + nu * nu,
-                      (nx * nx + 2 * nu * nx + nu * nu + 7) / 8 * 8, (nx * nx + 2 * nu * nx + nu * nu + 7) / 8 * 8,
-                      2 * ((nx * nx + 2 * nu * nx + nu * nu + 7) / 8 * 8),
-                      3 * ((nx * nx + 2 * nu * nx + nu * nu + 7) / 8 * 8),
-                      3 * ((nx * nx + 2 * nu * nx + nu * nu + 7) / 8 * 8) + nx * nx,
-                      3 * ((nx * nx + 2 * nu * nx + nu * nu + 7) / 8 * 8) + 2 * nx * nx};
+    const int len = nx * nx + 2 * nu * nx + nu * nu, pad = (len + 7) / 8 * 8, padz = (len + nx + 7) / 8 * 8;
+    const int old_total = 3 * pad + 2 * nx * nx, oz = (old_total + 7) / 8 * 8;
+    return LeanLayout{0, nx * nx, nx * nx + nu * nx, nx * nx + 2 * nu * nx, len, pad, pad, 2 * pad, 3 * pad, 3 * pad + nx * nx,
+                      oz + padz + 2 * nx, oz, len, padz, oz + padz, oz + padz + nx};
 }
 
 enum : int { LSP_UNIT = 16, LSP_B = 32, LSP_ON = 48 };
@@ -144,6 +143,62 @@
 constexpr bool lean_pattern_covers(uint64_t built, uint64_t model) {
     const uint64_t nz = 0xFFFFull | (0xFFFFull << LSP_B), one = 0xFFFFull << LSP_UNIT;
     return built != 0 && model != 0 && (model & nz & ~built) == 0 && ((built & one) & ~(model & one)) == 0;
+}
+
+enum : int { LSP_SCALED = 49, LSP_BU = 50, LSP_BU_ON = 54 };
+constexpr bool lsp_scaled(uint64_t sp) { return (sp >> LSP_SCALED) & 1; }
+constexpr bool lsp_b_one(uint64_t sp, int nu, int i, int a) {
+    return ((sp >> LSP_BU_ON) & 1) && (int)((sp >> LSP_BU) & 15) == i * nu + a;
+}
+constexpr int lean_cost_scaled(uint64_t sp, int nx, int nu) {
+    int c = nx * nu + nu * nu;
+    for (int i = 0; i < nx; ++i) {
+        int row = 0, col = 1 + nu;
+        bool ru = false, cu = false;
+        for (int j = 0; j < nx; ++j) {
+            row += lsp_a(sp, nx, i, j), ru = ru || lsp_one(sp, nx, i, j);
+            col += lsp_a(sp, nx, j, i), cu = cu || lsp_one(sp, nx, j, i);
+        }
+        for (int a = 0; a < nu; ++a) {
+            row += lsp_b(sp, nu, i, a), ru = ru || lsp_b_one(sp, nu, i, a);
+            c += lsp_b(sp, nu, i, a);
+        }
+        c += row - (ru && row > 0 ? 1 : 0) + col - (cu ? 1 : 0);
+    }
+    return c;
+}
+constexpr uint64_t lean_pattern_scaled(uint64_t sp, int nx, int nu) {
+    if (sp == 0 || lsp_scaled(sp) || nx < 1 || nu < 1 || nx > 4 || nu > 4) return 0;
+    uint64_t base = (sp & (0xFFFFull | (0xFFFFull << LSP_B))) | (1ull << LSP_ON) | (1ull << LSP_SCALED);
+    uint32_t cand = 0;
+    for (int i = 0; i < nx; ++i)
+        for (int j = 0; j < nx; ++j) {
+            if (i == j && lsp_one(sp, nx, i, i)) base |= 1ull << (LSP_UNIT + i * nx + i);
+            if (i != j && lsp_a(sp, nx, i, j)) cand |= 1u << (i * nx + j);
+        }
+    uint64_t best = 0;
+    int best_cost = 0, best_units = 0;
+    for (uint32_t m = 0, done = 0; !done; done = (m == cand), m = (m - cand) & cand) {
+        int comp[4] = {0, 1, 2, 3};
+        bool ok = true;
+        for (int e = 0; e < nx * nx && ok; ++e) {
+            if (!((m >> e) & 1)) continue;
+            const int ci = comp[e / nx], cj = comp[e % nx];
+            if (ci == cj) ok = false;
+            for (int q = 0; q < nx; ++q)
+                if (comp[q] == cj) comp[q] = ci;
+        }
+        for (int b = -1; ok && b < nx * nu; ++b) {
+            if (b >= 0 && !((sp >> (LSP_B + b)) & 1)) continue;
+            uint64_t s = base | ((uint64_t)m << LSP_UNIT);
+            if (b >= 0) s |= (1ull << LSP_BU_ON) | ((uint64_t)b << LSP_BU);
+            int units = b >= 0 ? 1 : 0;
+            for (int e = 0; e < nx * nx; ++e) units += (m >> e) & 1;
+            const int cost = lean_cost_scaled(s, nx, nu);
+            if (best == 0 || cost < best_cost || (cost == best_cost && units > best_units)) best = s, best_cost = cost, best_units = units;
+        }
+    }
+    return best;
 }
 
 #ifdef __HIPCC__
diff --git a/tinympc-julia_amd/csrc/kernels.hip b/tinympc-julia_amd/csrc/kernels.hip
--- a/tinympc-julia_amd/csrc/kernels.hip
+++ b/tinympc-julia_amd/csrc/kernels.hip
@@ -57,8 +57,58 @@
     return nullptr;
 }
 
-bool build_lean_pack(const Solver &sv, std::vector<double> &out) {
+uint64_t lean_scale_model(uint64_t built, int nx, int nu, const double *A, const double *B, double *s) {
+    const uint64_t sz = lean_pattern_scaled(built, nx, nu);
+    if (!sz || !lean_pattern_covers(built, lean_pattern_rm(nx, nu, A, B))) return 0;
+    if (lean_cost_scaled(sz, nx, nu) >= lean_cost_sparse(built, nx, nu)) return 0;
+    bool known[4] = {false, false, false, false};
+    int comp[4] = {0, 1, 2, 3};
+    for (int i = 0; i < nx; ++i)
+        for (int j = 0; j < nx; ++j)
+            if (i != j && lsp_one(sz, nx, i, j)) {
+                if (A[i * nx + j] == 0.0) return 0;
+                const int ci = comp[i], cj = comp[j];
+                for (int q = 0; q < nx; ++q)
+                    if (comp[q] == cj) comp[q] = ci;
+            }
+    for (int r = 0; r < nx; ++r) {
+        if (known[r]) continue;
+        s[r] = 1.0, known[r] = true;
+        for (int pass = 0; pass < nx; ++pass)
+            for (int i = 0; i < nx; ++i)
+                for (int j = 0; j < nx; ++j) {
+                    if (i == j || !lsp_one(sz, nx, i, j)) continue;
+                    if (known[j] && !known[i]) s[i] = s[j] / A[i * nx + j], known[i] = true;
+                    else if (known[i] && !known[j]) s[j] = s[i] * A[i * nx + j], known[j] = true;
+                }
+    }
+    for (int i = 0; i < nx; ++i)
+        for (int a = 0; a < nu; ++a)
+            if (lsp_b_one(sz, nu, i, a)) {
+                if (B[i * nu + a] == 0.0) return 0;
+                const double f = 1.0 / (B[i * nu + a] * s[i]);
+                for (int q = 0; q < nx; ++q)
+                    if (comp[q] == comp[i]) s[q] *= f;
+            }
+    for (int i = 0; i < nx; ++i)
+        if (!std::isfinite(s[i]) || s[i] == 0.0 || !std::isfinite(1.0 / (s[i] * s[i]))) return 0;
+    return sz;
+}
+void lean_scaled_coefficients(uint64_t sz, int nx, int nu, const double *A, const double *B, const double *K, const double *s,
+                              double *Ah, double *Bh, double *Kh) {
+    for (int i = 0; i < nx; ++i) {
+        for (int j = 0; j < nx; ++j)
+            Ah[i * nx + j] = i == j ? A[i * nx + j] : (lsp_one(sz, nx, i, j) ? 1.0 : s[i] * A[i * nx + j] / s[j]);
+        for (int a = 0; a < nu; ++a) Bh[i * nu + a] = lsp_b_one(sz, nu, i, a) ? 1.0 : s[i] * B[i * nu + a];
+    }
+    if (K && Kh)
+        for (int a = 0; a < nu; ++a)
+            for (int j = 0; j < nx; ++j) Kh[a * nx + j] = K[a * nx + j] / s[j];
+}
+
+bool build_lean_pack(const Solver &sv, std::vector<double> &out, bool *scaled) {
     const int nx = sv.nx, nu = sv.nu;
+    if (scaled) *scaled = false;
     const LeanLayout L = lean_layout(nx, nu);
     out.assign((size_t)L.total, 0.0);
     const Cache &c = sv.cache;
@@ -97,6 +147,22 @@
     for (int i = 0; i < nx; ++i)
         for (int j = 0; j < nx; ++j) out[L.oS + L.oM + i * nx + j] = sv.A(i, j);
     for (int i = L.oK; i < L.len; ++i) out[L.oS + i] = out[i];
+    if (sv.le && sv.le->sp_scaled && nx <= 4 && nu <= 4) {
+        double s[4];
+        const uint64_t sz = lean_scale_model(sv.le->sp, nx, nu, out.data() + L.oS + L.oM, out.data() + L.oS + L.oB, s);
+        if (sz && sz == sv.le->sp_scaled) {
+            double *z = out.data() + L.oZ;
+            lean_scaled_coefficients(sz, nx, nu, out.data() + L.oS + L.oM, out.data() + L.oS + L.oB, out.data() + L.oS + L.oK, s,
+                                     z + L.oM, z + L.oB, z + L.oK);
+            for (int i = 0; i < nu * nu; ++i) z[L.oC + i] = out[L.oC + i];
+            for (int i = 0; i < nx; ++i) {
+                z[L.oW + i] = 1.0 / (s[i] * s[i]);
+                out[L.oSc + i] = s[i];
+                out[L.oSi + i] = 1.0 / s[i];
+            }
+            if (scaled) *scaled = true;
+        }
+    }
     return true;
 }
 
@@ -175,6 +241,18 @@
     if (nx < 1 || nu < 1 || nx > 4 || nu > 4 || !out3) return 1;
     out3[0] = tmpc::lean_cost_sparse(sp, nx, nu), out3[1] = tmpc::lean_cost_hessenberg(nx, nu), out3[2] = tmpc::lean_cost_dense(nx, nu);
     return 0;
+}
+extern "C" unsigned long long tmpc_lean_scaled_pattern(int nx, int nu, unsigned long long sp) { return tmpc::lean_pattern_scaled(sp, nx, nu); }
+extern "C" int tmpc_lean_scaled_cost(int nx, int nu, unsigned long long sz) {
+    return (nx < 1 || nu < 1 || nx > 4 || nu > 4 || !tmpc::lsp_scaled(sz)) ? -1 : tmpc::lean_cost_scaled(sz, nx, nu);
+}
+extern "C" unsigned long long tmpc_lean_scale_model(int nx, int nu, const double *A, const double *B, unsigned long long built, double *s,
+                                                    double *Ah, double *Bh) {
+    if (nx < 1 || nu < 1 || nx > 4 || nu > 4 || !A || !B || !s || !Ah || !Bh) return 0;
+    if (!built) built = tmpc::lean_pattern_rm(nx, nu, A, B);
+    const uint64_t sz = tmpc::lean_scale_model(built, nx, nu, A, B, s);
+    if (sz) tmpc::lean_scaled_coefficients(sz, nx, nu, A, B, nullptr, s, Ah, Bh, nullptr);
+    return sz;
 }
 extern "C" int tmpc_lean_covers(unsigned long long built, unsigned long long model) { return tmpc::lean_pattern_covers(built, model) ? 1 : 0; }
 extern "C" int tmpc_lean_pick_form(int nx, int nu, unsigned long long built, unsigned long long model, int one, int live, int xb) {
diff --git a/tinympc-julia_amd/csrc/lean_entry.hip.h b/tinympc-julia_amd/csrc/lean_entry.hip.h
--- a/tinympc-julia_amd/csrc/lean_entry.hip.h
+++ b/tinympc-julia_amd/csrc/lean_entry.hip.h
@@ -102,6 +102,27 @@
                                    0.0, 0.0, 0.458, 1.002};
 constexpr double kCartpoleB[4] = {0.0, 0.02, 0.0, 0.067};
 constexpr uint64_t kCartpolePattern = lean_pattern_rm(4, 1, kCartpoleA, kCartpoleB);
+constexpr uint64_t kCartpolePatternScaled = lean_pattern_scaled(kCartpolePattern, 4, 1);
+static_assert(lean_cost_scaled(kCartpolePatternScaled, 4, 1) == 25 && lean_cost_sparse(kCartpolePattern, 4, 1) == 27, "cartpole: 25 for 27");
+
+template <int NX, int NU, int N, uint64_t SPZ>
+hipError_t launch_lean_scaled(TMPC_LEAN_ARGS) {
+    static_assert(lsp_scaled(SPZ), "a scaled pattern");
+    const int grid = (P.batch + 255) / 256;
+#define TMPC_LEAN_LAUNCH(LIVE_, ONE_) \
+    lean_dispatch(admm_lean_kernel<NX, NU, N, LIVE_, true, ONE_, false, REF_ZERO, float, SPZ>, grid, stream, ev0, ev1, P)
+    switch (variant & (LV_LIVE | LV_ONE)) {
+        case LV_LIVE | LV_ONE: TMPC_LEAN_LAUNCH(true, true); break;
+        case LV_ONE: TMPC_LEAN_LAUNCH(false, true); break;
+        default: return hipErrorNotSupported;
+    }
+#undef TMPC_LEAN_LAUNCH
+    return hipGetLastError();
+}
+#define TMPC_DEFINE_LEAN_SCALED(NX, NU, NN, SPZ)                                             \
+    hipError_t lean_scaled_##NX##_##NU##_##NN(TMPC_LEAN_ARGS) {                              \
+        return launch_lean_scaled<NX, NU, NN, (SPZ)>(P, variant, stream, ev0, ev1);          \
+    }
 
 #define TMPC_DECLARE_LEAN_PARTS(KIND, NX, NU, NN)                          \
     hipError_t lean_##KIND##_##NX##_##NU##_##NN##_z(TMPC_LEAN_ARGS);      \
@@ -124,20 +145,24 @@
 #define TMPC_DEFINE_LEAN_WS_SPARSE(NX, NU, NN, SP) TMPC_DEFINE_LEAN_PART_SPARSE(ws, true, false, NX, NU, NN, SP)
 #define TMPC_DEFINE_LEAN_MPC_PART(NX, NU, NN, TAG, XB, REFS) TMPC_DEFINE_LEAN_PART(mpc, true, true, NX, NU, NN, TAG, XB, REFS)
 #define TMPC_DEFINE_LEAN_MPC_SPARSE(NX, NU, NN, SP) TMPC_DEFINE_LEAN_PART_SPARSE(mpc, true, true, NX, NU, NN, SP)
-#define TMPC_DEFINE_LEAN_ENTRY_FULL(NX, NU, NN, SP)                                                                    \
+#define TMPC_DEFINE_LEAN_ENTRY_FULL(NX, NU, NN, SP, SPZ)                                                               \
     TMPC_DECLARE_LEAN_PARTS(ws, NX, NU, NN)                                                                            \
     TMPC_DECLARE_LEAN_PARTS(mpc, NX, NU, NN)                                                                           \
+    hipError_t lean_scaled_##NX##_##NU##_##NN(TMPC_LEAN_ARGS);                                                         \
+    const LeanEntry *lean_entry_##NX##_##NU##_##NN();                                                                  \
     static hipError_t lean_launch_##NX##_##NU##_##NN(TMPC_LEAN_ARGS) {                                                 \
         static constexpr LeanLaunch ws[5] = TMPC_LEAN_PARTS(ws, NX, NU, NN), mpc[5] = TMPC_LEAN_PARTS(mpc, NX, NU, NN); \
         if (variant & LV_F64) return hipErrorNotSupported;                                                             \
         const int part = (variant & LV_SPARSE) ? 4 : ((variant & LV_SHARED) ? 2 : 0) + ((variant & LV_XB) ? 1 : 0);    \
         if (variant & LV_MPC) return mpc[part](P, variant, stream, ev0, ev1);                                          \
         if (variant & LV_WS) return ws[part](P, variant, stream, ev0, ev1);                                            \
+        if (lean_runs_scaled(lean_entry_##NX##_##NU##_##NN(), variant, P.host_flags))                                  \
+            return lean_scaled_##NX##_##NU##_##NN(P, variant, stream, ev0, ev1);                                       \
         return part == 4 ? launch_lean_sparse<NX, NU, NN, (SP)>(P, variant, stream, ev0, ev1)                          \
                          : launch_lean<NX, NU, NN>(P, variant, stream, ev0, ev1);                                      \
     }                                                                                                                  \
     const LeanEntry *lean_entry_##NX##_##NU##_##NN() {                                                                 \
-        static const LeanEntry e = {NX, NU, NN, "lean<" #NX "," #NU "," #NN ">", (SP), LK_ALL, &lean_launch_##NX##_##NU##_##NN}; \
+        static const LeanEntry e = {NX, NU, NN, "lean<" #NX "," #NU "," #NN ">", (SP), LK_ALL, &lean_launch_##NX##_##NU##_##NN, (SPZ)}; \
         return &e;                                                                                                     \
     }
 
diff --git a/tinympc-julia_amd/csrc/linst_4_1_20.hip b/tinympc-julia_amd/csrc/linst_4_1_20.hip
--- a/tinympc-julia_amd/csrc/linst_4_1_20.hip
+++ b/tinympc-julia_amd/csrc/linst_4_1_20.hip
@@ -1,4 +1,4 @@
 #include "lean_entry.hip.h"
 namespace tmpc {
-TMPC_DEFINE_LEAN_ENTRY_FULL(4, 1, 20, kCartpolePattern)
+TMPC_DEFINE_LEAN_ENTRY_FULL(4, 1, 20, kCartpolePattern, kCartpolePatternScaled)
 }
diff --git a/tinympc-julia_amd/csrc/linst_4_1_20_scaled.hip b/tinympc-julia_amd/csrc/linst_4_1_20_scaled.hip
--- /dev/null
+++ b/tinympc-julia_amd/csrc/linst_4_1_20_scaled.hip
@@ -0,0 +1,4 @@
+#include "lean_entry.hip.h"
+namespace tmpc {
+TMPC_DEFINE_LEAN_SCALED(4, 1, 20, kCartpolePatternScaled)
+}
diff --git a/tinympc-julia_amd/csrc/solver.h b/tinympc-julia_amd/csrc/solver.h
--- a/tinympc-julia_amd/csrc/solver.h
+++ b/tinympc-julia_amd/csrc/solver.h
@@ -37,7 +37,13 @@
     uint64_t sp;
     int kinds;
     LeanLaunch launch;
-};
+    uint64_t sp_scaled = 0;
+};
+inline bool lean_runs_scaled(const LeanEntry *e, int variant, int host_flags) {
+    if (!e || !e->sp_scaled || !(host_flags & HF_LEAN_SCALED)) return false;
+    if ((variant & (LV_SPARSE | LV_UBK | LV_SHARED | LV_F64 | LV_WS | LV_MPC | LV_XB)) != (LV_SPARSE | LV_UBK)) return false;
+    return (variant & LV_ONE) != 0;
+}
 const LeanEntry *find_lean_kernel(int nx, int nu, int N);
 const LeanEntry *jit_lean_for(int nx, int nu, int N, int variant, uint64_t sp, int verbose);
 bool lean_ws_fits(int nx, int nu, int N, bool live, bool xb, bool shared, bool knot_bounds);
@@ -80,7 +86,10 @@
 };
 LeanPlan lean_plan(const LeanPlanIn &);
 uint64_t lean_pattern(const Mat &A, const Mat &B);
-bool build_lean_pack(const Solver &, std::vector<double> &);
+bool build_lean_pack(const Solver &, std::vector<double> &, bool *scaled = nullptr);
+uint64_t lean_scale_model(uint64_t built, int nx, int nu, const double *A, const double *B, double *s);
+void lean_scaled_coefficients(uint64_t sz, int nx, int nu, const double *A, const double *B, const double *K, const double *s,
+                              double *Ah, double *Bh, double *Kh);
 void append_lean_bounds(const Solver &, std::vector<double> &);
 struct StreamEntry {
     int nx, nu;
@@ -127,6 +136,7 @@
          no_uni = false, no_os = false, lean_one = false,
          no_jit = false,
          lean_dense = false,
+         lean_unscaled = false,
          lean_ws = false,
          lean_loop = false,
          stream_f64 = false,
@@ -212,6 +222,8 @@
     bool lean_ok = false, lean_knot_bounds = false;
     bool lean_enabled = true;
     uint64_t lean_sp = 0;
+    bool lean_scaled_ok = false;
+    bool last_lean_scaled = false;
     int last_lean_form = LF_NONE;
     int last_lean_cost[2] = {0, 0};
     std::string last_launch_name;
diff --git a/tinympc-julia_amd/csrc/solver.hip b/tinympc-julia_amd/csrc/solver.hip
--- a/tinympc-julia_amd/csrc/solver.hip
+++ b/tinympc-julia_amd/csrc/solver.hip
@@ -352,6 +352,7 @@
     w.no_os = on("TINYMPC_HIP_NO_OS");
     w.lean_one = on("TINYMPC_HIP_LEAN_ONE");
     w.lean_dense = on("TINYMPC_HIP_LEAN_DENSE");
+    w.lean_unscaled = on("TINYMPC_HIP_LEAN_UNSCALED");
     w.lean_ws = on("TINYMPC_HIP_LEAN_WS");
     w.lean_loop = on("TINYMPC_HIP_LEAN_LOOP");
     w.stream_f64 = on("TINYMPC_HIP_STREAM_F64");
@@ -660,10 +661,11 @@
     if (precision == 2 && !ke && !ce && !hetero && !extensions_active() && lean_enabled && !sw.no_jit && !no_specialise && !bounds_mode) lean_jit = true;
     std::fill(le_var_tried, le_var_tried + LV_COUNT, false);
     lean_ok = false;
+    lean_scaled_ok = false;
     lean_sp = lean_pattern(A, B);
     if (le || lean_jit) {
         std::vector<double> lp;
-        if (build_lean_pack(*this, lp)) {
+        if (build_lean_pack(*this, lp, &lean_scaled_ok)) {
             if (!le && (!ke || ke->G != 1)) append_lean_bounds(*this, lp);
             if (dev_alloc(d_lean, lp.size())) return -1;
             HIP_TRY(hipMemcpy(d_lean, lp.data(), lp.size() * sizeof(double), hipMemcpyHostToDevice));
@@ -1329,7 +1331,8 @@
         P.ib_hx = (long)batch * nx * (bounds_mode == 2 ? N : 1), P.ib_hu = (long)batch * nu * (bounds_mode == 2 ? N - 1 : 1);
         P.ib_on = (st.en_state_bound ? IB_STATE : 0) | (st.en_input_bound ? IB_INPUT : 0);
     }
-    P.host_flags = (sw.no_refill ? HF_NO_REFILL : 0) | (sw.no_uni ? HF_NO_UNI : 0) | (sw.no_os ? HF_NO_OS : 0);
+    P.host_flags = (sw.no_refill ? HF_NO_REFILL : 0) | (sw.no_uni ? HF_NO_UNI : 0) | (sw.no_os ? HF_NO_OS : 0) |
+                   (lean_ok && lean_scaled_ok && !sw.lean_unscaled ? HF_LEAN_SCALED : 0);
 }
 
 int Solver::ensure_mpc_log(int mpc_steps) {
@@ -1411,6 +1414,7 @@
     }
     last_launch_name = lean ? lk->name : kernel_name;
     last_lean_form = lean ? plan.form : LF_NONE;
+    last_lean_scaled = lean && lean_runs_scaled(lk, plan.variant, P.host_flags);
     last_lean_cost[0] = lean ? plan.cost_sparse : 0;
     last_lean_cost[1] = lean ? plan.cost_dense : 0;
     solved_once = true;
@@ -2123,4 +2127,6 @@
     return 0;
 }
 
+extern "C" int tmpc_lean_last_scaled(tinympc_solver *s) { return s ? (s->s.last_lean_scaled ? 1 : 0) : -1; }
+
 extern "C" int tmpc_last_rollout_launches(tinympc_solver *s) { return s ? s->s.last_rollout_launches : -1; }
```

Result: faster. 581.7 million, median of 6 (+4.1%).
